# Immortal-ibr/Verifiable-Federated-Training-with-Zero-Knowledge-Proofs-ZK-FL-

Hardware: AMD Instinct MI355X
Metric: Groth16 proofs/sec (training-step circuit, ~2^18 constraints) at 1/8 MI355X (higher is better)
Workload: dtype u32; 1 GPU; groth16 prove, sgd_verified(128, 4, 7, 1000) (BATCH,DIM,DEPTH,PRECISION); constraints=261399, wires=262810, domain=262144, global_batch=20, step=20 proofs per GPU (one per slot), parallelism=replicas1, slots_in_flight=20, hw_queues=28

## Files before the change

include/zkfl.h:

```cpp
#ifndef ZKFL_H
#define ZKFL_H

#include <stddef.h>
#include <stdint.h>

#ifdef __cplusplus
extern "C" {
#endif

#define ZKFL_OK 0
#define ZKFL_E_ARG -1
#define ZKFL_E_FORMAT -2
#define ZKFL_E_PRIME -3
#define ZKFL_E_MISMATCH -4
#define ZKFL_E_DEVICE -5
#define ZKFL_E_OOM -6
#define ZKFL_E_CONSTRAINT -7
#define ZKFL_E_KEY -8

typedef struct zkfl_ctx zkfl_ctx;
typedef struct zkfl_key zkfl_key;
typedef struct zkfl_witness zkfl_witness;
typedef struct zkfl_wprog zkfl_wprog;
typedef struct zkfl_vkey zkfl_vkey;

int zkfl_version(void);
const char* zkfl_build_id(void);
const char* zkfl_last_error(void);
int zkfl_device_count(int* count);

int zkfl_ctx_create(int device, zkfl_ctx** out);
int zkfl_ctx_destroy(zkfl_ctx* ctx);
int zkfl_ctx_set_profiling(zkfl_ctx* ctx, int enabled);
int zkfl_ctx_profile(zkfl_ctx* ctx, const char* name, double* total_ms, uint64_t* launches, double* units,
                     double* median_ms);
int zkfl_ctx_profile_reset(zkfl_ctx* ctx);
int zkfl_ctx_synchronize(zkfl_ctx* ctx);

int zkfl_zkey_load(zkfl_ctx* ctx, const uint8_t* buf, size_t len, zkfl_key** out);
typedef struct zkfl_zkey_file zkfl_zkey_file;
int zkfl_zkey_file_open(const char* path, zkfl_zkey_file** out);
int zkfl_zkey_load_file(zkfl_ctx* ctx, const zkfl_zkey_file* f, zkfl_key** out);
int zkfl_zkey_file_close(zkfl_zkey_file* f);
int zkfl_key_free(zkfl_key* key);
int zkfl_key_info(const zkfl_key* key, uint32_t* n_vars, uint32_t* n_public, uint32_t* domain_size);
int zkfl_key_ab_shared(const zkfl_key* key, uint32_t* d_form, uint32_t* shared_wires, uint32_t* a_bases);
int zkfl_debug_ab_partition(const uint8_t* sec_a, const uint8_t* sec_b1, size_t n, uint32_t shard, uint32_t n_shards,
                            uint32_t* counts, uint32_t* sidx_out, uint8_t* img_out);
typedef struct zkfl_groups_info {
  uint32_t grouped;
  uint32_t learned;
  uint32_t groups;
  uint32_t non_rep;
  uint32_t bases[4];
  uint32_t bases_rep[4];
  uint32_t builds;
  uint32_t last_miss;
  double build_ms;
} zkfl_groups_info;
typedef struct zkfl_group_rows_info {
  uint32_t rows_grouped;
  uint32_t row_classes;
  uint32_t terms;
  uint32_t terms_rep;
  uint32_t wire_list;
  uint32_t wires_over_cap;
  uint32_t last_dirty;
  uint32_t last_plain;
  double rows_build_ms;
} zkfl_group_rows_info;
int zkfl_key_set_groups(zkfl_key* key, const uint32_t* rep, size_t n_vars);
int zkfl_key_learn_groups(zkfl_ctx* ctx, zkfl_key* key, const zkfl_witness* w);
int zkfl_key_groups(const zkfl_key* key, zkfl_groups_info* out);
int zkfl_key_group_rows(const zkfl_key* key, zkfl_group_rows_info* out);
int zkfl_debug_groups(const uint8_t* values, const uint8_t* sig, size_t n, uint32_t* rep_out, const uint32_t* sidx,
                      size_t n_bases, uint32_t u_base, uint32_t* sidx_out, uint32_t* start_out,
                      uint32_t* members_out);
int zkfl_debug_group_rows(const uint32_t* rows, uint32_t domain, const uint32_t* cols, uint32_t cshift,
                          const uint32_t* coefs, const uint32_t* rep, uint32_t n_vars, uint32_t hash_bits,
                          uint32_t wire_cap, uint32_t* cls_out, uint32_t* crp_out, uint32_t* cterms_out,
                          uint32_t* ccoefs_out, uint32_t* wstart_out, uint32_t* wlist_out, uint32_t* info_out);
int zkfl_debug_abc(zkfl_ctx* ctx, zkfl_key* key, const zkfl_witness* w, int grouped, uint8_t* abc_out,
                   uint32_t* counts_out);
int zkfl_key_set_slots(zkfl_key* key, int slots);

int zkfl_groth16_prove(zkfl_ctx* ctx, zkfl_key* key, const uint8_t* wtns, size_t wtns_len,
                       const uint8_t* rs, uint8_t proof_out[256], uint8_t* pub_out, size_t* npub);

int zkfl_witness_upload(zkfl_ctx* ctx, const zkfl_key* key, const uint8_t* wtns, size_t wtns_len,
                        zkfl_witness** out);
int zkfl_witness_free(zkfl_witness* w);
int zkfl_groth16_prove_resident(zkfl_ctx* ctx, zkfl_key* key, const zkfl_witness* w, const uint8_t* rs,
                                uint8_t proof_out[256]);
int zkfl_groth16_prove_batch(zkfl_ctx* ctx, zkfl_key* key, size_t n, const zkfl_witness* const* w,
                             const uint8_t* rs, uint8_t* proofs_out);

int zkfl_groth16_prove_multi(zkfl_ctx* ctx, size_t n, zkfl_key* const* keys, const zkfl_witness* const* w,
                             const uint8_t* rs, uint8_t* proofs_out);

int zkfl_zkey_load_shard(zkfl_ctx* ctx, const uint8_t* buf, size_t len, uint32_t shard, uint32_t n_shards,
                         zkfl_key** out);
int zkfl_key_shard(const zkfl_key* key, uint32_t* shard, uint32_t* n_shards);
int zkfl_groth16_prove_part_batch(zkfl_ctx* ctx, zkfl_key* key, size_t n, const zkfl_witness* const* w,
                                  const uint8_t* rs, uint8_t* parts_out);
int zkfl_groth16_assemble(zkfl_ctx* ctx, size_t n, size_t n_parts, const uint8_t* parts, const uint8_t* rs,
                          uint8_t* proofs_out);

int zkfl_debug_prove_parts(zkfl_ctx* ctx, zkfl_key* key, const uint8_t* wtns, size_t wtns_len, uint8_t* h_out,
                           uint8_t* msm_out);

int zkfl_debug_glv_split(const uint8_t k[32], uint8_t out[40]);

int zkfl_debug_g1_glv_mul(zkfl_ctx* ctx, size_t n, const uint8_t* points, const uint8_t* scalars, uint8_t* out);

int zkfl_debug_msm_front(zkfl_ctx* ctx, uint32_t n1, const size_t* n, const uint8_t* const* bases,
                         const uint8_t* const* scalars, const size_t* n_scalars, const uint32_t* const* sidx,
                         const uint32_t* extra_start, const uint8_t* const* extra, const size_t* n_extra, uint32_t b,
                         const uint8_t* bases_g2, size_t n_b, int fast, int joint, uint8_t* out_g1, uint8_t out_g2[128]);

int zkfl_debug_wtrace(zkfl_ctx* ctx, int op, uint32_t cap, void* out, uint32_t* count);

int zkfl_debug_ntt_coset(zkfl_ctx* ctx, uint8_t* data, uint32_t logn, uint32_t nvec, size_t vstride, int col_max);

int zkfl_msm_g1(zkfl_ctx* ctx, const uint8_t* bases, const uint8_t* scalars, size_t n, uint8_t out[64]);
int zkfl_msm_g2(zkfl_ctx* ctx, const uint8_t* bases, const uint8_t* scalars, size_t n, uint8_t out[128]);
int zkfl_ntt_coset(zkfl_ctx* ctx, uint8_t* data, uint32_t logn);

int zkfl_wprog_load(zkfl_ctx* ctx, const uint8_t* prog, size_t len, zkfl_wprog** out);
int zkfl_wprog_free(zkfl_wprog* prog);
int zkfl_wprog_info(const zkfl_wprog* prog, uint32_t* n_wires, uint32_t* n_inputs, uint32_t* n_public);
size_t zkfl_wtns_size(const zkfl_wprog* prog);
int zkfl_wprog_parse_inputs(const uint8_t* prog, size_t len, const char* input_json, uint8_t* inputs_out, size_t cap,
                            size_t* n_inputs);
int zkfl_witness_compute_json(zkfl_ctx* ctx, const zkfl_wprog* prog, const char* input_json, uint8_t* wtns_out);
int zkfl_witness_compute(zkfl_ctx* ctx, const zkfl_wprog* prog, size_t n, const uint8_t* inputs, uint8_t* wtns_out);
int zkfl_witness_compute_resident(zkfl_ctx* ctx, const zkfl_wprog* prog, const zkfl_key* key, size_t n,
                                  const uint8_t* inputs, zkfl_witness** out);

int zkfl_groth16_full_prove_batch(zkfl_ctx* ctx, zkfl_key* key, const zkfl_wprog* prog, size_t n,
                                  const uint8_t* inputs, const uint8_t* rs, uint8_t* proofs_out, uint8_t* pubs_out);

int zkfl_groth16_full_prove_json(zkfl_ctx* ctx, zkfl_key* key, const zkfl_wprog* prog, const char* input_json,
                                 const uint8_t* rs, uint8_t proof_out[256], uint8_t* pub_out);

int zkfl_groth16_full_prove_json_batch(zkfl_ctx* ctx, zkfl_key* key, const zkfl_wprog* prog, size_t n,
                                       const char* const* input_jsons, const uint8_t* rs, uint8_t* proofs_out,
                                       uint8_t* pubs_out);

int zkfl_groth16_full_prove_multi(zkfl_ctx* ctx, size_t n, zkfl_key* const* keys, const zkfl_wprog* const* progs,
                                  const uint8_t* const* inputs, const uint8_t* rs, uint8_t* proofs_out,
                                  uint8_t* const* pubs_out);

typedef struct zkfl_r1cs zkfl_r1cs;
typedef struct {
  uint32_t n_wires, n_pub_out, n_pub_in, n_prv_in, n_constraints;
  uint64_t n_labels, n_terms;
} zkfl_r1cs_header;
typedef struct {
  uint32_t n_failed, first;
  uint8_t a[32], b[32], c[32];
// ... 132 lines not shown
```

verifiable-federated-training-with-zero-knowledge-proofs-zk-fl-_amd/csrc/groups.h:

```cpp
#pragma once
#include <stddef.h>
#include <stdint.h>
#include <string.h>

#include <algorithm>
#include <unordered_map>
#include <vector>

namespace zkfl {

inline bool groups_valid(const uint32_t* rep, size_t n) {
  for (size_t i = 0; i < n; i++)
    if (rep[i] > i || rep[rep[i]] != rep[i]) return false;
  return true;
}

inline void groups_learn(const uint32_t* w, size_t n, std::vector<uint32_t>& rep) {
  rep.resize(n);
  std::vector<uint32_t> big;
  for (size_t i = 0; i < n; i++) {
    rep[i] = (uint32_t)i;
    const uint32_t* v = w + 8 * i;
    if (v[4] | v[5] | v[6] | v[7]) big.push_back((uint32_t)i);
  }
  std::sort(big.begin(), big.end(), [&](uint32_t a, uint32_t b) {
    const int c = memcmp(w + 8 * (size_t)a, w + 8 * (size_t)b, 32);
    return c ? c < 0 : a < b;
  });
  for (size_t k = 1; k < big.size(); k++)
    if (memcmp(w + 8 * (size_t)big[k], w + 8 * (size_t)big[k - 1], 32) == 0) rep[big[k]] = rep[big[k - 1]];
}

inline void groups_refine(uint32_t* rep, const uint8_t* sig, size_t n) {
  std::unordered_map<uint64_t, uint32_t> first;
  for (size_t i = 0; i < n; i++) {
    const uint32_t r = rep[i];
    if ((sig[i] & ~sig[r]) == 0) continue;
    rep[i] = first.emplace((uint64_t)r << 8 | sig[i], (uint32_t)i).first->second;
  }
}

struct GroupQuery {
  std::vector<uint32_t> sidx;
  std::vector<uint32_t> start;
  std::vector<uint32_t> members;
  uint32_t groups = 0;
  uint32_t non_rep = 0;
};

inline void groups_query(const uint32_t* rep, uint32_t n_vars, const uint32_t* sidx, size_t n, uint32_t u_base,
                         GroupQuery& q) {
  constexpr uint32_t NONE = 0xFFFFFFFFu;
  std::vector<uint32_t> slot_of(n_vars, NONE), to(n, NONE);
  for (size_t j = 0; j < n; j++)
    if (sidx[j] < n_vars) slot_of[sidx[j]] = (uint32_t)j;
  q.sidx.assign(sidx, sidx + n);
  q.start.assign(n + 1, 0);
  q.groups = q.non_rep = 0;
  for (size_t j = 0; j < n; j++) {
    const uint32_t i = sidx[j];
    if (i >= n_vars || rep[i] == i || slot_of[rep[i]] == NONE) continue;
    to[j] = slot_of[rep[i]];
    q.sidx[j] = u_base + i;
    if (q.start[to[j] + 1]++ == 0) q.groups++;
    q.non_rep++;
  }
  for (size_t j = 0; j < n; j++) q.start[j + 1] += q.start[j];
  q.members.resize(q.non_rep);
  std::vector<uint32_t> cur(q.start.begin(), q.start.end() - 1);
  for (size_t j = 0; j < n; j++)
    if (to[j] != NONE) q.members[cur[to[j]]++] = (uint32_t)j;
}


constexpr uint32_t GROUP_ROWS_WIRE_CAP = 256;
constexpr uint32_t GROUP_ROWS_DIRTY_DIV = 8;
inline uint32_t group_rows_dirty_cap(uint32_t domain) { return std::max<uint32_t>(64u, domain / GROUP_ROWS_DIRTY_DIV); }
constexpr uint32_t GROUP_ROWS_MISS_DIV = 64;
inline uint32_t group_rows_miss_cap(uint32_t domain) { return std::max<uint32_t>(64u, domain / GROUP_ROWS_MISS_DIV); }
constexpr uint32_t GROUP_ROWS_OVER = 0x80000000u;

struct GroupRows {
  std::vector<uint32_t> cls;
  std::vector<uint32_t> crp;
  std::vector<uint32_t> cterms;
  std::vector<uint32_t> ccoefs;
  std::vector<uint32_t> wstart;
  std::vector<uint32_t> wlist;
  uint32_t classes = 0;
  uint32_t over_cap = 0;
  bool keep = false;
};

inline void group_rows_build(const uint32_t* rows, uint32_t domain, const uint32_t* cols, uint32_t cshift,
                             const uint32_t* coefs, const uint32_t* rep, uint32_t n_vars, uint32_t hash_bits,
                             uint32_t wire_cap, GroupRows& g) {
  const uint32_t nrows = 2 * domain, K = rows[nrows];
  const uint32_t cmask = cshift ? (1u << cshift) - 1u : 0xFFFFFFFFu;
  std::vector<uint64_t> key(K);
  std::vector<uint32_t> uniq;
  if (cshift) {
    for (uint32_t p = 0; p < K; p++) key[p] = (cols[p] & ~cmask) | rep[cols[p] & cmask];
  } else {
    struct H32 {
      const uint32_t* c;
      size_t operator()(uint32_t p) const {
        uint64_t h = 1469598103934665603ull;
        for (int k = 0; k < 8; k++) h = (h ^ c[8 * (size_t)p + k]) * 1099511628211ull;
        return (size_t)h;
      }
    };
    struct E32 {
      const uint32_t* c;
      bool operator()(uint32_t a, uint32_t b) const { return memcmp(c + 8 * (size_t)a, c + 8 * (size_t)b, 32) == 0; }
    };
    std::unordered_map<uint32_t, uint32_t, H32, E32> ids(16, H32{coefs}, E32{coefs});
    for (uint32_t p = 0; p < K; p++) {
      const auto it = ids.emplace(p, (uint32_t)uniq.size());
      if (it.second) uniq.push_back(p);
      key[p] = (uint64_t)it.first->second << 32 | rep[cols[p]];
    }
  }
  std::vector<uint64_t> hash(nrows);
  const uint64_t hmask = hash_bits >= 64 ? ~0ull : (1ull << hash_bits) - 1ull;
  for (uint32_t r = 0; r < nrows; r++) {
    std::sort(key.begin() + rows[r], key.begin() + rows[r + 1]);
    uint64_t h = 0x9E3779B97F4A7C15ull + (rows[r + 1] - rows[r]);
    for (uint32_t p = rows[r]; p < rows[r + 1]; p++) {
      h = (h ^ key[p]) * 0xFF51AFD7ED558CCDull;
      h ^= h >> 29;
    }
    hash[r] = h & hmask;
  }
  uint32_t tbits = 4;
  while ((1ull << tbits) < 2ull * nrows) tbits++;
  std::vector<uint32_t> table((size_t)1 << tbits, 0xFFFFFFFFu), first;
  const size_t tmask = ((size_t)1 << tbits) - 1;
  g.cls.assign(nrows, 0);
  g.crp.assign(1, 0);
  g.cterms.clear();
  g.ccoefs.clear();
  for (uint32_t r = 0; r < nrows; r++) {
    const uint32_t s = rows[r], len = rows[r + 1] - s;
    size_t slot = (size_t)((hash[r] * 0x9E3779B97F4A7C15ull) >> (64 - tbits)) & tmask;
    uint32_t c;
    for (;; slot = (slot + 1) & tmask) {
      c = table[slot];
      if (c == 0xFFFFFFFFu) break;
      const uint32_t f = first[c];
      if (hash[f] == hash[r] && rows[f + 1] - rows[f] == len &&
          std::equal(key.begin() + s, key.begin() + s + len, key.begin() + rows[f]))
        break;
    }
    if (c == 0xFFFFFFFFu) {
// ... 77 lines not shown
```

verifiable-federated-training-with-zero-knowledge-proofs-zk-fl-_amd/csrc/groups.hip:

```cpp
#include <hip/hip_runtime.h>
#include <stdint.h>

#include <chrono>
#include <cstdio>
#include <vector>

#include "devbufs.h"
#include "groups.h"
#include "objects.h"

using namespace zkfl;

namespace {

ZK_DEV Fq from_m29(const Fq& a) {
  Fq c = fp_zero<FqP>();
  c.v[7] = 0x08000000u;
  return fp_mul(a, c);
}

template <class F>
ZK_DEV Affine<F> load_base(const Affine<F>* __restrict__ p) {
  Affine<F> a = *p;
  Fq* q = reinterpret_cast<Fq*>(&a);
#pragma unroll
  for (int k = 0; k < (int)(sizeof(Affine<F>) / sizeof(Fq)); k++) q[k] = from_m29(q[k]);
  return a;
}

template <class F>
__global__ void __launch_bounds__(64) k_group_sums(const Affine<F>* __restrict__ bases_w, int W, size_t n,
                                                   const uint32_t* __restrict__ start,
                                                   const uint32_t* __restrict__ members, Affine<F>* __restrict__ out) {
  const size_t j = (size_t)blockIdx.x * blockDim.x + threadIdx.x;
  if (j >= n) return;
  const Affine<F> p = load_base<F>(bases_w + j * W);
  const uint32_t b = start[j], e = start[j + 1];
  if (b == e) {
    out[j] = p;
    return;
  }
  XYZZ<F> acc = xyzz_from_affine<F>(p);
  for (uint32_t m = b; m < e; m++) acc = xyzz_madd<F>(acc, load_base<F>(bases_w + (size_t)members[m] * W));
  out[j] = xyzz_to_affine<F>(acc);
}

constexpr int DELTA_T = 256;

__global__ void __launch_bounds__(DELTA_T) k_group_delta(const Fr* __restrict__ w, const uint32_t* __restrict__ rep,
                                                         uint32_t n, Fr* __restrict__ u, uint32_t* __restrict__ cnt,
                                                         uint32_t* __restrict__ miss_out, const GroupMark M) {
  ZK_LIGHT();
  const uint32_t i = blockIdx.x * DELTA_T + threadIdx.x;
  int nz = 0;
  if (i < n) {
    const uint32_t r = rep[i];
    Fr v = fp_zero<FrP>();
    if (r != i) {
      v = fp_sub(w[i], w[r]);
#pragma unroll
      for (int k = 0; k < 8; k++) nz |= v.v[k] != 0;
    }
    u[i] = v;
  }
  if (M.wstart) {
    const unsigned long long m = __ballot(nz);
    if (m) {
      const uint32_t lane = threadIdx.x & (warpSize - 1);
      const int first = __ffsll((long long)m) - 1;
      uint32_t base = 0;
      if ((int)lane == first) base = atomicAdd(&M.state[2], (uint32_t)__popcll(m));
      base = __shfl(base, first);
      const uint32_t at = base + (uint32_t)__popcll(m & ((1ull << lane) - 1ull));
      if (nz && at < M.miss_cap) M.missing[at] = i;
    }
  }
  const int blk = __syncthreads_count(nz);
  if (threadIdx.x == 0) {
    if (blk) atomicAdd(&cnt[0], (uint32_t)blk);
    __threadfence();
    if (atomicAdd(&cnt[1], 1u) == gridDim.x - 1) {
      __threadfence();
      miss_out[0] = atomicExch(&cnt[0], 0u);
      cnt[1] = 0;
    }
  }
}

constexpr int MARK_T = 256, MARK_BLOCKS_MAX = 256;

__global__ void __launch_bounds__(MARK_T) k_group_mark(const GroupMark M) {
  ZK_LIGHT();
  const uint32_t n = M.state[2];
  if (n == 0) return;
  if (n > M.miss_cap) {
    if (blockIdx.x == 0 && threadIdx.x == 0) atomicExch(&M.state[1], 1u);
    return;
  }
  const uint32_t lane = threadIdx.x & (warpSize - 1), per = MARK_T / warpSize;
  for (uint32_t k = blockIdx.x * per + threadIdx.x / warpSize; k < n; k += gridDim.x * per) {
    if (__any((int)__atomic_load_n(&M.state[1], __ATOMIC_RELAXED))) return;
    const uint32_t i = M.missing[k], s = M.wstart[i], e = M.wstart[i + 1] & ~GROUP_ROWS_OVER;
    if (s & GROUP_ROWS_OVER) {
      if (lane == 0) atomicExch(&M.state[1], 1u);
      return;
    }
    for (uint32_t p = s + lane; p < e; p += warpSize) {
      const uint32_t j = M.wlist[p], bit = 1u << (j & 31);
      if (atomicOr(&M.state[GROUP_ROWS_STATE_BITS + (j >> 5)], bit) & bit) continue;
      const uint32_t at = atomicAdd(&M.state[0], 1u);
      if (at < M.cap) M.dirty[at] = j;
      else atomicExch(&M.state[1], 1u);
    }
  }
}

}

namespace zkfl {

template <class F>
void group_sums(hipStream_t st, const Affine<F>* bases_w, int W, size_t n, const uint32_t* start,
                const uint32_t* members, Affine<F>* out) {
  if (n) hipLaunchKernelGGL(k_group_sums<F>, dim3(zk_grid(n, 64)), dim3(64), 0, st, bases_w, W, n, start, members, out);
}
template void group_sums<FqOps>(hipStream_t, const G1Aff*, int, size_t, const uint32_t*, const uint32_t*, G1Aff*);
template void group_sums<Fq2Ops>(hipStream_t, const G2Aff*, int, size_t, const uint32_t*, const uint32_t*, G2Aff*);

void group_delta(hipStream_t st, const Fr* w, const uint32_t* rep, uint32_t n, Fr* u, uint32_t* cnt,
                 uint32_t* miss_out, const GroupMark& mark) {
  hipLaunchKernelGGL(k_group_delta, dim3(zk_grid(n, DELTA_T)), dim3(DELTA_T), 0, st, w, rep, n, u, cnt, miss_out, mark);
}

void group_mark_rows(hipStream_t st, const GroupMark& mark) {
  const unsigned blocks = std::min<unsigned>(zk_grid((size_t)mark.miss_cap * 64, MARK_T), MARK_BLOCKS_MAX);
  hipLaunchKernelGGL(k_group_mark, dim3(blocks), dim3(MARK_T), 0, st, mark);
}

void key_groups_release(zkfl_key* k) {
  msm_bases_free(k->gA);
  msm_bases_free(k->gB1);
  msm_bases_free(k->gB2);
  msm_bases_free(k->gCH);
  void* ptrs[] = {k->grp.d_rep,    k->grp.d_cls,    k->grp.d_crp,  k->grp.d_cterms,
                  k->grp.d_ccoefs, k->grp.d_wstart, k->grp.d_wlist};
  for (void* p : ptrs)
    if (p) (void)hipFree(p);
  const uint32_t builds = k->grp.builds;
  k->grp = KeyGroups();
  k->grp.builds = builds;
}

}

namespace {

template <class F>
hipError_t build_query(const MsmBases<F>& plain, MsmBases<F>& out, const GroupQuery& q, uint32_t extra_start,
                       DevBufs& D, hipStream_t st) {
  ZK_CHECK(msm_bases_alloc(out, plain.n, plain.c));
  if (plain.n == 0) return hipSuccess;
  uint32_t *d_start, *d_members;
  Affine<F>* d_img;
  ZK_CHECK(D.get(&d_start, q.start.size()));
  ZK_CHECK(D.get(&d_members, q.members.size()));
  ZK_CHECK(D.get(&d_img, plain.n));
  ZK_CHECK(hipMemcpyAsync(d_start, q.start.data(), q.start.size() * 4, hipMemcpyHostToDevice, st));
  if (!q.members.empty())
    ZK_CHECK(hipMemcpyAsync(d_members, q.members.data(), q.members.size() * 4, hipMemcpyHostToDevice, st));
  group_sums<F>(st, plain.bases_w, msm_w_of(plain.c), plain.n, d_start, d_members, d_img);
  ZK_CHECK(hipGetLastError());
  return msm_bases_set(out, d_img, q.sidx.data(), extra_start, st, false);
}

bool group_rows_wanted(const zkfl_key* k) {
  return k->ctx->opts.group_rows && k->K != 0 && k->logn > k->ctx->opts.small_logn;
}

hipError_t build_rows(zkfl_key* k, const std::vector<uint32_t>& rep, hipStream_t st) {
  KeyGroups& g = k->grp;
  if (!group_rows_wanted(k)) return hipSuccess;
  const auto t0 = std::chrono::steady_clock::now();
  const uint32_t dom = k->n;
  const size_t K = k->K;
  std::vector<uint32_t> rows(2 * (size_t)dom + 1), cols(K), coefs;
  ZK_CHECK(hipMemcpyAsync(rows.data(), k->rows, rows.size() * 4, hipMemcpyDeviceToHost, st));
  ZK_CHECK(hipMemcpyAsync(cols.data(), k->cols, K * 4, hipMemcpyDeviceToHost, st));
  if (!k->cshift) {
    coefs.resize(K * 8);
    ZK_CHECK(hipMemcpyAsync(coefs.data(), k->coefs, K * 32, hipMemcpyDeviceToHost, st));
  }
  ZK_CHECK(hipStreamSynchronize(st));
  GroupRows R;
  const uint32_t low = (uint32_t)k->ctx->opts.group_rows_cap;
  group_rows_build(rows.data(), dom, cols.data(), k->cshift, coefs.data(), rep.data(), k->nVars, 64,
                   low ? std::min(low, GROUP_ROWS_WIRE_CAP) : GROUP_ROWS_WIRE_CAP, R);
  g.row_classes = R.classes;
  g.terms_rep = (uint32_t)R.cterms.size();
  g.wire_list = (uint32_t)R.wlist.size();
  g.over_cap = R.over_cap;
  if (R.keep && !R.cterms.empty()) {
    auto up = [&](auto*& dst, const std::vector<uint32_t>& v) -> hipError_t {
      ZK_CHECK(hipMalloc(&dst, (v.size() ? v.size() : 1) * 4));
      if (!v.empty()) ZK_CHECK(hipMemcpyAsync(dst, v.data(), v.size() * 4, hipMemcpyHostToDevice, st));
      return hipSuccess;
    };
    ZK_CHECK(up(g.d_cls, R.cls));
    ZK_CHECK(up(g.d_crp, R.crp));
    ZK_CHECK(up(g.d_cterms, R.cterms));
    if (!k->cshift) ZK_CHECK(up(g.d_ccoefs, R.ccoefs));
    ZK_CHECK(up(g.d_wstart, R.wstart));
    ZK_CHECK(up(g.d_wlist, R.wlist));
    ZK_CHECK(hipStreamSynchronize(st));
    g.rows_on = true;
  }
  g.rows_ms = std::chrono::duration<double, std::milli>(std::chrono::steady_clock::now() - t0).count();
  return hipSuccess;
}

int key_build_groups(zkfl_key* k, std::vector<uint32_t>& rep, bool learned, double host_ms) {
  const auto t0 = std::chrono::steady_clock::now();
  HIP_TRY(hipSetDevice(k->ctx->device), "hipSetDevice");
  int rc = key_reset_graphs(k);
  if (rc) return rc;
  key_groups_release(k);
  const uint32_t nV = k->nVars, X = nV, dom = k->n;
  std::vector<uint8_t> sig(nV, 0);
  for (int qi = 0; qi < 4; qi++)
    for (uint32_t i : k->q_sidx[qi])
      if (i < nV) sig[i] |= (uint8_t)(1u << qi);
  groups_refine(rep.data(), sig.data(), nV);
  const uint32_t u_base[4] = {X + 4, X + 4, X + 4, X + dom + 4};
  GroupQuery q[4];
  for (int qi = 0; qi < 4; qi++)
    groups_query(rep.data(), nV, k->q_sidx[qi].data(), k->q_sidx[qi].size(), u_base[qi], q[qi]);
  hipStream_t st = k->ctx->st;
  hipError_t e;
  {
    DevBufs D;
    e = hipMalloc(&k->grp.d_rep, (size_t)(nV ? nV : 1) * 4);
    if (e == hipSuccess) e = hipMemcpyAsync(k->grp.d_rep, rep.data(), (size_t)nV * 4, hipMemcpyHostToDevice, st);
    if (e == hipSuccess) e = build_query(k->bA, k->gA, q[0], X, D, st);
    if (e == hipSuccess) e = build_query(k->bB1, k->gB1, q[1], X, D, st);
    if (e == hipSuccess) e = build_query(k->bB2, k->gB2, q[2], X, D, st);
    if (e == hipSuccess) e = build_query(k->bCH, k->gCH, q[3], X, D, st);
    const hipError_t es = hipStreamSynchronize(st);
    if (e == hipSuccess) e = es;
    if (e == hipSuccess) e = build_rows(k, rep, st);
  }
  if (e != hipSuccess) {
    key_groups_release(k);
    return hip_fail(e, "grouped base sets");
  }
  KeyGroups& g = k->grp;
  g.on = true;
  g.learned = learned;
  for (uint32_t i = 0; i < nV; i++) g.non_rep += rep[i] != i;
  std::vector<uint8_t> has(nV, 0);
  for (uint32_t i = 0; i < nV; i++)
    if (rep[i] != i && !has[rep[i]]) {
      has[rep[i]] = 1;
      g.groups++;
    }
  for (int qi = 0; qi < 4; qi++) {
    g.bases[qi] = (uint32_t)k->q_sidx[qi].size();
    g.bases_rep[qi] = g.bases[qi] - q[qi].non_rep;
  }
  g.builds++;
  g.build_ms = host_ms + std::chrono::duration<double, std::milli>(std::chrono::steady_clock::now() - t0).count();
  fprintf(stderr,
          "zkfl: key of %u wires: %u groups, %u non-representative wires; bases A %u -> %u, B %u -> %u, C+H %u -> %u; "
          "%s and built in %.1f ms\n",
          nV, g.groups, g.non_rep, g.bases[0], g.bases_rep[0], g.bases[1], g.bases_rep[1], g.bases[3], g.bases_rep[3],
          learned ? "learned" : "set", g.build_ms);
  if (group_rows_wanted(k))
    fprintf(stderr,
            "zkfl: key of %u wires: %u row classes, terms %zu -> %u, wire lists %u entries (%u wires over the cap); "
            "%s ABC, built in %.1f ms of the above\n",
            nV, g.row_classes, k->K, g.terms_rep, g.wire_list, g.over_cap, g.rows_on ? "grouped" : "plain", g.rows_ms);
  return ZKFL_OK;
}

int groups_allowed(const zkfl_key* k) {
  if (k->nshards != 1) return fail(ZKFL_E_ARG, "groups: a sharded key keeps the plain form");
  if (!k->ctx->opts.groups) return fail(ZKFL_E_ARG, "groups: turned off on this context (ZKFL_GROUPS=0)");
  return ZKFL_OK;
}

}

int zkfl::key_learn_groups(zkfl_ctx* ctx, zkfl_key* k, const Fr* d_w) {
  const auto t0 = std::chrono::steady_clock::now();
  HIP_TRY(hipSetDevice(ctx->device), "hipSetDevice");
  std::vector<uint32_t> w((size_t)k->nVars * 8), rep;
  HIP_TRY(hipMemcpy(w.data(), d_w, w.size() * 4, hipMemcpyDeviceToHost), "download witness");
  groups_learn(w.data(), k->nVars, rep);
  const double ms = std::chrono::duration<double, std::milli>(std::chrono::steady_clock::now() - t0).count();
  return key_build_groups(k, rep, true, ms);
}

extern "C" {

int zkfl_key_set_groups(zkfl_key* key, const uint32_t* rep, size_t n_vars) {
  if (!key) return fail(ZKFL_E_ARG, "null key");
  if (!rep) {
    HIP_TRY(hipSetDevice(key->ctx->device), "hipSetDevice");
    const int rc = key_reset_graphs(key);
    if (rc) return rc;
    key_groups_release(key);
    return ZKFL_OK;
  }
  int rc = groups_allowed(key);
  if (rc) return rc;
  if (n_vars != key->nVars) return fail(ZKFL_E_ARG, "groups: rep must hold one entry per wire of the key");
  if (!groups_valid(rep, n_vars)) return fail(ZKFL_E_ARG, "groups: rep[i] <= i and rep[rep[i]] == rep[i] must hold");
  std::vector<uint32_t> r(rep, rep + n_vars);
  return key_build_groups(key, r, false, 0.0);
}

int zkfl_key_learn_groups(zkfl_ctx* ctx, zkfl_key* key, const zkfl_witness* w) {
  if (!ctx || !key || !w) return fail(ZKFL_E_ARG, "null argument");
  if (key->ctx != ctx) return fail(ZKFL_E_ARG, "groups: key of another context");
  if (w->key != key) return fail(ZKFL_E_MISMATCH, "witness uploaded for another key");
  const int rc = groups_allowed(key);
  if (rc) return rc;
  return key_learn_groups(ctx, key, w->d);
}

int zkfl_key_groups(const zkfl_key* key, zkfl_groups_info* out) {
  if (!key || !out) return fail(ZKFL_E_ARG, "null argument");
  const KeyGroups& g = key->grp;
  *out = zkfl_groups_info();
  out->grouped = g.on;
  out->learned = g.learned;
  out->groups = g.groups;
  out->non_rep = g.non_rep;
  for (int i = 0; i < 4; i++) {
    out->bases[i] = g.on ? g.bases[i] : (uint32_t)key->q_sidx[i].size();
    out->bases_rep[i] = g.on ? g.bases_rep[i] : out->bases[i];
  }
  out->builds = g.builds;
  out->last_miss = g.last_miss;
  out->build_ms = g.build_ms;
  return ZKFL_OK;
}

int zkfl_key_group_rows(const zkfl_key* key, zkfl_group_rows_info* out) {
  if (!key || !out) return fail(ZKFL_E_ARG, "null argument");
  const KeyGroups& g = key->grp;
  *out = zkfl_group_rows_info();
  out->rows_grouped = g.rows_on;
  out->row_classes = g.row_classes;
  out->terms = (uint32_t)key->K;
  out->terms_rep = g.row_classes ? g.terms_rep : out->terms;
  out->wire_list = g.wire_list;
  out->wires_over_cap = g.over_cap;
  out->last_dirty = g.last_dirty;
  out->last_plain = g.last_plain;
  out->rows_build_ms = g.rows_ms;
  return ZKFL_OK;
}

int zkfl_debug_group_rows(const uint32_t* rows, uint32_t domain, const uint32_t* cols, uint32_t cshift,
                          const uint32_t* coefs, const uint32_t* rep, uint32_t n_vars, uint32_t hash_bits,
                          uint32_t wire_cap, uint32_t* cls_out, uint32_t* crp_out, uint32_t* cterms_out,
                          uint32_t* ccoefs_out, uint32_t* wstart_out, uint32_t* wlist_out, uint32_t* info_out) {
  if (!rows || !rep || !cls_out || !crp_out || !cterms_out || !wstart_out || !wlist_out || !info_out ||
      cshift >= 32 || domain > 0x3FFFFFFFu)
    return fail(ZKFL_E_ARG, "debug_group_rows: bad arguments");
  const uint32_t K = rows[2 * (size_t)domain];
  if (K && (!cols || (!cshift && !coefs))) return fail(ZKFL_E_ARG, "debug_group_rows: terms missing");
  for (uint32_t r = 0; r < 2 * domain; r++)
    if (rows[r] > rows[r + 1]) return fail(ZKFL_E_ARG, "debug_group_rows: row pointers must not descend");
  if (!groups_valid(rep, n_vars)) return fail(ZKFL_E_ARG, "debug_group_rows: not a partition");
  const uint32_t cmask = cshift ? (1u << cshift) - 1u : 0xFFFFFFFFu;
  for (uint32_t p = 0; p < K; p++)
    if ((cols[p] & cmask) >= n_vars) return fail(ZKFL_E_ARG, "debug_group_rows: column past the wires");
  GroupRows R;
  group_rows_build(rows, domain, cols, cshift, coefs, rep, n_vars, hash_bits, wire_cap ? wire_cap : GROUP_ROWS_WIRE_CAP,
                   R);
  auto put = [](uint32_t* dst, const std::vector<uint32_t>& v) {
    if (dst && !v.empty()) memcpy(dst, v.data(), v.size() * 4);
  };
  put(cls_out, R.cls);
  put(crp_out, R.crp);
  put(cterms_out, R.cterms);
  put(ccoefs_out, R.ccoefs);
  put(wstart_out, R.wstart);
  put(wlist_out, R.wlist);
  info_out[0] = R.classes;
  info_out[1] = (uint32_t)R.cterms.size();
  info_out[2] = (uint32_t)R.wlist.size();
  info_out[3] = R.keep;
  return ZKFL_OK;
}

int zkfl_debug_groups(const uint8_t* values, const uint8_t* sig, size_t n, uint32_t* rep_out, const uint32_t* sidx,
                      size_t n_bases, uint32_t u_base, uint32_t* sidx_out, uint32_t* start_out,
                      uint32_t* members_out) {
  if (!rep_out || n > 0x7FFFFFF0u || (n_bases && !sidx)) return fail(ZKFL_E_ARG, "debug_groups: bad arguments");
  std::vector<uint32_t> rep;
  if (values) {
    std::vector<uint32_t> w(n * 8);
    memcpy(w.data(), values, n * 32);
    groups_learn(w.data(), n, rep);
  } else {
    rep.assign(rep_out, rep_out + n);
    if (!groups_valid(rep.data(), n)) return fail(ZKFL_E_ARG, "debug_groups: not a partition");
  }
  if (sig) groups_refine(rep.data(), sig, n);
  memcpy(rep_out, rep.data(), n * 4);
  if (sidx_out || start_out || members_out) {
    GroupQuery q;
    groups_query(rep.data(), (uint32_t)n, sidx, n_bases, u_base, q);
    if (sidx_out) memcpy(sidx_out, q.sidx.data(), n_bases * 4);
    if (start_out) memcpy(start_out, q.start.data(), (n_bases + 1) * 4);
    if (members_out && !q.members.empty()) memcpy(members_out, q.members.data(), q.members.size() * 4);
  }
  return ZKFL_OK;
}

}
```

verifiable-federated-training-with-zero-knowledge-proofs-zk-fl-_amd/csrc/msm.h:

```cpp
#pragma once
#include <algorithm>
#include <cstring>

#include "field29.h"
#include "msm_api.h"
#include "msm_sort.h"
#include "wtrace.h"

namespace zkfl {

template <class F>
struct MsmIO;
template <>
struct MsmIO<FqOps29> {
  using S = FqOps;
  static constexpr int LANES = 1;
  static constexpr int PIECES = 4;
  static ZK_DEV const uint4* piece(const Affine<S>* p, size_t i, int q) {
    return reinterpret_cast<const uint4*>(p + i) + q;
  }
  static ZK_DEV Affine<FqOps29> from_pieces(const uint32_t (&w)[4 * PIECES]) {
    Affine<FqOps29> a;
    uint32_t x[8], y[8];
#pragma unroll
// ... 411 lines not shown
  ZK_WT((L0 ? WT_WSUM0 : WT_WSUM1) | (MsmIO<F>::LANES == 2 ? WT_G2 : 0u));
  ZK_LIGHT();
  constexpr int RB = msm_wsum_rb<L0, Q0, C>();
  __shared__ XYZZ<S> sh[RB], shy[RB];
  msm_wsum_block<F, L0, Q0, C>(ta, blockIdx.y, blockIdx.x, threadIdx.x / MsmIO<F>::LANES, sh, shy, true);
}

template <class S1, class S2>
struct MsmJointArgs {
  MsmTailArgs<S1> a;
  MsmTailArgs<S2> b;
  int n1;
};
constexpr int MSM_JOINT_T = 128;

template <class F1, class F2, int MINW, class S1 = typename MsmIO<F1>::S, class S2 = typename MsmIO<F2>::S>
__global__ void __launch_bounds__(MSM_JOINT_T) __attribute__((amdgpu_waves_per_eu(MINW)))
k_msm_stitch_joint(const MsmJointArgs<S1, S2> ja, int level, int src) {
  ZK_WT(WT_STITCH | WT_JOINT);
  ZK_LIGHT();
  const int y = blockIdx.y;
  if (y < ja.n1) {
    if (ja.a.live[y][level - 1] == 0u) return;
    const uint32_t g = (blockIdx.x * MSM_JOINT_T + threadIdx.x) / MsmIO<F1>::LANES;
    const uint32_t N = msm_items_at<S1>(*ja.a.nnz[y], level, ja.a.target[y]);
    if (g * MSM_SG < N) msm_stitch_lane<F1>(ja.a, y, level, src, g, N);
  } else {
    const int z = y - ja.n1;
    if (ja.b.live[z][level - 1] == 0u) return;
    const uint32_t g = (blockIdx.x * MSM_JOINT_T + threadIdx.x) / MsmIO<F2>::LANES;
    const uint32_t N = msm_items_at<S2>(*ja.b.nnz[z], level, ja.b.target[z]);
    if (g * MSM_SG < N) msm_stitch_lane<F2>(ja.b, z, level, src, g, N);
  }
}

template <class F1, class F2, int MINW, class S1 = typename MsmIO<F1>::S, class S2 = typename MsmIO<F2>::S>
__global__ void __launch_bounds__(2 * MSM_STITCH_LAST) k_msm_stitch_last_joint(const MsmJointArgs<S1, S2> ja, int level,
                                                                                int src) {
  static_assert(MsmIO<F1>::LANES == 1 && MsmIO<F2>::LANES == 2, "joint tails: G1 lanes, G2 lane pairs");
  ZK_WT(WT_STITCH | WT_JOINT);
  ZK_LIGHT();
  const int y = blockIdx.y;
  if (y < ja.n1)
    msm_stitch_last_block<F1>(ja.a, y, level, src);
  else
    msm_stitch_last_block<F2>(ja.b, y - ja.n1, level, src);
}

template <class F1, class F2, int MINW, bool L0, int Q0, int C, class S1 = typename MsmIO<F1>::S,
          class S2 = typename MsmIO<F2>::S>
__global__ void __launch_bounds__((2 * msm_wsum_rb<L0, Q0, C>())) __attribute__((amdgpu_waves_per_eu(MINW)))
k_msm_wsum_joint(const MsmJointArgs<S1, S2> ja) {
  ZK_WT((L0 ? WT_WSUM0 : WT_WSUM1) | WT_JOINT);
  ZK_LIGHT();
  constexpr int RB = msm_wsum_rb<L0, Q0, C>();
  constexpr int NBLK = L0 ? msm_nb_of(C) / (MSM_RB * Q0) : 1;
  constexpr size_t B1 = 2 * 2 * RB * sizeof(XYZZ<S1>), B2 = 2 * RB * sizeof(XYZZ<S2>);
  __shared__ __attribute__((aligned(16))) unsigned char lds[B1 > B2 ? B1 : B2];
  const int y = blockIdx.y;
  if (y < ja.n1) {
    if (2 * (int)blockIdx.x >= NBLK) return;
    const int half = threadIdx.x / RB, bx = 2 * blockIdx.x + half;
    XYZZ<S1>* sh = reinterpret_cast<XYZZ<S1>*>(lds) + half * 2 * RB;
    msm_wsum_block<F1, L0, Q0, C>(ja.a, y, bx, threadIdx.x % RB, sh, sh + RB, bx < NBLK);
  } else {
    XYZZ<S2>* sh = reinterpret_cast<XYZZ<S2>*>(lds);
    msm_wsum_block<F2, L0, Q0, C>(ja.b, y - ja.n1, blockIdx.x, threadIdx.x / MsmIO<F2>::LANES, sh, sh + RB, true);
  }
}

template <class F>
hipError_t msm_bases_alloc(MsmBases<F>& b, size_t n, int c) {
  if (c != MSM_C && c != MSM_C_SMALL) return hipErrorInvalidValue;
  b.n = n;
  b.c = c;
  ZK_CHECK(hipMalloc(&b.bases_w, (n ? n : 1) * msm_w_of(c) * sizeof(Affine<F>)));
  return hipSuccess;
}

template <class F>
void msm_bases_free(MsmBases<F>& b) {
  if (b.bases_w) (void)hipFree(b.bases_w);
  if (b.sidx) (void)hipFree(b.sidx);
  b = MsmBases<F>();
}

template <class F>
hipError_t msm_bases_set(MsmBases<F>& b, const Affine<F>* d_bases, const uint32_t* h_sidx, uint32_t extra_start,
                         hipStream_t st, bool pairs) {
  if (pairs && !std::is_same<F, FqOps>::value) return hipErrorInvalidValue;
  b.extra_start = h_sidx ? extra_start : 0xFFFFFFFFu;
  if (h_sidx && b.n) {
    ZK_CHECK(hipMalloc(&b.sidx, b.n * sizeof(uint32_t)));
    ZK_CHECK(hipMemcpyAsync(b.sidx, h_sidx, b.n * sizeof(uint32_t), hipMemcpyHostToDevice, st));
  }
  if (b.n)
    ZK_CHECK(msm_with_c(b.c, [&](auto cc) {
      constexpr int C = decltype(cc)::value;
      if constexpr (std::is_same<F, FqOps>::value) {
        if (pairs) {
          hipLaunchKernelGGL((k_msm_expand<F, C, true>), dim3(zk_grid(b.n, 64)), dim3(64), 0, st, d_bases, b.n,
                             b.bases_w);
          return hipSuccess;
        }
      }
      hipLaunchKernelGGL((k_msm_expand<F, C>), dim3(zk_grid(b.n, 64)), dim3(64), 0, st, d_bases, b.n, b.bases_w);
      return hipSuccess;
    }));
  const size_t nfq = b.n * msm_w_of(b.c) * (sizeof(Affine<F>) / sizeof(Fq));
  if (nfq)
    hipLaunchKernelGGL(k_msm_to_m29, dim3(zk_grid(nfq, 256)), dim3(256), 0, st, reinterpret_cast<Fq*>(b.bases_w), nfq);
  return hipGetLastError();
}

template <class F>
hipError_t msm_scratch_alloc(MsmScratch<F>& s, size_t cap, int c, hipStream_t st) {
  s.cap = cap;
  s.c = c;
  const size_t m = cap * msm_w_of(c);
  ZK_CHECK(hipMalloc(&s.keys_in, m * sizeof(uint16_t)));
  ZK_CHECK(hipMalloc(&s.keys_out, m * sizeof(uint16_t)));
  ZK_CHECK(hipMalloc(&s.vals_in, m * sizeof(uint32_t)));
  ZK_CHECK(hipMalloc(&s.vals_out, m * sizeof(uint32_t)));
  s.sort_tmp_bytes = MSM_SORT_TMP_WORDS * sizeof(uint32_t);
  ZK_CHECK(hipMalloc(&s.sort_tmp, s.sort_tmp_bytes));
  (void)st;
  return hipSuccess;
}

template <class F>
void msm_scratch_free(MsmScratch<F>& s) {
  void* ptrs[] = {s.keys_in, s.keys_out, s.vals_in, s.vals_out, s.sort_tmp};
  for (void* p : ptrs)
    if (p) (void)hipFree(p);
  s = MsmScratch<F>();
}

template <class F>
uint32_t msm_resident_chunks() {
  if (const char* e = getenv("ZKFL_MSM_TARGET")) return (uint32_t)strtoul(e, nullptr, 10);
  using FC = typename MsmCurve<F>::Compute;
  constexpr int AW = MsmCurve<F>::ACC_WAVES;
  int dev = 0, ncu = 0, nb = 0;
  if (hipGetDevice(&dev) != hipSuccess) return 0;
  if (hipDeviceGetAttribute(&ncu, hipDeviceAttributeMultiprocessorCount, dev) != hipSuccess) return 0;
  if (hipOccupancyMaxActiveBlocksPerMultiprocessor(&nb, k_msm_accumulate<FC, AW>, 64, 0) != hipSuccess) return 0;
  if (ncu <= 0 || nb <= 0) return 0;
  return (uint32_t)ncu * (uint32_t)nb * (64u / MsmIO<FC>::LANES);
}

template <class F>
uint32_t msm_tail_l0(size_t cap) {
  static_assert(MSM_SMALL_L >= 1 && MSM_SMALL_L <= 255 && MsmCurve<F>::L >= 1 && MsmCurve<F>::L <= 255,
                "chunk length: 8 bits of the target argument");
  return cap <= ((size_t)1 << 16) ? (uint32_t)MSM_SMALL_L : (uint32_t)MsmCurve<F>::L;
}

template <class F>
hipError_t msm_tail_alloc(MsmTail<F>& t, size_t cap, int c) {
  if (c != MSM_C && c != MSM_C_SMALL) return hipErrorInvalidValue;
  t.c = c;
  const size_t m = cap * msm_w_of(c);
  t.target = std::min<uint32_t>(msm_resident_chunks<F>(), 0xFFFFFFu);
  t.l0 = msm_tail_l0<F>(cap);
  t.max_chunks = (m + t.l0 - 1) / t.l0;
  if (t.target) t.max_chunks = std::min<size_t>(t.max_chunks, t.target);
  t.item_cap[0] = 2 * t.max_chunks;
  t.item_cap[1] = 2 * ((t.item_cap[0] + MSM_SG - 1) / MSM_SG);
  for (int k = 0; k < 2; k++) {
    ZK_CHECK(hipMalloc(&t.item_key[k], (t.item_cap[k] ? t.item_cap[k] : 2) * sizeof(uint32_t)));
    ZK_CHECK(hipMalloc(&t.item_val[k], (t.item_cap[k] ? t.item_cap[k] : 2) * sizeof(XYZZ<F>)));
  }
  ZK_CHECK(hipMalloc(&t.buckets, msm_nb_of(c) * sizeof(XYZZ<F>)));
  ZK_CHECK(hipMalloc(&t.red_a, MSM_TAIL_RED * sizeof(XYZZ<F>)));
  ZK_CHECK(hipMalloc(&t.red_s, MSM_TAIL_RED * sizeof(XYZZ<F>)));
  ZK_CHECK(hipMalloc(&t.nnz, sizeof(uint32_t)));
  ZK_CHECK(hipMalloc(&t.live, MSM_LIVE_LEVELS * sizeof(uint32_t)));
  return hipSuccess;
}

template <class F>
void msm_tail_free(MsmTail<F>& t) {
  void* ptrs[] = {t.item_key[0], t.item_key[1], t.item_val[0], t.item_val[1], t.buckets, t.red_a, t.red_s, t.nnz,
                  t.live};
  for (void* p : ptrs)
    if (p) (void)hipFree(p);
  t = MsmTail<F>();
}

template <class F>
MsmTailArgs<F> msm_tail_args(MsmTail<F>* const* t, XYZZ<F>* const* outs, int n) {
  MsmTailArgs<F> ta = {};
  ta.c = n > 0 ? t[0]->c : MSM_C;
  for (int i = 0; i < n; i++) {
    for (int k = 0; k < 2; k++) {
      ta.key[i][k] = t[i]->item_key[k];
      ta.val[i][k] = t[i]->item_val[k];
    }
    ta.buckets[i] = t[i]->buckets;
    ta.red_a[i] = t[i]->red_a;
    ta.red_s[i] = t[i]->red_s;
    ta.nnz[i] = t[i]->nnz;
    ta.out[i] = outs ? outs[i] : nullptr;
    ta.live[i] = t[i]->live;
    ta.target[i] = msm_target_arg(*t[i]);
  }
  return ta;
}

template <class F>
bool msm_tails_one_c(MsmTail<F>* const* t, int n) {
  for (int i = 1; i < n; i++)
    if (t[i]->c != t[0]->c) return false;
  return true;
}

template <class F>
hipError_t msm_tails_reset(MsmTail<F>* const* t, int n, hipStream_t st) {
  if (n < 1 || n > MSM_TAIL_MAX || !msm_tails_one_c(t, n)) return hipErrorInvalidValue;
  hipLaunchKernelGGL(k_msm_tail_reset<F>, dim3(128, n), dim3(256), 0, st, msm_tail_args<F>(t, nullptr, n));
  return hipGetLastError();
}

template <class F>
hipError_t msm_sort_multi(const MsmBases<F>* const* b, MsmScratch<F>* const* pl, uint32_t* const* nnz,
                          const uint32_t* const* sc, const uint32_t* const* ex, int n, hipStream_t st) {
  if (n < 1 || n > MSM_TAIL_MAX) return hipErrorInvalidValue;
  MsmSortArgs A = {};
  uint32_t gx = 0;
  int ny = 0;
  bool sorted = true;
  const int c = b[0]->c;
  for (int i = 0; i < n; i++) {
    const size_t m = b[i]->n;
    if (m > pl[i]->cap || b[i]->c != c || pl[i]->c != c) return hipErrorInvalidValue;
    if (m == 0) {
      continue;
    }
    uint32_t per_blk, nblk;
    if (!msm_sort_blocking(m, per_blk, nblk)) return hipErrorInvalidValue;
    MsmSortJob& J = A.j[ny++];
    J = {sc[i], ex[i], b[i]->sidx, b[i]->extra_start, (uint32_t)m, per_blk, nblk,
         static_cast<uint32_t*>(pl[i]->sort_tmp), static_cast<uint32_t*>(pl[i]->sort_tmp) + MSM_SORT_HB * MSM_SORT_MAXBLK,
         nnz[i], pl[i]->keys_in, pl[i]->vals_in, pl[i]->keys_out, pl[i]->vals_out};
    gx = std::max(gx, nblk);
    sorted = sorted && pl[i]->ko_sorted;
    pl[i]->ko_sorted = 1;
  }
  if (ny == 0) return hipSuccess;
  return msm_sort_launch(A, gx, ny, c, sorted, st);
}

template <class F>
hipError_t msm_sort(const MsmBases<F>& b, MsmScratch<F>& pl, uint32_t* nnz, const uint32_t* d_scalars,
                    const uint32_t* d_extra, hipStream_t st) {
  const MsmBases<F>* bp = &b;
  MsmScratch<F>* pp = &pl;
  return msm_sort_multi(&bp, &pp, &nnz, &d_scalars, &d_extra, 1, st);
}

template <class F>
hipError_t msm_accumulate_sorted(const MsmBases<F>& b, const uint16_t* keys, const uint32_t* vals, MsmTail<F>& t,
                                 hipStream_t st, Profiler* prof, const char* tag) {
  if (b.n == 0) return hipSuccess;
  if (b.c != t.c) return hipErrorInvalidValue;
  const size_t m = b.n * msm_w_of(b.c);
  size_t chunks = (m + t.l0 - 1) / t.l0;
  if (t.target) chunks = std::min<size_t>(chunks, t.target);
  if (chunks > t.max_chunks) return hipErrorInvalidValue;
  const int pidx = prof ? prof->begin(tag, st) : -1;
  using FC = typename MsmCurve<F>::Compute;
  constexpr int LN = MsmIO<FC>::LANES;
  constexpr int AW = MsmCurve<F>::ACC_WAVES;
  if (!((ZK_KNOCKOUT & 64) && LN == 1))
    hipLaunchKernelGGL((k_msm_accumulate<FC, AW>), dim3(zk_grid(chunks * LN, 64)), dim3(64), 0, st, keys, vals,
                       b.bases_w, t.nnz, t.item_key[0], t.item_val[0], t.buckets, msm_target_arg(t), t.live);
  if (prof) prof->end(pidx, st, 0.0, t.nnz);
  return hipGetLastError();
}

template <class F>
hipError_t msm_accumulate_sorted_multi(const MsmBases<F>* const* b, const uint16_t* const* keys,
                                       const uint32_t* const* vals, MsmTail<F>* const* t, int n, hipStream_t st) {
  if (n < 1 || n > MSM_TAIL_MAX) return hipErrorInvalidValue;
  using FC = typename MsmCurve<F>::Compute;
  constexpr int LN = MsmIO<FC>::LANES;
  constexpr int AW = MsmCurve<F>::ACC_WAVES;
  MsmAccArgs<F> A = {};
  size_t gx = 0;
  int ny = 0;
  for (int i = 0; i < n; i++) {
    if (b[i]->n == 0) continue;
    if (b[i]->c != t[i]->c) return hipErrorInvalidValue;
    const size_t m = b[i]->n * msm_w_of(b[i]->c);
    size_t chunks = (m + t[i]->l0 - 1) / t[i]->l0;
    if (t[i]->target) chunks = std::min<size_t>(chunks, t[i]->target);
    if (chunks > t[i]->max_chunks) return hipErrorInvalidValue;
    gx = std::max<size_t>(gx, zk_grid(chunks * LN, 64));
    A.keys[ny] = keys[i];
    A.vals[ny] = vals[i];
    A.bases[ny] = b[i]->bases_w;
    A.nnz[ny] = t[i]->nnz;
    A.item_key[ny] = t[i]->item_key[0];
    A.item_val[ny] = t[i]->item_val[0];
    A.buckets[ny] = t[i]->buckets;
    A.target[ny] = msm_target_arg(*t[i]);
    A.live[ny] = t[i]->live;
    ny++;
  }
  if (ny && !((ZK_KNOCKOUT & 64) && LN == 1))
    hipLaunchKernelGGL((k_msm_accumulate_multi<FC, AW>), dim3((uint32_t)gx, ny), dim3(64), 0, st, A);
  return hipGetLastError();
}

template <class F>
hipError_t msm_accumulate(const MsmBases<F>& b, MsmScratch<F>& pl, MsmTail<F>& t, const uint32_t* d_scalars,
                          const uint32_t* d_extra, hipStream_t st, Profiler* prof, const char* tag) {
  ZK_CHECK(msm_sort(b, pl, t.nnz, d_scalars, d_extra, st));
  return msm_accumulate_sorted(b, pl.keys_out, pl.vals_out, t, st, prof, tag);
}

template <class F>
hipError_t msm_stitch(MsmTail<F>* const* t, int n, hipStream_t st) {
  if (n < 1 || n > MSM_TAIL_MAX || !msm_tails_one_c(t, n)) return hipErrorInvalidValue;
  using FC = typename MsmCurve<F>::Compute;
  constexpr int LN = MsmIO<FC>::LANES;
  constexpr int SW = MsmCurve<F>::STITCH_WAVES;
  const MsmTailArgs<F> ta = msm_tail_args<F>(t, nullptr, n);
  size_t N = 0;
  for (int i = 0; i < n; i++) N = std::max(N, t[i]->item_cap[0]);
  N = std::max<size_t>(N, 2);
  int cur = 0;
  for (int level = 1; !(ZK_KNOCKOUT & 8); level++) {
    if (level >= MSM_LIVE_LEVELS) return hipErrorInvalidValue;
    const size_t lanes = (N + MSM_SG - 1) / MSM_SG;
    if (lanes <= (size_t)MSM_STITCH_LAST) {
      hipLaunchKernelGGL((k_msm_stitch_last<FC, SW>), dim3(1, n), dim3(MSM_STITCH_LAST * LN), 0, st, ta, level, cur);
      break;
    }
    hipLaunchKernelGGL((k_msm_stitch<FC, SW>), dim3(zk_grid(lanes * LN, 64), n), dim3(64), 0, st, ta, level, cur);
    if (N <= (size_t)MSM_SG) break;
    N = 2 * lanes;
    cur ^= 1;
  }
  return hipGetLastError();
}

template <class F>
hipError_t msm_wsum(const MsmTailArgs<F>& ta, int n, hipStream_t st, bool fast) {
  if (n < 1 || n > MSM_TAIL_MAX) return hipErrorInvalidValue;
  if (ZK_KNOCKOUT & 16) return hipGetLastError();
  using FC = typename MsmCurve<F>::Compute;
  constexpr int LN = MsmIO<FC>::LANES;
  constexpr int TW = MsmCurve<F>::TAIL_WAVES;
  return msm_with_c(ta.c, [&](auto cc) {
    constexpr int C = decltype(cc)::value, NB = msm_nb_of(C);
    constexpr int Q0 = MsmCurve<F>::WSUM_Q, QF = msm_wsum_q_fast<C>();
    if (fast) {
      hipLaunchKernelGGL((k_msm_wsum<FC, TW, true, QF, C>), dim3(NB / (MSM_RB * QF), n), dim3(MSM_RB * LN), 0, st, ta);
      hipLaunchKernelGGL((k_msm_wsum<FC, TW, false, QF, C>), dim3(1, n), dim3(msm_wsum_rb<false, QF, C>() * LN), 0, st,
                         ta);
    } else {
      hipLaunchKernelGGL((k_msm_wsum<FC, TW, true, Q0, C>), dim3(NB / (MSM_RB * Q0), n), dim3(MSM_RB * LN), 0, st, ta);
      hipLaunchKernelGGL((k_msm_wsum<FC, TW, false, Q0, C>), dim3(1, n), dim3(msm_wsum_rb<false, Q0, C>() * LN), 0, st,
                         ta);
    }
    return hipGetLastError();
  });
}

template <class F>
hipError_t msm_tails(MsmTail<F>* const* t, XYZZ<F>* const* outs, int n, hipStream_t st, bool fast) {
  ZK_CHECK(msm_stitch(t, n, st));
  return msm_wsum(msm_tail_args<F>(t, outs, n), n, st, fast);
}

template <class S1, class S2>
hipError_t msm_tails_joint(MsmTail<S1>* const* t1, XYZZ<S1>* const* o1, int n1, MsmTail<S2>* const* t2,
                           XYZZ<S2>* const* o2, int n2, hipStream_t st, bool fast) {
  if (n1 < 1 || n1 > MSM_TAIL_MAX || n2 < 1 || n2 > MSM_TAIL_MAX || !msm_tails_one_c(t1, n1) ||
      !msm_tails_one_c(t2, n2) || t1[0]->c != t2[0]->c)
    return hipErrorInvalidValue;
  using F1 = typename MsmCurve<S1>::Compute;
  using F2 = typename MsmCurve<S2>::Compute;
  static_assert(MsmCurve<S1>::WSUM_Q == MsmCurve<S2>::WSUM_Q, "joint reduction: one fold for both curves");
  constexpr int W = std::min(MsmCurve<S1>::TAIL_WAVES, MsmCurve<S2>::TAIL_WAVES);
  constexpr int L1 = MsmIO<F1>::LANES, L2 = MsmIO<F2>::LANES;
  static_assert(L1 == 1 && L2 == 2, "joint tails: G1 lanes, G2 lane pairs");
  MsmJointArgs<S1, S2> ja;
  ja.a = msm_tail_args<S1>(t1, o1, n1);
  ja.b = msm_tail_args<S2>(t2, o2, n2);
  ja.n1 = n1;
  const int ny = n1 + n2;
  size_t N1 = 2, N2 = 2;
  for (int i = 0; i < n1; i++) N1 = std::max(N1, t1[i]->item_cap[0]);
  for (int i = 0; i < n2; i++) N2 = std::max(N2, t2[i]->item_cap[0]);
  int cur = 0;
  for (int level = 1; !(ZK_KNOCKOUT & 8); level++) {
    if (level >= MSM_LIVE_LEVELS) return hipErrorInvalidValue;
    const size_t lanes1 = (N1 + MSM_SG - 1) / MSM_SG, lanes2 = (N2 + MSM_SG - 1) / MSM_SG;
    if (lanes1 <= (size_t)MSM_STITCH_LAST && lanes2 <= (size_t)MSM_STITCH_LAST) {
      hipLaunchKernelGGL((k_msm_stitch_last_joint<F1, F2, W>), dim3(1, ny), dim3(2 * MSM_STITCH_LAST), 0, st, ja,
                         level, cur);
      break;
    }
    const size_t bx = std::max(zk_grid(lanes1 * L1, MSM_JOINT_T), zk_grid(lanes2 * L2, MSM_JOINT_T));
    hipLaunchKernelGGL((k_msm_stitch_joint<F1, F2, W>), dim3((uint32_t)bx, ny), dim3(MSM_JOINT_T), 0, st, ja, level, cur);
    if (N1 > (size_t)MSM_SG) N1 = 2 * lanes1;
    if (N2 > (size_t)MSM_SG) N2 = 2 * lanes2;
    cur ^= 1;
  }
  if (ZK_KNOCKOUT & 16) return hipGetLastError();
  return msm_with_c(t1[0]->c, [&](auto cc) {
    constexpr int C = decltype(cc)::value, NB = msm_nb_of(C);
    constexpr int Q0 = MsmCurve<S1>::WSUM_Q, QF = msm_wsum_q_fast<C>();
    if (fast) {
      hipLaunchKernelGGL((k_msm_wsum_joint<F1, F2, W, true, QF, C>), dim3(NB / (MSM_RB * QF), ny),
                         dim3(2 * msm_wsum_rb<true, QF, C>()), 0, st, ja);
      hipLaunchKernelGGL((k_msm_wsum_joint<F1, F2, W, false, QF, C>), dim3(1, ny), dim3(2 * msm_wsum_rb<false, QF, C>()),
                         0, st, ja);
    } else {
      hipLaunchKernelGGL((k_msm_wsum_joint<F1, F2, W, true, Q0, C>), dim3(NB / (MSM_RB * Q0), ny),
                         dim3(2 * msm_wsum_rb<true, Q0, C>()), 0, st, ja);
      hipLaunchKernelGGL((k_msm_wsum_joint<F1, F2, W, false, Q0, C>), dim3(1, ny), dim3(2 * msm_wsum_rb<false, Q0, C>()),
                         0, st, ja);
    }
    return hipGetLastError();
  });
}

template <class F>
hipError_t msm_run(const MsmBases<F>& b, MsmScratch<F>& pl, MsmTail<F>& t, const uint32_t* d_scalars,
                   const uint32_t* d_extra, XYZZ<F>* d_out, hipStream_t st, Profiler* prof, const char* tag) {
  MsmTail<F>* tp = &t;
  ZK_CHECK(msm_tails_reset(&tp, 1, st));
  ZK_CHECK(msm_accumulate(b, pl, t, d_scalars, d_extra, st, prof, tag));
  return msm_tails(&tp, &d_out, 1, st);
}

}
```

verifiable-federated-training-with-zero-knowledge-proofs-zk-fl-_amd/csrc/msm_api.h:

```cpp
#pragma once
#include <hip/hip_runtime.h>

#include <cstdlib>
#include <type_traits>

#include "common.h"
#include "curve.h"
#include "prof.h"

namespace zkfl {

constexpr int MSM_C = 16;
constexpr int MSM_C_SMALL = 14;
constexpr int MSM_SMALL_C_BASES = 1 << 16;
constexpr int MSM_SORT_HIGH_BITS = 7;
constexpr int MSM_SORT_BIN_THREADS = 1024;
constexpr int MSM_SG = 8;
constexpr int MSM_SMALL_L = 8;

struct FqOps29;
struct Fq2Pair29;
template <class S>
struct MsmCurve;
template <>
struct MsmCurve<FqOps> {
  using Compute = FqOps29;
  static constexpr int ACC_WAVES = 3, STITCH_WAVES = 2, TAIL_WAVES = 2;
  static constexpr int L = 16, WSUM_Q = 16;
};
template <>
struct MsmCurve<Fq2Ops> {
  using Compute = Fq2Pair29;
  static constexpr int ACC_WAVES = 2, STITCH_WAVES = 2, TAIL_WAVES = 2;
  static constexpr int L = 16, WSUM_Q = 16;
};

__host__ __device__ constexpr int msm_w_of(int c) { return (255 + c - 1) / c; }
__host__ __device__ constexpr int msm_nb_of(int c) { return 1 << (c - 1); }
constexpr int MSM_W = msm_w_of(MSM_C);
constexpr int MSM_NB = msm_nb_of(MSM_C);
constexpr int MSM_W_MAX = msm_w_of(MSM_C < MSM_C_SMALL ? MSM_C : MSM_C_SMALL);
static_assert(MSM_C >= 14 && MSM_C <= 16 && MSM_C_SMALL >= 14 && MSM_C_SMALL <= 16,
              "window width: the widths the GPU parity suite runs (>= 64 low counters per high bin of the bucket sort)");
#ifndef ZK_KNOCKOUT
#define ZK_KNOCKOUT 0
#endif
#if ZK_KNOCKOUT != 0 && !defined(ZK_KNOCKOUT_AB_ONLY)
#error "ZK_KNOCKOUT builds compute wrong proofs: timing A/B only (define ZK_KNOCKOUT_AB_ONLY to acknowledge)"
#endif
constexpr int MSM_RB = 64;
constexpr uint32_t MSM_ITEM_DUMMY = 0x80000000u;
template <class S>
__host__ __device__ inline uint32_t msm_chunk_len(uint32_t nnz, uint32_t target) {
  const uint32_t L0 = (target >> 24) ? (target >> 24) : (uint32_t)MsmCurve<S>::L;
  target &= 0xFFFFFFu;
  if (target == 0) return L0;
  const uint32_t l = (uint32_t)(((uint64_t)nnz + target - 1) / target);
  return l > L0 ? l : L0;
}
constexpr int MSM_LIVE_LEVELS = 32;


template <class F>
struct MsmBases {
  size_t n = 0;
  int c = MSM_C;
  Affine<F>* bases_w = nullptr;
  uint32_t* sidx = nullptr;
  uint32_t extra_start = 0xFFFFFFFFu;
};

template <class F>
struct MsmScratch {
  size_t cap = 0;
  int c = MSM_C;
  uint16_t* keys_in = nullptr;
  uint16_t* keys_out = nullptr;
  uint32_t* vals_in = nullptr;
  uint32_t* vals_out = nullptr;
  void* sort_tmp = nullptr;
  size_t sort_tmp_bytes = 0;
  int ko_sorted = 0;
};

template <class F>
struct MsmTail {
  size_t max_chunks = 0;
  int c = MSM_C;
  uint32_t* item_key[2] = {nullptr, nullptr};
  XYZZ<F>* item_val[2] = {nullptr, nullptr};
  size_t item_cap[2] = {0, 0};
  XYZZ<F>* buckets = nullptr;
  XYZZ<F>* red_a = nullptr;
  XYZZ<F>* red_s = nullptr;
  uint32_t* nnz = nullptr;
  uint32_t* live = nullptr;
  uint32_t target = 0;
  uint32_t l0 = 0;
};

template <class F>
inline uint32_t msm_target_arg(const MsmTail<F>& t) {
  return (t.l0 << 24) | (t.target & 0xFFFFFFu);
}

inline int msm_pick_c(size_t n) {
  if (const char* e = getenv("ZKFL_MSM_C")) {
    const int c = atoi(e);
    if (c == MSM_C || c == MSM_C_SMALL) return c;
  }
  return n <= (size_t)MSM_SMALL_C_BASES ? MSM_C_SMALL : MSM_C;
}
template <class Fn>
hipError_t msm_with_c(int c, Fn&& fn) {
  if (c == MSM_C) return fn(std::integral_constant<int, MSM_C>());
  if constexpr (MSM_C_SMALL != MSM_C)
    if (c == MSM_C_SMALL) return fn(std::integral_constant<int, MSM_C_SMALL>());
  return hipErrorInvalidValue;
}

constexpr int MSM_TAIL_MAX = 4;
constexpr int MSM_TAIL_RED = 4 * MSM_RB;

template <class F>
hipError_t msm_bases_alloc(MsmBases<F>& b, size_t n, int c);
template <class F>
hipError_t msm_bases_set(MsmBases<F>& b, const Affine<F>* src, const uint32_t* h_sidx, uint32_t extra_start,
                         hipStream_t st, bool pairs = false);
template <class F>
void msm_bases_free(MsmBases<F>& b);
template <class F>
hipError_t msm_scratch_alloc(MsmScratch<F>& s, size_t cap, int c, hipStream_t st);
template <class F>
void msm_scratch_free(MsmScratch<F>& s);
template <class F>
hipError_t msm_tail_alloc(MsmTail<F>& t, size_t cap, int c);
template <class F>
void msm_tail_free(MsmTail<F>& t);
template <class F>
hipError_t msm_accumulate(const MsmBases<F>& b, MsmScratch<F>& s, MsmTail<F>& t, const uint32_t* scalars,
                          const uint32_t* extra, hipStream_t st, Profiler* prof, const char* tag);
template <class F>
hipError_t msm_tails_reset(MsmTail<F>* const* t, int n, hipStream_t st);
template <class F>
hipError_t msm_sort(const MsmBases<F>& b, MsmScratch<F>& s, uint32_t* nnz, const uint32_t* sc, const uint32_t* ex,
                    hipStream_t st);
template <class F>
hipError_t msm_accumulate_sorted(const MsmBases<F>& b, const uint16_t* keys, const uint32_t* vals, MsmTail<F>& t,
                                 hipStream_t st, Profiler* prof, const char* tag);
template <class F>
hipError_t msm_tails(MsmTail<F>* const* t, XYZZ<F>* const* outs, int n, hipStream_t st, bool fast = false);
template <class F>
hipError_t msm_run(const MsmBases<F>& b, MsmScratch<F>& s, MsmTail<F>& t, const uint32_t* scalars,
                   const uint32_t* extra, XYZZ<F>* out, hipStream_t st, Profiler* prof, const char* tag);
template <class F>
hipError_t msm_sort_multi(const MsmBases<F>* const* b, MsmScratch<F>* const* s, uint32_t* const* nnz,
                          const uint32_t* const* sc, const uint32_t* const* ex, int n, hipStream_t st);
template <class F>
hipError_t msm_accumulate_sorted_multi(const MsmBases<F>* const* b, const uint16_t* const* keys,
                                       const uint32_t* const* vals, MsmTail<F>* const* t, int n, hipStream_t st);

#define ZKFL_MSM_API(X, F)                                                                                     \
  X hipError_t msm_bases_alloc<F>(MsmBases<F>&, size_t, int);                                                  \
  X hipError_t msm_bases_set<F>(MsmBases<F>&, const Affine<F>*, const uint32_t*, uint32_t, hipStream_t, bool); \
  X void msm_bases_free<F>(MsmBases<F>&);                                                                      \
  X hipError_t msm_scratch_alloc<F>(MsmScratch<F>&, size_t, int, hipStream_t);                                 \
  X void msm_scratch_free<F>(MsmScratch<F>&);                                                                  \
  X hipError_t msm_tail_alloc<F>(MsmTail<F>&, size_t, int);                                                    \
  X void msm_tail_free<F>(MsmTail<F>&);                                                                        \
  X hipError_t msm_accumulate<F>(const MsmBases<F>&, MsmScratch<F>&, MsmTail<F>&, const uint32_t*,             \
                                 const uint32_t*, hipStream_t, Profiler*, const char*);                        \
  X hipError_t msm_tails_reset<F>(MsmTail<F>* const*, int, hipStream_t);                                       \
  X hipError_t msm_sort<F>(const MsmBases<F>&, MsmScratch<F>&, uint32_t*, const uint32_t*, const uint32_t*,    \
                           hipStream_t);                                                                       \
  X hipError_t msm_accumulate_sorted<F>(const MsmBases<F>&, const uint16_t*, const uint32_t*, MsmTail<F>&,     \
                                        hipStream_t, Profiler*, const char*);                                  \
  X hipError_t msm_tails<F>(MsmTail<F>* const*, XYZZ<F>* const*, int, hipStream_t, bool);                      \
  X hipError_t msm_run<F>(const MsmBases<F>&, MsmScratch<F>&, MsmTail<F>&, const uint32_t*, const uint32_t*,   \
                          XYZZ<F>*, hipStream_t, Profiler*, const char*);                                      \
  X hipError_t msm_sort_multi<F>(const MsmBases<F>* const*, MsmScratch<F>* const*, uint32_t* const*,           \
                                 const uint32_t* const*, const uint32_t* const*, int, hipStream_t);            \
  X hipError_t msm_accumulate_sorted_multi<F>(const MsmBases<F>* const*, const uint16_t* const*,               \
                                              const uint32_t* const*, MsmTail<F>* const*, int, hipStream_t);
ZKFL_MSM_API(extern template, FqOps)
ZKFL_MSM_API(extern template, Fq2Ops)

hipError_t msm_tails_joint(MsmTail<FqOps>* const* t1, XYZZ<FqOps>* const* o1, int n1, MsmTail<Fq2Ops>* const* t2,
                           XYZZ<Fq2Ops>* const* o2, int n2, hipStream_t st, bool fast);

}
```

verifiable-federated-training-with-zero-knowledge-proofs-zk-fl-_amd/csrc/msm_joint.hip:

```cpp
#include "msm.h"

namespace zkfl {
hipError_t zk_wtrace_bind_joint(const WtBuf& b) { return zk_wtrace_bind_tu(b); }
hipError_t msm_tails_joint(MsmTail<FqOps>* const* t1, XYZZ<FqOps>* const* o1, int n1, MsmTail<Fq2Ops>* const* t2,
                           XYZZ<Fq2Ops>* const* o2, int n2, hipStream_t st, bool fast) {
  return msm_tails_joint<FqOps, Fq2Ops>(t1, o1, n1, t2, o2, n2, st, fast);
}
}
```

verifiable-federated-training-with-zero-knowledge-proofs-zk-fl-_amd/csrc/msm_sort.h:

```cpp
#pragma once
#include "msm_api.h"

namespace zkfl {

constexpr int MSM_SORT_T = 256;
constexpr int MSM_SORT_HB = 1 << MSM_SORT_HIGH_BITS;
constexpr int MSM_SORT_MAXBLK = 32768 / MSM_SORT_HB;
constexpr int MSM_SORT_BT = 1024;
constexpr int MSM_SORT_BINT = MSM_SORT_BIN_THREADS;
static_assert(MSM_SORT_HB <= MSM_SORT_T, "bucket sort split");
static_assert(MSM_SORT_HB * MSM_SORT_MAXBLK == 32 * MSM_SORT_BT, "scan: 32 counters per thread");
constexpr size_t MSM_SORT_TMP_WORDS = MSM_SORT_HB * MSM_SORT_MAXBLK + MSM_SORT_HB + 1;

struct MsmSortJob {
  const uint32_t* scalars;
  const uint32_t* extra;
  const uint32_t* sidx;
  uint32_t extra_start;
  uint32_t n, per_blk, nblk;
  uint32_t* cnt;
  uint32_t* bin_start;
  uint32_t* nnz;
  uint16_t* keys_in;
  uint32_t* vals_in;
  uint16_t* keys_out;
  uint32_t* vals_out;
};
struct MsmSortArgs {
  MsmSortJob j[MSM_TAIL_MAX];
};

inline bool msm_sort_blocking(size_t m, uint32_t& per_blk, uint32_t& nblk) {
  const size_t per = (m + MSM_SORT_MAXBLK - 1) / MSM_SORT_MAXBLK;
  const size_t pb = per < MSM_SORT_T ? (size_t)MSM_SORT_T : (per + MSM_SORT_T - 1) / MSM_SORT_T * MSM_SORT_T;
  per_blk = (uint32_t)pb;
  nblk = (uint32_t)((m + pb - 1) / pb);
  return nblk <= (uint32_t)MSM_SORT_MAXBLK;
}

hipError_t msm_sort_launch(const MsmSortArgs& A, uint32_t gx, int ny, int c, bool sorted, hipStream_t st);

}
```

verifiable-federated-training-with-zero-knowledge-proofs-zk-fl-_amd/csrc/msm_sort.hip:

```cpp
#include "msm_sort.h"
#include "wtrace.h"

namespace zkfl {

hipError_t zk_wtrace_bind_sort(const WtBuf& b) { return zk_wtrace_bind_tu(b); }

template <int C>
constexpr int msm_sort_lb() {
  return C - 1 - MSM_SORT_HIGH_BITS;
}
template <int C>
constexpr int msm_sort_nl() {
  return 1 << msm_sort_lb<C>();
}

template <int C>
ZK_DEV uint32_t msm_window(const uint32_t (&s)[8], int j) {
  const int b = C * j, w = b >> 5, sh = b & 31;
  uint32_t x = s[w] >> sh;
  if (sh + C > 32 && w + 1 < 8) x |= s[w + 1] << (32 - sh);
  return x & ((1u << C) - 1u);
}

template <int C, class Fn>
ZK_DEV void msm_for_digits(const uint32_t* __restrict__ scalars, const uint32_t* __restrict__ extra,
                           const uint32_t* __restrict__ sidx, uint32_t extra_start, size_t i, Fn&& fn) {
  constexpr int W = msm_w_of(C), NB = msm_nb_of(C);
  const uint32_t si = sidx ? sidx[i] : (uint32_t)i;
  const uint32_t* src = si < extra_start ? scalars + (size_t)si * 8 : extra + (size_t)(si - extra_start) * 8;
  const uint4* sp = reinterpret_cast<const uint4*>(src);
  const uint4 a = sp[0], b = sp[1];
  const uint32_t s[8] = {a.x, a.y, a.z, a.w, b.x, b.y, b.z, b.w};
  uint32_t carry = 0;
#pragma unroll
  for (int j = 0; j < W; j++) {
    const uint32_t raw = msm_window<C>(s, j);
    int32_t d = (int32_t)(raw + carry);
    carry = d > NB ? 1u : 0u;
    if (carry) d -= (1 << C);
    if (d != 0) {
      const uint32_t mag = (uint32_t)(d < 0 ? -d : d);
      fn(mag - 1, (uint32_t)(i * W + j) | (d < 0 ? 0x80000000u : 0u));
    }
  }
}

template <int C>
__global__ void __launch_bounds__(MSM_SORT_T) k_msm_bin_count(const MsmSortArgs A) {
  ZK_WT(WT_SORT_COUNT);
  ZK_LIGHT();
  constexpr int LB = msm_sort_lb<C>();
  const MsmSortJob& J = A.j[blockIdx.y];
  if (blockIdx.x >= J.nblk) return;
  __shared__ uint32_t h[MSM_SORT_HB];
  if (threadIdx.x < MSM_SORT_HB) h[threadIdx.x] = 0;
  __syncthreads();
  const size_t i0 = (size_t)blockIdx.x * J.per_blk, i1 = i0 + J.per_blk < J.n ? i0 + J.per_blk : J.n;
  for (size_t i = i0 + threadIdx.x; i < i1; i += MSM_SORT_T)
    msm_for_digits<C>(J.scalars, J.extra, J.sidx, J.extra_start, i,
                      [&](uint32_t key, uint32_t) { atomicAdd(&h[key >> LB], 1u); });
  __syncthreads();
  if (threadIdx.x < MSM_SORT_HB) J.cnt[(size_t)threadIdx.x * J.nblk + blockIdx.x] = h[threadIdx.x];
}

#if defined(__HIP_DEVICE_COMPILE__) && !defined(__gfx950__)
#error "the bucket sort's scan needs gfx950's 160 KB of LDS"
#endif
static __global__ void __launch_bounds__(MSM_SORT_BT) k_msm_bin_scan(const MsmSortArgs A) {
  ZK_WT(WT_SORT_SCAN);
  ZK_LIGHT();
  const MsmSortJob& J = A.j[blockIdx.y];
  uint32_t* __restrict__ cnt = J.cnt;
  uint32_t* __restrict__ bin_start = J.bin_start;
  const uint32_t nblk = J.nblk;
  __shared__ uint32_t c[MSM_SORT_HB * MSM_SORT_MAXBLK + MSM_SORT_BT];
  __shared__ uint32_t part[MSM_SORT_BT];
  const uint32_t total = MSM_SORT_HB * nblk, t = threadIdx.x;
  for (uint32_t k = t; k < total; k += MSM_SORT_BT) c[k + (k >> 5)] = cnt[k];
  __syncthreads();
  uint32_t s = 0;
  for (uint32_t q = 0; q < 32; q++) {
    const uint32_t k = t * 32 + q;
    if (k < total) s += c[k + (k >> 5)];
  }
  part[t] = s;
  __syncthreads();
  for (uint32_t off = 1; off < MSM_SORT_BT; off <<= 1) {
    const uint32_t v = t >= off ? part[t - off] : 0u;
    __syncthreads();
    part[t] += v;
    __syncthreads();
  }
  uint32_t run = part[t] - s;
  for (uint32_t q = 0; q < 32; q++) {
    const uint32_t k = t * 32 + q;
    if (k < total) {
      const uint32_t v = c[k + (k >> 5)];
      c[k + (k >> 5)] = run;
      run += v;
    }
  }
  __syncthreads();
  for (uint32_t k = t; k < total; k += MSM_SORT_BT) {
    const uint32_t v = c[k + (k >> 5)];
    cnt[k] = v;
    if (k % nblk == 0) bin_start[k / nblk] = v;
  }
  if (t == MSM_SORT_BT - 1) {
    bin_start[MSM_SORT_HB] = part[t];
    *J.nnz = part[t];
  }
}

template <int C>
__global__ void __launch_bounds__(MSM_SORT_T) k_msm_bin_scatter(const MsmSortArgs A) {
  ZK_WT(WT_SORT_SCATTER);
  ZK_LIGHT();
  constexpr int LB = msm_sort_lb<C>();
  const MsmSortJob& J = A.j[blockIdx.y];
  if (blockIdx.x >= J.nblk) return;
  __shared__ uint32_t cur[MSM_SORT_HB];
  if (threadIdx.x < MSM_SORT_HB) cur[threadIdx.x] = J.cnt[(size_t)threadIdx.x * J.nblk + blockIdx.x];
  __syncthreads();
  uint16_t* __restrict__ keys = J.keys_in;
  uint32_t* __restrict__ vals = J.vals_in;
  const size_t i0 = (size_t)blockIdx.x * J.per_blk, i1 = i0 + J.per_blk < J.n ? i0 + J.per_blk : J.n;
  for (size_t i = i0 + threadIdx.x; i < i1; i += MSM_SORT_T)
    msm_for_digits<C>(J.scalars, J.extra, J.sidx, J.extra_start, i, [&](uint32_t key, uint32_t val) {
      const uint32_t p = atomicAdd(&cur[key >> LB], 1u);
      keys[p] = (uint16_t)key;
      vals[p] = val;
    });
}

template <int BINT, int NL>
__global__ void __launch_bounds__(BINT) k_msm_bin_sort(const MsmSortArgs A) {
  static_assert(BINT >= NL && BINT <= 1024 && NL >= 64, "bins: one thread per low counter");
  ZK_WT(WT_SORT_BINS);
  ZK_LIGHT();
  const MsmSortJob& J = A.j[blockIdx.y];
  const uint32_t* __restrict__ bin_start = J.bin_start;
  const uint16_t* __restrict__ tk = J.keys_in;
  const uint32_t* __restrict__ tv = J.vals_in;
  uint16_t* __restrict__ ko = J.keys_out;
  uint32_t* __restrict__ vo = J.vals_out;
  __shared__ uint32_t c[NL];
  const uint32_t b0 = bin_start[blockIdx.x], b1 = bin_start[blockIdx.x + 1], t = threadIdx.x;
  if (b0 == b1) return;
  if (t < NL) c[t] = 0;
  __syncthreads();
  for (uint32_t p = b0 + t; p < b1; p += BINT) atomicAdd(&c[tk[p] & (NL - 1)], 1u);
  __syncthreads();
  uint32_t v = 0, x = 0;
  if (t < NL) {
    v = c[t];
    x = v;
#pragma unroll
    for (int o = 1; o < 64; o <<= 1) {
      const uint32_t y = __shfl_up(x, o);
      if ((t & 63) >= (uint32_t)o) x += y;
    }
  }
  __shared__ uint32_t wt[NL / 64];
  if (t < NL && (t & 63) == 63) wt[t >> 6] = x;
  __syncthreads();
  if (t < NL) {
    uint32_t base = b0;
    for (uint32_t w = 0; w < (t >> 6); w++) base += wt[w];
    c[t] = base + x - v;
  }
  __syncthreads();
  for (uint32_t p = b0 + t; p < b1; p += BINT) {
    const uint16_t key = tk[p];
    const uint32_t val = tv[p];
    const uint32_t q = atomicAdd(&c[key & (NL - 1)], 1u);
    ko[q] = key;
    vo[q] = val;
  }
}

hipError_t msm_sort_launch(const MsmSortArgs& A, uint32_t gx, int ny, int c, bool sorted, hipStream_t st) {
  return msm_with_c(c, [&](auto cc) {
    constexpr int C = decltype(cc)::value;
    constexpr int NL = msm_sort_nl<C>();
    static_assert(NL >= 64 && NL <= 1024 && MSM_SORT_BINT >= NL, "bins: one thread per low counter");
    hipLaunchKernelGGL((k_msm_bin_count<C>), dim3(gx, ny), dim3(MSM_SORT_T), 0, st, A);
    hipLaunchKernelGGL(k_msm_bin_scan, dim3(1, ny), dim3(MSM_SORT_BT), 0, st, A);
    if (!(ZK_KNOCKOUT & 2) || !sorted) {
      hipLaunchKernelGGL((k_msm_bin_scatter<C>), dim3(gx, ny), dim3(MSM_SORT_T), 0, st, A);
      hipLaunchKernelGGL((k_msm_bin_sort<MSM_SORT_BINT, NL>), dim3(MSM_SORT_HB, ny), dim3(MSM_SORT_BINT), 0, st, A);
    }
    return hipGetLastError();
  });
}

}
```

verifiable-federated-training-with-zero-knowledge-proofs-zk-fl-_amd/csrc/objects.h:

```cpp
#pragma once
#include <hip/hip_runtime.h>
#include <stdint.h>

#include <atomic>
#include <string>
#include <vector>

#include "curve.h"
#include "field.h"
#include "msm_api.h"
#include "ntt.h"
#include "prof.h"
#include "wtrace.h"
#include "zkfl.h"

namespace zkfl {
struct VkDev;
struct PosTables;
struct WProg;

int fail(int code, const std::string& msg);
int hip_fail(hipError_t e, const char* where);
}

#define HIP_TRY(x, where)                              \
  do {                                                 \
    hipError_t _e = (x);                               \
    if (_e != hipSuccess) return ::zkfl::hip_fail(_e, where); \
  } while (0)

using namespace zkfl;

struct WitPipe;

struct SchedOpts {
  bool graph = true;
  bool stagger = true;
  bool lowlat = true;
  bool fast_wsum = true;
  int small_logn = 16;
  bool ab_shared = true;
  bool groups = true;
  int group_min_batch = 8;
  bool group_rows = true;
  int group_rows_cap = 0;
};

struct zkfl_ctx {
  int device = 0;
  hipStream_t st = nullptr;
  SchedOpts opts;
  Profiler prof;
  zkfl::VkDev* vk = nullptr;
  zkfl::PosTables* pos = nullptr;
  void* asm_buf = nullptr;
  size_t asm_cap = 0;
  WtBuf wt;
  std::atomic<int> refs{1};
};

struct ProofSlot {
  hipStream_t st_main = nullptr;
  hipEvent_t ev_done = nullptr;
  MsmScratch<FqOps> g1s;
#if ZK_KNOCKOUT & 2
  MsmScratch<FqOps> g1s_ko[3];
#endif
  MsmTail<FqOps> g1t[4];
  MsmScratch<Fq2Ops> g2s;
  MsmTail<Fq2Ops> g2t;
  Fr* extra = nullptr;
  Fr* abc = nullptr;
  Fr* abc_head = nullptr;
  Fr* abc_tail = nullptr;
  Fr* h = nullptr;
  uint32_t* grp_cnt = nullptr;
  uint32_t* gr_state = nullptr;
  uint32_t* gr_dirty = nullptr;
  uint32_t* gr_missing = nullptr;
  Fr* cls_val = nullptr;
  size_t cls_cap = 0;
  zkfl_key* key = nullptr;
  bool grouped_run = false;
  bool rows_run = false;
  G1P* res = nullptr;
  G2P* resB2 = nullptr;
  Fr* d_rs = nullptr;
  uint32_t* d_parts = nullptr;
  uint8_t* pinned = nullptr;
  hipStream_t st_lat[2] = {nullptr, nullptr};
  hipEvent_t ev_lat[3] = {nullptr, nullptr, nullptr};
  MsmScratch<FqOps> g1s_b;
  MsmScratch<FqOps> g1s_a;
  hipGraph_t graph = nullptr;
  hipGraphExec_t graph_exec = nullptr;
  Fr* w_stage = nullptr;
  uint32_t direct_proofs = 0;
  bool nnz_alias = false;
  bool busy = false;
  int index = 0;
  size_t job = 0;
  uint8_t* out_proof = nullptr;
  uint8_t* out_part = nullptr;
};

struct KeyGroups {
  bool on = false;
  bool learned = false;
  uint32_t groups = 0;
  uint32_t non_rep = 0;
  uint32_t bases[4] = {0, 0, 0, 0};
  uint32_t bases_rep[4] = {0, 0, 0, 0};
  double build_ms = 0;
  uint32_t builds = 0;
  uint32_t last_miss = 0;
  uint32_t* d_rep = nullptr;
  bool rows_on = false;
  uint32_t row_classes = 0;
  uint32_t terms_rep = 0;
  uint32_t wire_list = 0;
  uint32_t over_cap = 0;
  double rows_ms = 0;
  uint32_t last_dirty = 0, last_plain = 0;
  uint32_t *d_cls = nullptr, *d_crp = nullptr, *d_cterms = nullptr, *d_wstart = nullptr, *d_wlist = nullptr;
  Fr* d_ccoefs = nullptr;
};

struct zkfl_key {
  zkfl_ctx* ctx = nullptr;
  uint32_t nVars = 0, nPub = 0, n = 0;
  int logn = 0;
  size_t nC = 0;
  size_t K = 0;
  uint32_t* rows = nullptr;
  uint32_t* cols = nullptr;
  Fr* coefs = nullptr;
  uint32_t cshift = 0;
  MsmBases<FqOps> bA, bB1;
  MsmBases<Fq2Ops> bB2;
  MsmBases<FqOps> bCH;
  MsmBases<FqOps> gA, gB1, gCH;
  MsmBases<Fq2Ops> gB2;
  KeyGroups grp;
  std::vector<uint32_t> q_sidx[4];
  Fr* dbg_zero = nullptr;
  bool a_diff = false;
  uint32_t ab_shared = 0;
  bool share_b = false;
  bool front = false;
  int msm_c = MSM_C;
  NttPlan ntt;
  std::vector<ProofSlot*> slots;
  int max_slots = 3;
  uint32_t shard = 0, nshards = 1;
  WitPipe* wpipe = nullptr;
};

struct zkfl_witness {
  const zkfl_key* key = nullptr;
  Fr* d = nullptr;
  std::vector<uint8_t> pub;
};

struct zkfl_wprog {
  zkfl_ctx* ctx = nullptr;
  zkfl::WProg* p = nullptr;
};

struct zkfl_vkey {
  zkfl_ctx* ctx = nullptr;
  zkfl::VkDev* vk = nullptr;
  void* wtab = nullptr;
  bool wave_ok = false;
};

namespace zkfl {
void ctx_retain(zkfl_ctx* ctx);
void ctx_release(zkfl_ctx* ctx);
int pos_ready(zkfl_ctx* ctx);
int get_slot(zkfl_key* k, size_t idx, ProofSlot** out);
void key_release_slots(zkfl_key* k);
int key_reset_graphs(zkfl_key* k);
void key_groups_release(zkfl_key* k);
int key_learn_groups(zkfl_ctx* ctx, zkfl_key* k, const Fr* d_w);
constexpr size_t MISS_OFF = 456;
}
```

verifiable-federated-training-with-zero-knowledge-proofs-zk-fl-_amd/csrc/prove.hip:

```cpp
#include <hip/hip_runtime.h>
#include <stdint.h>
#include <string.h>
#include <sys/random.h>

#include <algorithm>
#include <atomic>
#include <chrono>
#include <condition_variable>
#include <mutex>
#include <string>
#include <thread>
#include <vector>

#include "assemble.h"
#include "devbufs.h"
#include "glv.h"
#include "groups.h"
#include "host_parse.h"
#include "objects.h"
#include "poly.h"
#include "witness.h"

using namespace zkfl;

// ... 8 lines not shown
    if (st) {
      (void)hipStreamSynchronize(st);
      (void)hipStreamDestroy(st);
      st = nullptr;
    }
  for (hipEvent_t& e : s->ev_lat)
    if (e) {
      (void)hipEventDestroy(e);
      e = nullptr;
    }
}

void slot_release(ProofSlot* s) {
  if (!s) return;
  if (s->st_main) (void)hipStreamSynchronize(s->st_main);
  slot_drop_lowlat(s);
  if (s->nnz_alias) s->g2t.nnz = nullptr;
  msm_scratch_free(s->g1s);
#if ZK_KNOCKOUT & 2
  for (MsmScratch<FqOps>& x : s->g1s_ko) msm_scratch_free(x);
#endif
  for (auto& t : s->g1t) msm_tail_free(t);
  msm_scratch_free(s->g2s);
  msm_tail_free(s->g2t);
  void* ptrs[] = {s->abc, s->abc_head, s->abc_tail, s->h, s->res, s->resB2, s->d_rs, s->d_parts,
                  s->w_stage, s->grp_cnt, s->gr_state, s->gr_dirty, s->gr_missing, s->cls_val};
  for (void* p : ptrs)
    if (p) (void)hipFree(p);
  if (s->pinned) (void)hipHostFree(s->pinned);
  msm_scratch_free(s->g1s_b);
  msm_scratch_free(s->g1s_a);
  if (s->graph_exec) (void)hipGraphExecDestroy(s->graph_exec);
  if (s->graph) (void)hipGraphDestroy(s->graph);
  if (s->ev_done) (void)hipEventDestroy(s->ev_done);
  if (s->st_main) (void)hipStreamDestroy(s->st_main);
  delete s;
}

hipError_t slot_side_resources(ProofSlot* s, const zkfl_key* k, bool need_streams) {
  if (need_streams) {
    for (hipStream_t& st : s->st_lat)
      if (!st) ZK_CHECK(hipStreamCreateWithFlags(&st, hipStreamNonBlocking));
    for (hipEvent_t& e : s->ev_lat)
      if (!e) ZK_CHECK(hipEventCreateWithFlags(&e, hipEventDisableTiming));
  }
  if (!s->g1s_a.keys_out) ZK_CHECK(msm_scratch_alloc(s->g1s_a, k->bA.n, k->msm_c, k->ctx->st));
  if (!s->g1s_b.keys_out) ZK_CHECK(msm_scratch_alloc(s->g1s_b, k->bB1.n, k->msm_c, k->ctx->st));
  return hipSuccess;
}

hipError_t slot_create(zkfl_key* k, ProofSlot** out) {
  ProofSlot* s = new ProofSlot();
  *out = s;
  const size_t nV = k->nVars, n = k->n;
  const size_t cap1 = std::max<size_t>({k->bA.n, k->bB1.n, k->bCH.n});
  hipStream_t st = k->ctx->st;
  ZK_CHECK(hipStreamCreateWithFlags(&s->st_main, hipStreamNonBlocking));
  ZK_CHECK(hipEventCreateWithFlags(&s->ev_done, hipEventDisableTiming));
  const int c = k->msm_c;
  ZK_CHECK(msm_scratch_alloc(s->g1s, cap1, c, st));
#if ZK_KNOCKOUT & 2
  for (MsmScratch<FqOps>& x : s->g1s_ko) {
    ZK_CHECK(msm_scratch_alloc(x, cap1, c, st));
    ZK_CHECK(hipMemsetAsync(x.keys_out, 0, cap1 * msm_w_of(c) * sizeof(uint16_t), st));
    ZK_CHECK(hipMemsetAsync(x.vals_out, 0, cap1 * msm_w_of(c) * sizeof(uint32_t), st));
  }
#endif
  const size_t caps[4] = {k->bA.n, k->bB1.n, k->bCH.n, k->bCH.n};
  for (int i = 0; i < 4; i++) ZK_CHECK(msm_tail_alloc(s->g1t[i], caps[i], c));
  ZK_CHECK(msm_scratch_alloc(s->g2s, k->bB2.n, c, st));
  ZK_CHECK(msm_tail_alloc(s->g2t, k->bB2.n, c));
  if (k->share_b && !ZK_KNOCKOUT) {
    ZK_CHECK(hipFree(s->g2t.nnz));
    s->g2t.nnz = s->g1t[1].nnz;
    s->nnz_alias = true;
  }
  if (k->ctx->opts.graph) ZK_CHECK(hipMalloc(&s->w_stage, nV * 32));
  if (k->front) ZK_CHECK(slot_side_resources(s, k, false));
  const bool may_group = k->ctx->opts.groups && k->nshards == 1;
  ZK_CHECK(hipMalloc(&s->h, (n + 4 + (may_group ? nV : 0)) * 32));
  s->extra = s->h + n;
  ZK_CHECK(hipMalloc(&s->grp_cnt, 2 * sizeof(uint32_t)));
  ZK_CHECK(hipMemsetAsync(s->grp_cnt, 0, 2 * sizeof(uint32_t), st));
  if (may_group && k->ctx->opts.group_rows && k->K && k->logn > k->ctx->opts.small_logn) {
    ZK_CHECK(hipMalloc(&s->gr_state, group_rows_state_words(n) * sizeof(uint32_t)));
    ZK_CHECK(hipMalloc(&s->gr_missing, (size_t)group_rows_miss_cap((uint32_t)n) * sizeof(uint32_t)));
    ZK_CHECK(hipMalloc(&s->gr_dirty, (size_t)group_rows_dirty_cap((uint32_t)n) * sizeof(uint32_t)));
  }
  s->key = k;
  ZK_CHECK(hipMalloc(&s->abc, n * 3 * 32));
  const size_t abc_chunks = (k->K + ABC_L - 1) / ABC_L + 1;
  ZK_CHECK(hipMalloc(&s->abc_head, abc_chunks * 32));
  ZK_CHECK(hipMalloc(&s->abc_tail, abc_chunks * 32));
  ZK_CHECK(hipMalloc(&s->res, 5 * sizeof(G1P)));
  ZK_CHECK(hipMalloc(&s->resB2, sizeof(G2P)));
  ZK_CHECK(hipMalloc(&s->d_rs, 2 * 32 + 4 * sizeof(GlvScalar)));
  ZK_CHECK(hipMalloc(&s->d_parts, PART_WORDS * 4));
  ZK_CHECK(hipHostMalloc(&s->pinned, 2048, hipHostMallocCoherent));
  return hipStreamSynchronize(st);
}

}

int zkfl::get_slot(zkfl_key* k, size_t idx, ProofSlot** out) {
  size_t want = idx % (size_t)k->max_slots;
  while (k->slots.size() <= want) {
    ProofSlot* s = nullptr;
    hipError_t e = slot_create(k, &s);
    if (e != hipSuccess) {
      slot_release(s);
      return hip_fail(e, "proof slot allocation");
    }
    s->index = (int)k->slots.size();
    k->slots.push_back(s);
  }
  *out = k->slots[want];
  return ZKFL_OK;
}

constexpr int WIT_SETS = 4;
struct WitPipe {
  struct Set {
    Fr* W = nullptr;
    Fr* d = nullptr;
    uint32_t* in = nullptr;
    uint32_t* fail = nullptr;
    Fr** outs = nullptr;
    uint8_t* pin_in = nullptr;
    hipEvent_t ev = nullptr;
  };
  size_t G = 0, nw = 0, n_in = 0;
  hipStream_t st = nullptr;
  Set set[WIT_SETS];
};

namespace {

void wpipe_release(WitPipe* p) {
  if (!p) return;
  if (p->st) (void)hipStreamSynchronize(p->st);
  for (auto& b : p->set) {
    for (void* q : {(void*)b.W, (void*)b.d, (void*)b.in, (void*)b.fail, (void*)b.outs})
      if (q) (void)hipFree(q);
    if (b.pin_in) (void)hipHostFree(b.pin_in);
    if (b.ev) (void)hipEventDestroy(b.ev);
  }
  if (p->st) (void)hipStreamDestroy(p->st);
  delete p;
}

}

int zkfl::key_reset_graphs(zkfl_key* k) {
  for (ProofSlot* s : k->slots)
    if (s->busy) return fail(ZKFL_E_ARG, "slots busy");
  for (ProofSlot* s : k->slots) {
    if (s->st_main) (void)hipStreamSynchronize(s->st_main);
    if (s->graph_exec) (void)hipGraphExecDestroy(s->graph_exec);
    if (s->graph) (void)hipGraphDestroy(s->graph);
    s->graph_exec = nullptr;
    s->graph = nullptr;
  }
  return ZKFL_OK;
}

void zkfl::key_release_slots(zkfl_key* k) {
  wpipe_release(k->wpipe);
  k->wpipe = nullptr;
  for (ProofSlot* s : k->slots) slot_release(s);
  k->slots.clear();
}

namespace {

hipError_t wpipe_get(zkfl_key* k, size_t G, size_t nw, size_t n_in, WitPipe** out) {
  WitPipe* p = k->wpipe;
  if (p && p->G == G && p->nw == nw && p->n_in == n_in) {
    *out = p;
    return hipSuccess;
  }
  wpipe_release(p);
  k->wpipe = p = new WitPipe();
  p->G = G;
  p->nw = nw;
  p->n_in = n_in;
  ZK_CHECK(hipStreamCreateWithFlags(&p->st, hipStreamNonBlocking));
  for (auto& b : p->set) {
    ZK_CHECK(hipMalloc(&b.W, G * nw * 32));
    ZK_CHECK(hipMalloc(&b.d, G * nw * 32));
    ZK_CHECK(hipMalloc(&b.in, G * n_in * 32 + 16));
    ZK_CHECK(hipMalloc(&b.fail, G * 4));
    ZK_CHECK(hipMalloc(&b.outs, G * sizeof(Fr*)));
    ZK_CHECK(hipHostMalloc(&b.pin_in, G * n_in * 32 + 16));
    ZK_CHECK(hipEventCreateWithFlags(&b.ev, hipEventDisableTiming));
    std::vector<Fr*> ptrs(G);
    for (size_t j = 0; j < G; j++) ptrs[j] = b.d + j * nw;
    ZK_CHECK(hipMemcpy(b.outs, ptrs.data(), G * sizeof(Fr*), hipMemcpyHostToDevice));
  }
  *out = p;
  return hipSuccess;
}

int get_rs(const uint8_t* rs, uint32_t out[16]) {
  if (rs) {
    memcpy(out, rs, 64);
    if (!fr_lt_r(out) || !fr_lt_r(out + 8)) return fail(ZKFL_E_ARG, "r/s must be < r");
    return ZKFL_OK;
  }
  for (int k = 0; k < 2; k++) {
    for (int tries = 0;; tries++) {
      uint8_t b[32];
      if (getrandom(b, 32, 0) != 32) return fail(ZKFL_E_DEVICE, "getrandom failed");
      b[31] &= 0x3f;
      memcpy(out + 8 * k, b, 32);
      if (fr_lt_r(out + 8 * k)) break;
      if (tries > 64) return fail(ZKFL_E_DEVICE, "rng");
    }
  }
  return ZKFL_OK;
}

int check_fr(const uint8_t* v, size_t count, const std::string& what) {
  for (size_t i = 0; i < count; i++) {
    uint32_t w[8];
    memcpy(w, v + 32 * i, 32);
    if (!fr_lt_r(w)) return fail(ZKFL_E_ARG, what + " " + std::to_string(i) + " is not < r");
  }
  return ZKFL_OK;
}

enum class ProofMode {
  Proof,
  Parts,
  SplitPart,
};

enum class Schedule { Lowlat, Front, Chain };

struct ProofPlan {
  ProofMode mode;
  Schedule schedule;
  bool share_b_sort;
  bool light_first;
  bool joint_tails;
  bool fast_wsum;
  bool graph;
  bool grouped;
  bool group_rows;
};

struct PlanBases {
  const MsmBases<FqOps>&A, &B1, &CH;
  const MsmBases<Fq2Ops>& B2;
};
inline PlanBases plan_bases(const zkfl_key* k, const ProofPlan& p) {
  if (p.grouped) return {k->gA, k->gB1, k->gCH, k->gB2};
  return {k->bA, k->bB1, k->bCH, k->bB2};
}

ProofPlan plan_proof(const SchedOpts& o, const zkfl_key* k, const ProofSlot* s, ProofMode mode, bool batch_of_one,
                     const Profiler* prof) {
  ProofPlan p = {};
  p.mode = mode;
  p.grouped = mode == ProofMode::Proof && k->grp.on && !ZK_KNOCKOUT;
  p.group_rows = p.grouped && k->grp.rows_on && s->gr_state;
  const bool plain = mode == ProofMode::Proof && k->share_b && !prof->serialize && !ZK_KNOCKOUT;
  const bool want_lowlat = batch_of_one && o.lowlat;
  p.graph = o.graph && s->w_stage && !want_lowlat && plain && !prof->on && s->direct_proofs > 0;
  p.share_b_sort = k->share_b && !(ZK_KNOCKOUT & 32);
  if (want_lowlat && plain) {
    p.schedule = Schedule::Lowlat;
    p.fast_wsum = o.fast_wsum;
    return p;
  }
  p.joint_tails = p.share_b_sort && k->front;
  const bool front = p.joint_tails && mode != ProofMode::Parts && !(ZK_KNOCKOUT & 2);
  p.schedule = front ? Schedule::Front : Schedule::Chain;
  p.light_first = !front && o.stagger && (s->index & 1) && !prof->serialize;
  p.fast_wsum = o.fast_wsum && k->logn <= o.small_logn;
  return p;
}

inline const GlvScalar* glv_halves(const ProofSlot* s) {
  return reinterpret_cast<const GlvScalar*>(reinterpret_cast<const uint8_t*>(s->d_rs) + 64);
}

void start(zkfl_key* k, ProofSlot* s, const ProofPlan& p) {
  const bool parts = p.mode == ProofMode::Parts;
  const int ntails = parts ? 4 : 3;
  ProofStart ps = {};
  auto add = [&](void* buckets, size_t bytes, uint32_t* nnz, uint32_t* live) {
    ps.buckets[ps.n] = static_cast<uint4*>(buckets);
    ps.nvec[ps.n] = (uint32_t)(bytes / sizeof(uint4));
    ps.nnz[ps.n] = nnz;
    ps.live[ps.n] = live;
    ps.n++;
  };
  const size_t nb = msm_nb_of(k->msm_c);
  for (int i = 0; i < ntails; i++) add(s->g1t[i].buckets, nb * sizeof(G1P), s->g1t[i].nnz, s->g1t[i].live);
  if (p.share_b_sort) add(s->g2t.buckets, nb * sizeof(G2P), s->g2t.nnz, s->g2t.live);
  uint32_t* res3 = parts ? nullptr : reinterpret_cast<uint32_t*>(s->res + 3);
  if (p.graph) {
    ps.w_src_host = reinterpret_cast<const uint64_t*>(s->pinned + W_PTR_OFF);
    ps.w_dst = reinterpret_cast<uint4*>(s->w_stage);
    ps.w_nvec = (uint32_t)((size_t)k->nVars * 32 / sizeof(uint4));
  }
  if (p.group_rows) {
    ps.gr_state = s->gr_state;
    ps.gr_words = (uint32_t)group_rows_state_words(k->n);
  }
  proof_start(s->st_main, reinterpret_cast<const uint32_t*>(s->pinned + 256), reinterpret_cast<uint32_t*>(s->d_rs),
              s->extra, parts, res3, ps);
}

inline GroupMark group_mark(const zkfl_key* k, const ProofSlot* s, const ProofPlan& p) {
  if (!p.group_rows) return GroupMark{};
  return {k->grp.d_wstart, k->grp.d_wlist, s->gr_state, s->gr_missing, group_rows_miss_cap(k->n), s->gr_dirty,
          group_rows_dirty_cap(k->n)};
}

void abc_stage(zkfl_key* k, ProofSlot* s, const Fr* d_w, hipStream_t st, const ProofPlan& p) {
  const size_t n = k->n;
  const uint32_t K = (uint32_t)k->K;
  const AbcTerms T = {k->cols, k->coefs, k->cshift};
  if (p.group_rows) {
    const KeyGroups& g = k->grp;
    const AbcTerms R = {g.d_cterms, k->cshift ? k->coefs : g.d_ccoefs, k->cshift};
    const AbcGrouped G = {g.d_crp, g.row_classes, R, g.terms_rep, g.d_cls, s->cls_val, s->gr_state, s->gr_dirty,
                          group_rows_dirty_cap(k->n), reinterpret_cast<uint32_t*>(s->pinned + MISS_OFF) + 1};
    abc_grouped(st, G, k->rows, n, T, d_w, K, s->abc_head, s->abc_tail, s->abc);
    return;
  }
  if (K) abc_chunks(st, k->rows, (uint32_t)(2 * n), T, d_w, K, s->abc_head, s->abc_tail, s->abc);
  abc_rows(st, k->rows, n, K, s->abc_head, s->abc_tail, s->abc);
}

hipError_t abc_ntt(zkfl_key* k, ProofSlot* s, const Fr* d_w, hipStream_t st, const ProofPlan& p, Profiler* prof) {
  const size_t n = k->n;
  int pi = prof->begin("abc", st);
  abc_stage(k, s, d_w, st, p);
  prof->end(pi, st, (double)k->K);
  pi = prof->begin("ntt", st);
  if (!(ZK_KNOCKOUT & 4)) ZK_CHECK(ntt_coset_shift(k->ntt, s->abc, 3, n, st));
  prof->end(pi, st, 3.0 * (double)n);
  join_h(st, s->abc, n, s->h);
  return hipSuccess;
}

hipError_t b2_from_b1_sort(const MsmBases<Fq2Ops>& bB2, MsmTail<Fq2Ops>& g2t, const uint32_t* b1_nnz, bool nnz_alias,
                           const MsmScratch<FqOps>& sorted, hipStream_t st, Profiler* prof) {
  if (!nnz_alias) ZK_CHECK(hipMemcpyAsync(g2t.nnz, b1_nnz, sizeof(uint32_t), hipMemcpyDeviceToDevice, st));
  return msm_accumulate_sorted(bB2, sorted.keys_out, sorted.vals_out, g2t, st, prof, "msm_accumulate_g2");
}

int finish(const zkfl_key* k, ProofSlot* s, const ProofPlan& p, Profiler* prof) {
  hipStream_t st = s->st_main;
  if (k->a_diff) fold_a(st, s->res);
  if (p.mode == ProofMode::SplitPart) {
    part_out(st, s->res, s->resB2, s->d_parts);
    HIP_TRY(hipMemcpyAsync(s->pinned + 512, s->d_parts, PART_WORDS * 4, hipMemcpyDeviceToHost, st), "download part");
  }
  if (p.mode == ProofMode::Proof && !(ZK_KNOCKOUT & 1)) {
    const int pa = prof->begin("assemble", st);
    assemble(st, 1, s->res, s->resB2, glv_halves(s), proof_out(s));
    prof->end(pa, st, 1.0);
  }
  return ZKFL_OK;
}

int run_lowlat(zkfl_key* k, ProofSlot* s, const Fr* d_w, const ProofPlan& p, Profiler* prof) {
  HIP_TRY(slot_side_resources(s, k, true), "latency schedule resources");
  hipStream_t st = s->st_main, sb = s->st_lat[0], sa = s->st_lat[1];
  hipEvent_t ev = s->ev_lat[0], ev_b2 = s->ev_lat[1], ev_t = s->ev_lat[2];
  const uint32_t *W = (const uint32_t*)d_w, *E = (const uint32_t*)s->extra;
  const PlanBases b = plan_bases(k, p);
  MsmTail<FqOps>* tails[3] = {&s->g1t[0], &s->g1t[1], &s->g1t[2]};
  G1P* outs[3] = {s->res + 0, s->res + 1, s->res + 2};
  MsmTail<Fq2Ops>* t2 = &s->g2t;
  G2P* o2 = s->resB2;
  HIP_TRY(hipEventRecord(ev, st), "event");
  HIP_TRY(hipStreamWaitEvent(sb, ev, 0), "wait");
  HIP_TRY(msm_sort(b.B1, s->g1s_b, s->g1t[1].nnz, W, E, sb), "msm B sort");
  HIP_TRY(hipEventRecord(ev, sb), "event");
  HIP_TRY(hipStreamWaitEvent(sa, ev, 0), "wait");
  HIP_TRY(b2_from_b1_sort(b.B2, s->g2t, s->g1t[1].nnz, s->nnz_alias, s->g1s_b, sb, prof), "msm B2");
  HIP_TRY(msm_tails(&t2, &o2, 1, sb, p.fast_wsum), "msm B2 tail");
  HIP_TRY(hipEventRecord(ev_b2, sb), "event");
  HIP_TRY(msm_accumulate_sorted(b.B1, s->g1s_b.keys_out, s->g1s_b.vals_out, s->g1t[1], sa, prof,
                                   "msm_accumulate_g1"), "msm B1");
  HIP_TRY(msm_accumulate(b.A, s->g1s_a, s->g1t[0], W, E, sa, prof, "msm_accumulate_g1"), "msm A");
  HIP_TRY(msm_tails(tails, outs, 2, sa, p.fast_wsum), "msm tails A, B1");
  if (k->a_diff) fold_a(sa, s->res);
  assemble_t(sa, s->res, glv_halves(s), proof_out(s));
  HIP_TRY(hipEventRecord(ev_t, sa), "event");
  HIP_TRY(abc_ntt(k, s, d_w, st, p, prof), "ntt");
  HIP_TRY(msm_accumulate(b.CH, s->g1s, s->g1t[2], W, (const uint32_t*)s->h, st, prof, "msm_accumulate_g1"),
          "msm C+H");
  HIP_TRY(msm_tails(&tails[2], &outs[2], 1, st, p.fast_wsum), "msm tail C+H");
  HIP_TRY(hipStreamWaitEvent(st, ev_b2, 0), "wait");
  HIP_TRY(hipStreamWaitEvent(st, ev_t, 0), "wait");
  const int pa = prof->begin("assemble", st);
  assemble_c(st, s->res, s->resB2, proof_out(s));
  prof->end(pa, st, 1.0);
  return ZKFL_OK;
}

struct FrontMsm {
  int n1 = 0;
  const MsmBases<FqOps>* bases[MSM_TAIL_MAX] = {};
  MsmScratch<FqOps>* scratch[MSM_TAIL_MAX] = {};
  MsmTail<FqOps>* tails[MSM_TAIL_MAX] = {};
  const uint32_t* scalars[MSM_TAIL_MAX] = {};
  const uint32_t* extra[MSM_TAIL_MAX] = {};
  G1P* outs[MSM_TAIL_MAX] = {};
  int ib = 1;
  const MsmBases<Fq2Ops>* b2 = nullptr;
  MsmTail<Fq2Ops>* t2 = nullptr;
  bool nnz_alias = false;
  G2P* out2 = nullptr;
};
int front_msm(const FrontMsm& m, hipStream_t st, bool fast, bool joint, Profiler* prof) {
  const int n = m.n1;
  uint32_t* nn[MSM_TAIL_MAX] = {};
  const uint16_t* kk[MSM_TAIL_MAX] = {};
  const uint32_t* vv[MSM_TAIL_MAX] = {};
  for (int i = 0; i < n; i++) nn[i] = m.tails[i]->nnz;
  HIP_TRY(msm_sort_multi(m.bases, m.scratch, nn, m.scalars, m.extra, n, st), "msm A, B1, C+H sorts");
  for (int i = 0; i < n; i++) {
    kk[i] = m.scratch[i]->keys_out;
    vv[i] = m.scratch[i]->vals_out;
  }
  HIP_TRY(msm_accumulate_sorted_multi(m.bases, kk, vv, m.tails, n, st), "msm A, B1, C+H");
  HIP_TRY(b2_from_b1_sort(*m.b2, *m.t2, m.tails[m.ib]->nnz, m.nnz_alias, *m.scratch[m.ib], st, prof), "msm B2");
  MsmTail<Fq2Ops>* t2 = m.t2;
  G2P* o2 = m.out2;
  if (joint) {
    HIP_TRY(msm_tails_joint(m.tails, m.outs, n, &t2, &o2, 1, st, fast), "msm tails (G1 + G2)");
  } else {
    HIP_TRY(msm_tails(m.tails, m.outs, n, st, fast), "msm tails");
    HIP_TRY(msm_tails(&t2, &o2, 1, st, fast), "msm B2 tail");
  }
  return ZKFL_OK;
}

int run_front(zkfl_key* k, ProofSlot* s, const Fr* d_w, const ProofPlan& p, Profiler* prof) {
  hipStream_t st = s->st_main;
  const uint32_t *W = (const uint32_t*)d_w, *E = (const uint32_t*)s->extra;
  HIP_TRY(abc_ntt(k, s, d_w, st, p, prof), "ntt");
  const PlanBases b = plan_bases(k, p);
  FrontMsm m;
  m.n1 = 3;
  const MsmBases<FqOps>* bs[3] = {&b.A, &b.B1, &b.CH};
  MsmScratch<FqOps>* ss[3] = {&s->g1s_a, &s->g1s_b, &s->g1s};
  const uint32_t* ex[3] = {E, E, (const uint32_t*)s->h};
  for (int i = 0; i < 3; i++) {
    m.bases[i] = bs[i];
    m.scratch[i] = ss[i];
    m.tails[i] = &s->g1t[i];
    m.scalars[i] = W;
    m.extra[i] = ex[i];
    m.outs[i] = s->res + i;
  }
  m.ib = 1;
  m.b2 = &b.B2;
  m.t2 = &s->g2t;
  m.nnz_alias = s->nnz_alias;
  m.out2 = s->resB2;
  const int rc = front_msm(m, st, p.fast_wsum, true, prof);
  if (rc) return rc;
  return finish(k, s, p, prof);
}

int run_chain(zkfl_key* k, ProofSlot* s, const Fr* d_w, const ProofPlan& p, Profiler* prof) {
  hipStream_t st = s->st_main;
  const bool parts = p.mode == ProofMode::Parts;
  if (parts && !k->dbg_zero) return fail(ZKFL_E_ARG, "parity hook: zeros not allocated");
  const uint32_t *W = (const uint32_t*)d_w, *E = (const uint32_t*)s->extra, *H = (const uint32_t*)s->h,
                 *Z = (const uint32_t*)k->dbg_zero;
#if ZK_KNOCKOUT & 2
  MsmScratch<FqOps>&sA = s->g1s_ko[0], &sB = s->g1s_ko[1], &sCH = s->g1s_ko[2];
#else
  MsmScratch<FqOps>&sA = s->g1s, &sB = s->g1s, &sCH = s->g1s;
#endif
  const PlanBases b = plan_bases(k, p);
  MsmTail<FqOps>* tails[4] = {&s->g1t[0], &s->g1t[1], &s->g1t[2], &s->g1t[3]};
  G1P* outs[4] = {s->res + 0, s->res + 1, s->res + 2, s->res + 3};
  MsmTail<Fq2Ops>* t2 = &s->g2t;
  G2P* o2 = s->resB2;
  if (!p.share_b_sort && !(ZK_KNOCKOUT & 32))
    HIP_TRY(msm_run(b.B2, s->g2s, s->g2t, W, E, s->resB2, st, prof, "msm_accumulate_g2"), "msm B2");
  if (p.light_first) HIP_TRY(abc_ntt(k, s, d_w, st, p, prof), "ntt");
  HIP_TRY(msm_accumulate(b.A, sA, s->g1t[0], W, E, st, prof, "msm_accumulate_g1"), "msm A");
  if (p.share_b_sort) {
    HIP_TRY(msm_sort(b.B1, sB, s->g1t[1].nnz, W, E, st), "msm B1 sort");
    HIP_TRY(msm_accumulate_sorted(b.B1, sB.keys_out, sB.vals_out, s->g1t[1], st, prof, "msm_accumulate_g1"),
            "msm B1");
    HIP_TRY(b2_from_b1_sort(b.B2, s->g2t, s->g1t[1].nnz, s->nnz_alias, sB, st, prof), "msm B2");
    if (!p.joint_tails) HIP_TRY(msm_tails(&t2, &o2, 1, st, p.fast_wsum), "msm B2 tail");
  } else {
    HIP_TRY(msm_accumulate(b.B1, sB, s->g1t[1], W, E, st, prof, "msm_accumulate_g1"), "msm B1");
  }
  if (parts) HIP_TRY(msm_accumulate(b.CH, s->g1s, s->g1t[2], W, Z, st, prof, "msm_accumulate_g1"), "msm C");
  if (!p.light_first) HIP_TRY(abc_ntt(k, s, d_w, st, p, prof), "ntt");
  if (parts)
    HIP_TRY(msm_accumulate(b.CH, s->g1s, s->g1t[3], Z, H, st, prof, "msm_accumulate_g1"), "msm H");
  else
    HIP_TRY(msm_accumulate(b.CH, sCH, s->g1t[2], W, H, st, prof, "msm_accumulate_g1"), "msm C+H");
  const int ntails = parts ? 4 : 3;
  if (p.joint_tails)
    HIP_TRY(msm_tails_joint(tails, outs, ntails, &t2, &o2, 1, st, p.fast_wsum), "msm tails (G1 + G2)");
  else
    HIP_TRY(msm_tails(tails, outs, ntails, st, p.fast_wsum), "msm tails");
  return finish(k, s, p, prof);
}

int run_proof(zkfl_ctx* ctx, zkfl_key* k, ProofSlot* s, const Fr* d_w, const ProofPlan& p) {
  Profiler* prof = &ctx->prof;
  const int pp = prof->begin("prove", s->st_main);
  start(k, s, p);
  if (p.grouped)
    group_delta(s->st_main, d_w, k->grp.d_rep, k->nVars, s->extra + 4, s->grp_cnt,
                reinterpret_cast<uint32_t*>(s->pinned + MISS_OFF), group_mark(k, s, p));
  if (p.group_rows) group_mark_rows(s->st_main, group_mark(k, s, p));
  const int rc = p.schedule == Schedule::Lowlat  ? run_lowlat(k, s, d_w, p, prof)
                 : p.schedule == Schedule::Front ? run_front(k, s, d_w, p, prof)
                                                 : run_chain(k, s, d_w, p, prof);
  if (rc) return rc;
  prof->end(pp, s->st_main, 1.0);
  return ZKFL_OK;
}

int enqueue_proof_graph(zkfl_ctx* ctx, zkfl_key* k, ProofSlot* s, const ProofPlan& p) {
  hipStream_t st = s->st_main;
  if (!s->graph_exec) {
    HIP_TRY(hipStreamBeginCapture(st, hipStreamCaptureModeThreadLocal), "begin capture");
    const int rc = run_proof(ctx, k, s, s->w_stage, p);
    hipError_t e = hipStreamEndCapture(st, &s->graph);
    if (rc == ZKFL_OK && e == hipSuccess) e = hipGraphInstantiate(&s->graph_exec, s->graph, nullptr, nullptr, 0);
    if (rc || e != hipSuccess) {
      if (s->graph) (void)hipGraphDestroy(s->graph);
      s->graph = nullptr;
      s->graph_exec = nullptr;
      return rc ? rc : hip_fail(e, "graph capture");
    }
  }
  HIP_TRY(hipGraphLaunch(s->graph_exec, st), "graph launch");
  return ZKFL_OK;
}

int enqueue_proof(zkfl_ctx* ctx, zkfl_key* k, ProofSlot* s, const Fr* d_w, const uint32_t rs_host[16], ProofMode mode,
                  bool batch_of_one) {
  memcpy(s->pinned + 256, rs_host, 64);
  GlvScalar* ks = reinterpret_cast<GlvScalar*>(s->pinned + 320);
  glv_split(rs_host + 8, ks[0], ks[1]);
  glv_split(rs_host, ks[2], ks[3]);
  const ProofPlan p = plan_proof(ctx->opts, k, s, mode, batch_of_one, &ctx->prof);
  s->grouped_run = p.grouped;
  s->rows_run = p.group_rows;
  if (p.group_rows && s->cls_cap < k->grp.row_classes) {
    if (s->cls_val) (void)hipFree(s->cls_val);
    s->cls_val = nullptr;
    s->cls_cap = 0;
    HIP_TRY(hipMalloc(&s->cls_val, (size_t)k->grp.row_classes * 32), "class values");
    s->cls_cap = k->grp.row_classes;
  }
  int rc;
  if (p.graph) {
    const uint64_t src = reinterpret_cast<uint64_t>(d_w);
    memcpy(s->pinned + W_PTR_OFF, &src, sizeof(src));
    rc = enqueue_proof_graph(ctx, k, s, p);
  } else {
    s->direct_proofs++;
    rc = run_proof(ctx, k, s, d_w, p);
  }
  if (rc) return rc;
  HIP_TRY(hipEventRecord(s->ev_done, s->st_main), "event");
  HIP_TRY(hipGetLastError(), "launch");
  return ZKFL_OK;
}

constexpr int WAIT_US = 50;
static hipError_t host_wait(hipEvent_t ev, bool poll) {
  if (!poll) return hipEventSynchronize(ev);
  for (;;) {
    const hipError_t e = hipEventQuery(ev);
    if (e != hipErrorNotReady) return e;
    std::this_thread::sleep_for(std::chrono::microseconds(WAIT_US));
  }
}

int wait_slot(ProofSlot* s, bool poll = false) {
  HIP_TRY(host_wait(s->ev_done, poll), "sync");
  if (s->out_proof) memcpy(s->out_proof, s->pinned, 256);
  if (s->out_part) memcpy(s->out_part, s->pinned + 512, PART_WORDS * 4);
  if (s->grouped_run) {
    uint32_t c[3];
    memcpy(c, s->pinned + MISS_OFF, sizeof(c));
    KeyGroups& g = s->key->grp;
    g.last_miss = c[0];
    g.last_dirty = s->rows_run ? c[1] : 0;
    g.last_plain = s->rows_run ? c[2] : 0;
  }
  s->rows_run = false;
  s->grouped_run = false;
  s->busy = false;
  return ZKFL_OK;
}

struct Job {
  zkfl_key* key = nullptr;
  const Fr* w = nullptr;
  hipEvent_t w_ready = nullptr;
  const uint8_t* rs = nullptr;
  uint8_t* proof_out = nullptr;
  uint8_t* part_out = nullptr;
};

int learn_for_batch(zkfl_ctx* ctx, const Job& J, size_t n) {
  zkfl_key* k = J.key;
  if (!ctx->opts.groups || ZK_KNOCKOUT || n < (size_t)ctx->opts.group_min_batch || k->nshards != 1 || J.part_out)
    return ZKFL_OK;
  const KeyGroups& g = k->grp;
  if (g.on && !(g.learned && 2 * (uint64_t)g.last_miss > g.non_rep)) return ZKFL_OK;
  if (J.w_ready) HIP_TRY(hipEventSynchronize(J.w_ready), "wait for the witness group");
  return key_learn_groups(ctx, k, J.w);
}

template <class GetJob>
int run_jobs(zkfl_ctx* ctx, size_t n, GetJob job) {
  HIP_TRY(hipSetDevice(ctx->device), "hipSetDevice");
  struct PerKey {
    zkfl_key* key;
    size_t issued = 0;
  };
  std::vector<PerKey> cursor;
  auto issue = [&](PerKey& pk, size_t i, const Job& J, const uint32_t* rsl) -> int {
    ProofSlot* s = nullptr;
    int rc = get_slot(J.key, pk.issued++, &s);
    if (rc) return rc;
    if (s->busy) {
      rc = wait_slot(s, n > 1);
      if (rc) return rc;
    }
    s->job = i;
    s->out_proof = J.part_out ? nullptr : J.proof_out;
    s->out_part = J.part_out;
    if (J.w_ready) {
      hipError_t e = hipStreamWaitEvent(s->st_main, J.w_ready, 0);
      if (e != hipSuccess) return hip_fail(e, "wait for the witness group");
    }
    rc = enqueue_proof(ctx, J.key, s, J.w, rsl, J.part_out ? ProofMode::SplitPart : ProofMode::Proof, n == 1);
    if (rc) return rc;
    s->busy = true;
    return ZKFL_OK;
  };
  int rc = ZKFL_OK;
  for (size_t i = 0; i < n && rc == ZKFL_OK; i++) {
    Job J;
    rc = job(i, J);
    if (rc) break;
    if (J.key->nshards != 1 && !J.part_out) {
      rc = fail(ZKFL_E_ARG, "this key is shard " + std::to_string(J.key->shard) + " of " +
                                std::to_string(J.key->nshards) +
                                " of a split proof: prove parts (zkfl_groth16_prove_part_batch) and assemble them");
      break;
    }
    uint32_t rsl[16];
    rc = get_rs(J.rs, rsl);
    if (rc) break;
    size_t c = 0;
    while (c < cursor.size() && cursor[c].key != J.key) c++;
    if (c == cursor.size()) {
      cursor.emplace_back();
      cursor.back().key = J.key;
      rc = learn_for_batch(ctx, J, n);
      if (rc) break;
    }
    rc = issue(cursor[c], i, J, rsl);
  }
  for (auto& pk : cursor) {
    for (ProofSlot* s : pk.key->slots)
      if (s->busy) {
        int r2 = wait_slot(s, n > 1);
        if (rc == ZKFL_OK) rc = r2;
      }
  }
  return rc;
}

}

extern "C" {

int zkfl_groth16_prove_resident(zkfl_ctx* ctx, zkfl_key* key, const zkfl_witness* w, const uint8_t* rs,
                                uint8_t proof_out[256]) {
  return zkfl_groth16_prove_batch(ctx, key, 1, &w, rs, proof_out);
}

int zkfl_key_set_slots(zkfl_key* key, int slots) {
  if (!key || slots < 1 || slots > 32) return fail(ZKFL_E_ARG, "slots must be in 1..32");
  (void)hipSetDevice(key->ctx->device);
  for (ProofSlot* s : key->slots) {
    if (s->busy) return fail(ZKFL_E_ARG, "slots busy");
// ... 587 lines not shown
```

verifiable-federated-training-with-zero-knowledge-proofs-zk-fl-_amd/csrc/zkfl.hip:

```cpp
#include <hip/hip_runtime.h>
#include <stdint.h>
#include <string.h>
#include <sys/random.h>

#include <algorithm>
#include <cstdlib>
#include <string>
#include <type_traits>
#include <vector>

#include "assemble.h"
#include "devbufs.h"
#include "glv.h"
#include "host_parse.h"
#include "merkle.h"
#include "objects.h"
#include "poly.h"
#include "setup.h"
#include "verify.h"
#include "witness.h"

using namespace zkfl;

static thread_local std::string g_err;
// ... 115 lines not shown

extern "C" {

int zkfl_version(void) { return 1; }

int zkfl_debug_glv_split(const uint8_t k[32], uint8_t out[40]) {
  if (!k || !out) return fail(ZKFL_E_ARG, "null argument");
  uint32_t kk[8];
  memcpy(kk, k, 32);
  if (!fr_lt_r(kk)) return fail(ZKFL_E_ARG, "k must be < r");
  GlvScalar a, b;
  glv_split(kk, a, b);
  memcpy(out, a.mag, 16);
  memcpy(out + 16, &a.neg, 4);
  memcpy(out + 20, b.mag, 16);
  memcpy(out + 36, &b.neg, 4);
  return ZKFL_OK;
}

int zkfl_debug_g1_glv_mul(zkfl_ctx* ctx, size_t n, const uint8_t* points, const uint8_t* scalars, uint8_t* out) {
  if (!ctx || (n && (!points || !scalars || !out))) return fail(ZKFL_E_ARG, "null argument");
  if (n == 0) return ZKFL_OK;
  if (n > (1u << 20)) return fail(ZKFL_E_ARG, "glv mul: n too large");
  std::vector<GlvScalar> ks(2 * n);
  for (size_t i = 0; i < n; i++) {
    uint32_t kk[8];
    memcpy(kk, scalars + 32 * i, 32);
    if (!fr_lt_r(kk)) return fail(ZKFL_E_ARG, "glv mul: scalar " + std::to_string(i) + " is not < r");
    glv_split(kk, ks[2 * i], ks[2 * i + 1]);
  }
  HIP_TRY(hipSetDevice(ctx->device), "hipSetDevice");
  hipStream_t st = ctx->st;
  DevBufs D;
  uint32_t *d_p, *d_o;
  GlvScalar* d_k;
  HIP_TRY(D.get(&d_p, n * 16), "glv mul");
  HIP_TRY(D.get(&d_k, ks.size()), "glv mul");
  HIP_TRY(D.get(&d_o, n * 16), "glv mul");
  HIP_TRY(hipMemcpyAsync(d_p, points, n * 64, hipMemcpyHostToDevice, st), "glv mul");
  HIP_TRY(hipMemcpyAsync(d_k, ks.data(), ks.size() * sizeof(GlvScalar), hipMemcpyHostToDevice, st), "glv mul");
  debug_glv_mul(st, (uint32_t)n, d_p, d_k, d_o);
  HIP_TRY(hipGetLastError(), "glv mul");
  HIP_TRY(hipMemcpyAsync(out, d_o, n * 64, hipMemcpyDeviceToHost, st), "glv mul");
  HIP_TRY(hipStreamSynchronize(st), "glv mul");
  return ZKFL_OK;
}

const char* zkfl_last_error(void) { return g_err.c_str(); }

int zkfl_device_count(int* count) {
  if (!count) return fail(ZKFL_E_ARG, "null");
  int c = 0;
  hipError_t e = hipGetDeviceCount(&c);
  if (e != hipSuccess) {
    *count = 0;
    return hip_fail(e, "hipGetDeviceCount");
  }
  *count = c;
  return ZKFL_OK;
}

int zkfl_ctx_create(int device, zkfl_ctx** out) {
  if (!out) return fail(ZKFL_E_ARG, "null out");
  int c = 0;
  if (hipGetDeviceCount(&c) != hipSuccess || c == 0) return fail(ZKFL_E_DEVICE, "no HIP device available");
  if (device < 0 || device >= c) return fail(ZKFL_E_ARG, "device index out of range");
  HIP_TRY(hipSetDevice(device), "hipSetDevice");
  zkfl_ctx* ctx = new zkfl_ctx();
  ctx->device = device;
  auto env = [](const char* name, int dflt) {
    const char* v = getenv(name);
    return v ? atoi(v) : dflt;
  };
  ctx->opts.graph = env("ZKFL_GRAPH", 1) != 0;
  ctx->opts.stagger = env("ZKFL_STAGGER", 1) != 0;
  ctx->opts.lowlat = env("ZKFL_LOWLAT", 1) != 0;
  ctx->opts.fast_wsum = env("ZKFL_FAST_WSUM", 1) != 0;
  ctx->opts.small_logn = env("ZKFL_SMALL_LOGN", 16);
  ctx->opts.ab_shared = env("ZKFL_AB_SHARED", 1) != 0;
  ctx->opts.groups = env("ZKFL_GROUPS", 1) != 0;
  ctx->opts.group_min_batch = std::max(1, env("ZKFL_GROUP_MIN_BATCH", 8));
  ctx->opts.group_rows = env("ZKFL_GROUP_ROWS", 1) != 0;
  ctx->opts.group_rows_cap = std::max(0, env("ZKFL_GROUP_ROWS_CAP", 0));
  hipError_t e = hipStreamCreateWithFlags(&ctx->st, hipStreamNonBlocking);
  if (e != hipSuccess) {
    delete ctx;
    return hip_fail(e, "hipStreamCreate");
  }
  *out = ctx;
  return ZKFL_OK;
}

int zkfl_ctx_destroy(zkfl_ctx* ctx) {
  if (!ctx) return ZKFL_OK;
  (void)hipSetDevice(ctx->device);
  (void)hipStreamSynchronize(ctx->st);
  ctx_release(ctx);
  return ZKFL_OK;
}

int zkfl_ctx_set_profiling(zkfl_ctx* ctx, int enabled) {
  if (!ctx) return fail(ZKFL_E_ARG, "null ctx");
  ctx->prof.on = enabled != 0;
  ctx->prof.serialize = enabled == 2;
  return ZKFL_OK;
}

int zkfl_ctx_profile(zkfl_ctx* ctx, const char* name, double* total_ms, uint64_t* launches, double* units,
                     double* median_ms) {
  if (!ctx || !name || !total_ms || !launches) return fail(ZKFL_E_ARG, "null");
  (void)hipSetDevice(ctx->device);
  HIP_TRY(hipDeviceSynchronize(), "sync");
  ctx->prof.query(name, total_ms, launches, units, median_ms);
  return ZKFL_OK;
}

int zkfl_ctx_profile_reset(zkfl_ctx* ctx) {
  if (!ctx) return fail(ZKFL_E_ARG, "null ctx");
  (void)hipStreamSynchronize(ctx->st);
  ctx->prof.reset();
  return ZKFL_OK;
}

int zkfl_ctx_synchronize(zkfl_ctx* ctx) {
  if (!ctx) return fail(ZKFL_E_ARG, "null ctx");
  HIP_TRY(hipSetDevice(ctx->device), "hipSetDevice");
  HIP_TRY(hipDeviceSynchronize(), "sync");
  return ZKFL_OK;
}

int zkfl_witness_upload(zkfl_ctx* ctx, const zkfl_key* key, const uint8_t* wtns, size_t wtns_len,
                        zkfl_witness** out) {
  if (!ctx || !key || !wtns || !out) return fail(ZKFL_E_ARG, "null argument");
  WtnsView v;
  int rc = parse_wtns(wtns, wtns_len, v);
  if (rc) return rc;
  if (v.n != key->nVars) return fail(ZKFL_E_MISMATCH, "wtns: nWitness != zkey nVars");
  HIP_TRY(hipSetDevice(ctx->device), "hipSetDevice");
  zkfl_witness* w = new zkfl_witness();
  w->key = key;
  hipError_t e = hipMalloc(&w->d, (size_t)v.n * 32);
  if (e == hipSuccess) e = hipMemcpyAsync(w->d, v.data, (size_t)v.n * 32, hipMemcpyHostToDevice, ctx->st);
  if (e == hipSuccess) e = hipStreamSynchronize(ctx->st);
  if (e != hipSuccess) {
    zkfl_witness_free(w);
    return hip_fail(e, "witness upload");
  }
  w->pub.assign(v.data + 32, v.data + 32 + (size_t)key->nPub * 32);
  *out = w;
  return ZKFL_OK;
}

int zkfl_witness_free(zkfl_witness* w) {
  if (!w) return ZKFL_OK;
  if (w->d) (void)hipFree(w->d);
  delete w;
  return ZKFL_OK;
}

int zkfl_debug_wtrace(zkfl_ctx* ctx, int op, uint32_t cap, void* out, uint32_t* count) {
#if !ZK_WTRACE
  (void)ctx;
  (void)op;
  (void)cap;
  (void)out;
  (void)count;
// ... 645 lines not shown
```

verifiable-federated-training-with-zero-knowledge-proofs-zk-fl-_amd/zkfl/native.py:

```python

from __future__ import annotations

import ctypes as C
import os

_PKG_DIR = os.path.dirname(os.path.dirname(os.path.abspath(__file__)))
LIB_PATH = os.path.abspath(os.environ["ZKFL_LIB"]) if os.environ.get("ZKFL_LIB") else os.path.join(_PKG_DIR, "libzkfl.so")

ZKFL_OK = 0
PART_BYTES = 768
PART_LAYOUT = {"A": (0, 128), "B1": (128, 256), "B2": (256, 512), "C": (512, 640), "H": (640, 768)}
ERRORS = {
    -1: "ZKFL_E_ARG", -2: "ZKFL_E_FORMAT", -3: "ZKFL_E_PRIME", -4: "ZKFL_E_MISMATCH",
    -5: "ZKFL_E_DEVICE", -6: "ZKFL_E_OOM", -7: "ZKFL_E_CONSTRAINT", -8: "ZKFL_E_KEY",
}

_P = C.c_void_p
_U8P = C.POINTER(C.c_uint8)


class R1csHeader(C.Structure):
    _fields_ = [("n_wires", C.c_uint32), ("n_pub_out", C.c_uint32), ("n_pub_in", C.c_uint32),
                ("n_prv_in", C.c_uint32), ("n_constraints", C.c_uint32), ("n_labels", C.c_uint64),
                ("n_terms", C.c_uint64)]

    def as_dict(self) -> dict:
        return {k: int(getattr(self, k)) for k, _ in self._fields_}


class R1csReport(C.Structure):
    _fields_ = [("n_failed", C.c_uint32), ("first", C.c_uint32), ("a", C.c_uint8 * 32), ("b", C.c_uint8 * 32),
                ("c", C.c_uint8 * 32)]


class PtauView(C.Structure):
    _fields_ = [("power", C.c_uint32),
                ("L", C.c_char_p), ("L2", C.c_char_p), ("La", C.c_char_p), ("Lb", C.c_char_p), ("H0", C.c_char_p),
                ("L_len", C.c_size_t), ("L2_len", C.c_size_t), ("La_len", C.c_size_t), ("Lb_len", C.c_size_t),
                ("H0_len", C.c_size_t),
                ("alpha1", C.c_char_p), ("beta1", C.c_char_p), ("beta2", C.c_char_p)]


KEY_CHECKS = ("header", "points", "coefficients", "A", "B1", "B2", "IC", "C", "H")
KEY_STATES = ("pass", "fail", "not run")


class ZkeyReport(C.Structure):
    _fields_ = [("status", C.c_uint32 * len(KEY_CHECKS)),
                ("point_section", C.c_uint32), ("point_index", C.c_uint32), ("point_count", C.c_uint32),
                ("coef_matrix", C.c_uint32), ("coef_row", C.c_uint32), ("coef_count", C.c_uint32)]


PTAU_CHECKS = ("STRUCTURE", "POINTS", "TAU_G1", "TAU_G2", "ALPHA_G1", "BETA_G1", "BETA_G2",
               "L_TAU_G1", "L_TAU_G2", "L_ALPHA_G1", "L_BETA_G1")
PTAU_LAGRANGE_CHECKS = PTAU_CHECKS[7:]


class PtauHeader(C.Structure):
    _fields_ = [("power", C.c_uint32), ("ceremony_power", C.c_uint32), ("prepared", C.c_uint32),
                ("contributions", C.c_uint32)]

    def as_dict(self) -> dict:
        return {k: int(getattr(self, k)) for k, _ in self._fields_}


class PtauReportC(C.Structure):
    _fields_ = [("status", C.c_uint32 * len(PTAU_CHECKS)), ("prepared", C.c_uint32), ("power", C.c_uint32),
                ("point_section", C.c_uint32), ("point_index", C.c_uint32), ("point_count", C.c_uint32),
                ("chunks", C.c_uint32)]


GROUP_QUERIES = ("A", "B1", "B2", "CH")


class GroupsInfo(C.Structure):
    _fields_ = [("grouped", C.c_uint32), ("learned", C.c_uint32), ("groups", C.c_uint32), ("non_rep", C.c_uint32),
                ("bases", C.c_uint32 * 4), ("bases_rep", C.c_uint32 * 4), ("builds", C.c_uint32),
                ("last_miss", C.c_uint32), ("build_ms", C.c_double)]


class GroupRowsInfo(C.Structure):
    _fields_ = [("rows_grouped", C.c_uint32), ("row_classes", C.c_uint32), ("terms", C.c_uint32),
                ("terms_rep", C.c_uint32), ("wire_list", C.c_uint32), ("wires_over_cap", C.c_uint32),
                ("last_dirty", C.c_uint32), ("last_plain", C.c_uint32), ("rows_build_ms", C.c_double)]


SIGNATURES = {
    "zkfl_version": (C.c_int, []),
    "zkfl_build_id": (C.c_char_p, []),
    "zkfl_last_error": (C.c_char_p, []),
    "zkfl_device_count": (C.c_int, [C.POINTER(C.c_int)]),
    "zkfl_ctx_create": (C.c_int, [C.c_int, C.POINTER(_P)]),
    "zkfl_ctx_destroy": (C.c_int, [_P]),
    "zkfl_ctx_set_profiling": (C.c_int, [_P, C.c_int]),
    "zkfl_ctx_profile": (C.c_int, [_P, C.c_char_p, C.POINTER(C.c_double), C.POINTER(C.c_uint64),
                                   C.POINTER(C.c_double), C.POINTER(C.c_double)]),
    "zkfl_ctx_profile_reset": (C.c_int, [_P]),
    "zkfl_ctx_synchronize": (C.c_int, [_P]),
    "zkfl_zkey_load": (C.c_int, [_P, C.c_char_p, C.c_size_t, C.POINTER(_P)]),
    "zkfl_zkey_load_shard": (C.c_int, [_P, C.c_char_p, C.c_size_t, C.c_uint32, C.c_uint32, C.POINTER(_P)]),
    "zkfl_zkey_file_open": (C.c_int, [C.c_char_p, C.POINTER(_P)]),
    "zkfl_zkey_load_file": (C.c_int, [_P, _P, C.POINTER(_P)]),
    "zkfl_zkey_file_close": (C.c_int, [_P]),
    "zkfl_key_shard": (C.c_int, [_P, C.POINTER(C.c_uint32), C.POINTER(C.c_uint32)]),
    "zkfl_groth16_prove_part_batch": (C.c_int, [_P, _P, C.c_size_t, C.POINTER(_P), C.c_char_p, _U8P]),
    "zkfl_groth16_assemble": (C.c_int, [_P, C.c_size_t, C.c_size_t, C.c_char_p, C.c_char_p, _U8P]),
    "zkfl_key_free": (C.c_int, [_P]),
    "zkfl_key_info": (C.c_int, [_P, C.POINTER(C.c_uint32), C.POINTER(C.c_uint32), C.POINTER(C.c_uint32)]),
    "zkfl_key_ab_shared": (C.c_int, [_P, C.POINTER(C.c_uint32), C.POINTER(C.c_uint32), C.POINTER(C.c_uint32)]),
    "zkfl_debug_ab_partition": (C.c_int, [C.c_char_p, C.c_char_p, C.c_size_t, C.c_uint32, C.c_uint32,
                                          C.POINTER(C.c_uint32), C.POINTER(C.c_uint32), _U8P]),
    "zkfl_key_set_groups": (C.c_int, [_P, C.POINTER(C.c_uint32), C.c_size_t]),
    "zkfl_key_learn_groups": (C.c_int, [_P, _P, _P]),
    "zkfl_key_groups": (C.c_int, [_P, C.POINTER(GroupsInfo)]),
    "zkfl_key_group_rows": (C.c_int, [_P, C.POINTER(GroupRowsInfo)]),
    "zkfl_debug_groups": (C.c_int, [C.c_char_p, C.c_char_p, C.c_size_t, C.POINTER(C.c_uint32), C.POINTER(C.c_uint32),
                                    C.c_size_t, C.c_uint32, C.POINTER(C.c_uint32), C.POINTER(C.c_uint32),
                                    C.POINTER(C.c_uint32)]),
    "zkfl_debug_group_rows": (C.c_int, [C.POINTER(C.c_uint32), C.c_uint32, C.POINTER(C.c_uint32), C.c_uint32,
                                        C.POINTER(C.c_uint32), C.POINTER(C.c_uint32), C.c_uint32, C.c_uint32,
                                        C.c_uint32] + [C.POINTER(C.c_uint32)] * 7),
    "zkfl_debug_abc": (C.c_int, [_P, _P, _P, C.c_int, _U8P, C.POINTER(C.c_uint32)]),
    "zkfl_key_set_slots": (C.c_int, [_P, C.c_int]),
    "zkfl_groth16_prove": (C.c_int, [_P, _P, C.c_char_p, C.c_size_t, C.c_char_p, _U8P, _U8P,
                                     C.POINTER(C.c_size_t)]),
    "zkfl_witness_upload": (C.c_int, [_P, _P, C.c_char_p, C.c_size_t, C.POINTER(_P)]),
    "zkfl_witness_free": (C.c_int, [_P]),
    "zkfl_groth16_prove_resident": (C.c_int, [_P, _P, _P, C.c_char_p, _U8P]),
    "zkfl_groth16_prove_batch": (C.c_int, [_P, _P, C.c_size_t, C.POINTER(_P), C.c_char_p, _U8P]),
    "zkfl_debug_prove_parts": (C.c_int, [_P, _P, C.c_char_p, C.c_size_t, _U8P, _U8P]),
    "zkfl_debug_glv_split": (C.c_int, [C.c_char_p, _U8P]),
    "zkfl_debug_g1_glv_mul": (C.c_int, [_P, C.c_size_t, C.c_char_p, C.c_char_p, _U8P]),
    "zkfl_debug_msm_front": (C.c_int, [_P, C.c_uint32, C.POINTER(C.c_size_t), C.POINTER(C.c_char_p),
                                       C.POINTER(C.c_char_p), C.POINTER(C.c_size_t),
                                       C.POINTER(C.POINTER(C.c_uint32)), C.POINTER(C.c_uint32), C.POINTER(C.c_char_p),
                                       C.POINTER(C.c_size_t), C.c_uint32, C.c_char_p, C.c_size_t, C.c_int, C.c_int,
                                       _U8P, _U8P]),
    "zkfl_debug_wtrace": (C.c_int, [_P, C.c_int, C.c_uint32, _P, C.POINTER(C.c_uint32)]),
    "zkfl_msm_g1": (C.c_int, [_P, C.c_char_p, C.c_char_p, C.c_size_t, _U8P]),
    "zkfl_msm_g2": (C.c_int, [_P, C.c_char_p, C.c_char_p, C.c_size_t, _U8P]),
    "zkfl_ntt_coset": (C.c_int, [_P, _U8P, C.c_uint32]),
    "zkfl_debug_ntt_coset": (C.c_int, [_P, _U8P, C.c_uint32, C.c_uint32, C.c_size_t, C.c_int]),
    "zkfl_setup_g1_gen_mul": (C.c_int, [_P, C.c_char_p, C.c_size_t, _U8P]),
    "zkfl_setup_g2_gen_mul": (C.c_int, [_P, C.c_char_p, C.c_size_t, _U8P]),
    "zkfl_setup_g1_scale": (C.c_int, [_P, C.c_char_p, C.c_char_p, C.c_size_t, _U8P]),
    "zkfl_setup_g2_scale": (C.c_int, [_P, C.c_char_p, C.c_char_p, C.c_size_t, _U8P]),
    "zkfl_setup_g1_lagrange": (C.c_int, [_P, C.c_char_p, C.c_uint32, _U8P]),
    "zkfl_setup_g2_lagrange": (C.c_int, [_P, C.c_char_p, C.c_uint32, _U8P]),
    "zkfl_setup_g1_lincomb": (C.c_int, [_P, C.c_char_p, C.c_size_t, C.c_size_t, C.POINTER(C.c_uint64),
                                        C.POINTER(C.c_uint32), C.c_char_p, _U8P]),
    "zkfl_setup_g2_lincomb": (C.c_int, [_P, C.c_char_p, C.c_size_t, C.c_size_t, C.POINTER(C.c_uint64),
                                        C.POINTER(C.c_uint32), C.c_char_p, _U8P]),
    "zkfl_groth16_verify": (C.c_int, [_P, C.c_char_p, C.c_size_t, C.c_char_p, C.c_size_t, C.c_char_p]),
    "zkfl_groth16_verify_batch": (C.c_int, [_P, C.c_char_p, C.c_size_t, C.c_size_t, C.c_char_p, C.c_size_t,
                                            C.c_char_p, C.POINTER(C.c_int32)]),
    "zkfl_pairing": (C.c_int, [_P, C.c_size_t, C.c_char_p, C.c_char_p, _U8P]),
    "zkfl_debug_miller_loop": (C.c_int, [_P, C.c_size_t, C.c_char_p, C.c_char_p, _U8P]),
    "zkfl_vkey_load": (C.c_int, [_P, C.c_char_p, C.c_size_t, C.POINTER(_P)]),
    "zkfl_vkey_info": (C.c_int, [_P, C.POINTER(C.c_uint32)]),
    "zkfl_vkey_free": (C.c_int, [_P]),
    "zkfl_groth16_verify_multi": (C.c_int, [_P, C.c_size_t, C.POINTER(_P), C.POINTER(C.c_char_p),
                                            C.POINTER(C.c_size_t), C.c_char_p, C.POINTER(C.c_int32), C.c_int]),
    "zkfl_groth16_verify_round": (C.c_int, [_P, C.c_size_t, C.POINTER(_P), C.POINTER(C.c_char_p),
                                            C.POINTER(C.c_size_t), C.c_char_p, C.c_char_p, C.POINTER(C.c_int32),
                                            C.POINTER(C.c_uint32)]),
    "zkfl_debug_verify_round": (C.c_int, [_P, C.c_size_t, C.POINTER(_P), C.POINTER(C.c_char_p),
                                          C.POINTER(C.c_size_t), C.c_char_p, C.c_char_p, C.c_size_t, _U8P,
                                          C.POINTER(C.c_int32)]),
    "zkfl_debug_wave_pairing": (C.c_int,[_P, C.c_size_t, C.c_char_p, C.c_char_p, C.c_int, _U8P]),
    "zkfl_wprog_load": (C.c_int, [_P, C.c_char_p, C.c_size_t, C.POINTER(_P)]),
    "zkfl_wprog_free": (C.c_int, [_P]),
    "zkfl_wprog_info": (C.c_int, [_P, C.POINTER(C.c_uint32), C.POINTER(C.c_uint32), C.POINTER(C.c_uint32)]),
    "zkfl_wtns_size": (C.c_size_t, [_P]),
    "zkfl_witness_compute": (C.c_int, [_P, _P, C.c_size_t, C.c_char_p, _U8P]),
    "zkfl_witness_compute_resident": (C.c_int, [_P, _P, _P, C.c_size_t, C.c_char_p, C.POINTER(_P)]),
    "zkfl_wprog_parse_inputs": (C.c_int, [C.c_char_p, C.c_size_t, C.c_char_p, _U8P, C.c_size_t,
                                          C.POINTER(C.c_size_t)]),
    "zkfl_witness_compute_json": (C.c_int, [_P, _P, C.c_char_p, _U8P]),
    "zkfl_groth16_full_prove_batch": (C.c_int, [_P, _P, _P, C.c_size_t, C.c_char_p, C.c_char_p, _U8P, _U8P]),
    "zkfl_poseidon_params": (C.c_int, [C.c_uint32, _U8P, _U8P, C.POINTER(C.c_uint32)]),
    "zkfl_poseidon_batch": (C.c_int, [_P, C.c_uint32, C.c_size_t, C.c_char_p, _U8P]),
    "zkfl_vector_hash_batch": (C.c_int, [_P, C.c_uint32, C.c_size_t, C.c_char_p, _U8P]),
    "zkfl_merkle_build": (C.c_int, [_P, C.c_char_p, C.c_size_t, C.c_uint32, _U8P]),
    "zkfl_dataset_commit": (C.c_int, [_P, C.c_char_p, C.c_size_t, C.c_uint32, C.c_uint32, _U8P]),
    "zkfl_groth16_full_prove_json": (C.c_int, [_P, _P, _P, C.c_char_p, C.c_char_p, _U8P, _U8P]),
    "zkfl_groth16_prove_multi": (C.c_int, [_P, C.c_size_t, C.POINTER(_P), C.POINTER(_P), C.c_char_p, _U8P]),
    "zkfl_groth16_full_prove_json_batch": (C.c_int, [_P, _P, _P, C.c_size_t, C.POINTER(C.c_char_p), C.c_char_p, _U8P,
                                                     _U8P]),
    "zkfl_groth16_full_prove_multi": (C.c_int, [_P, C.c_size_t, C.POINTER(_P), C.POINTER(_P), C.POINTER(C.c_char_p),
                                                C.c_char_p, _U8P, C.POINTER(_U8P)]),
    "zkfl_r1cs_parse": (C.c_int, [C.c_char_p, C.c_size_t, C.POINTER(R1csHeader)]),
    "zkfl_r1cs_load": (C.c_int, [_P, C.c_char_p, C.c_size_t, C.POINTER(_P)]),
    "zkfl_r1cs_info": (C.c_int, [_P, C.POINTER(R1csHeader)]),
    "zkfl_r1cs_free": (C.c_int, [_P]),
    "zkfl_r1cs_check": (C.c_int, [_P, _P, C.c_size_t, C.POINTER(C.c_char_p), C.POINTER(C.c_size_t),
                                  C.POINTER(R1csReport)]),
    "zkfl_r1cs_check_resident": (C.c_int, [_P, _P, C.c_size_t, C.POINTER(_P), C.POINTER(R1csReport)]),
    "zkfl_zkey_check": (C.c_int, [_P, _P, C.c_char_p, C.c_size_t, C.POINTER(PtauView), C.c_char_p, C.c_char_p,
                                  C.POINTER(ZkeyReport)]),
    "zkfl_ptau_parse": (C.c_int, [_P, C.c_size_t, C.POINTER(PtauHeader)]),
    "zkfl_ptau_check": (C.c_int, [_P, _P, C.c_size_t, C.c_char_p, C.c_uint32, C.POINTER(PtauReportC)]),
# ... 491 lines not shown
        check(lib().zkfl_groth16_assemble(self.h, n, n_parts, parts, rs, out))
        return _proofs(out, n)

    def pairing(self, g1: bytes, g2: bytes, final_exp: bool = True) -> bytes:
        n = len(g1) // 64
        assert len(g1) == 64 * n and len(g2) == 128 * n
        out = _buf(384 * n if n else 1)
        fn = lib().zkfl_pairing if final_exp else lib().zkfl_debug_miller_loop
        check(fn(self.h, n, g1, g2, out))
        return bytes(out)[:384 * n]


VERIFY_SCHEDULES = {"auto": 0, "lanes": 1, "waves": 2}
ROUND_REPORT_FIELDS = ("keys", "screened", "combined", "passed", "fallback")


class VerifyingKey(_Handle):
    _free = "zkfl_vkey_free"

    def __init__(self, ctx: Context, vk_bytes: bytes):
        h = _P()
        check(lib().zkfl_vkey_load(ctx.h, vk_bytes, len(vk_bytes), C.byref(h)))
        self.h = h
        self.ctx = ctx
        ctx._own(self)
        npub = C.c_uint32()
        check(lib().zkfl_vkey_info(h, C.byref(npub)))
        self.n_public = npub.value


class ProvingKey(_Handle):
    _free = "zkfl_key_free"

    def __init__(self, ctx: Context, zkey, shard: int = 0, n_shards: int = 1):
        h = _P()
        if isinstance(zkey, (str, os.PathLike)):
            if (shard, n_shards) != (0, 1):
                with open(zkey, "rb") as f:
                    zkey = f.read()
            else:
                fh = _P()
                check(lib().zkfl_zkey_file_open(os.fsencode(zkey), C.byref(fh)))
                try:
                    check(lib().zkfl_zkey_load_file(ctx.h, fh, C.byref(h)))
                finally:
                    lib().zkfl_zkey_file_close(fh)
        if h:
            pass
        elif n_shards == 1 and shard == 0:
            check(lib().zkfl_zkey_load(ctx.h, zkey, len(zkey), C.byref(h)))
        else:
            check(lib().zkfl_zkey_load_shard(ctx.h, zkey, len(zkey), shard, n_shards, C.byref(h)))
        self.h = h
        self.shard, self.n_shards = shard, n_shards
        self.ctx = ctx
        ctx._own(self)
        nv, npub, dom = C.c_uint32(), C.c_uint32(), C.c_uint32()
        check(lib().zkfl_key_info(h, C.byref(nv), C.byref(npub), C.byref(dom)))
        self.n_vars, self.n_public, self.domain_size = nv.value, npub.value, dom.value

    def ab_shared(self) -> dict:
        d, sh, nb = C.c_uint32(), C.c_uint32(), C.c_uint32()
        check(lib().zkfl_key_ab_shared(self.h, C.byref(d), C.byref(sh), C.byref(nb)))
        return {"form": "D" if d.value else "A", "shared_wires": sh.value, "a_bases": nb.value}

    def set_groups(self, rep):
        if rep is None:
            check(lib().zkfl_key_set_groups(self.h, None, 0))
            return
        arr = (C.c_uint32 * max(1, len(rep)))(*rep)
        check(lib().zkfl_key_set_groups(self.h, arr, len(rep)))

    def learn_groups(self, w: "ResidentWitness"):
        check(lib().zkfl_key_learn_groups(self.ctx.h, self.h, w.h))

    def groups(self) -> dict:
        g = GroupsInfo()
        check(lib().zkfl_key_groups(self.h, C.byref(g)))
        r = GroupRowsInfo()
        check(lib().zkfl_key_group_rows(self.h, C.byref(r)))
        return {"grouped": bool(g.grouped), "learned": bool(g.learned), "groups": g.groups, "non_rep": g.non_rep,
                "bases": dict(zip(GROUP_QUERIES, g.bases)), "bases_rep": dict(zip(GROUP_QUERIES, g.bases_rep)),
                "builds": g.builds, "last_miss": g.last_miss, "build_ms": g.build_ms,
                "rows_grouped": bool(r.rows_grouped), "row_classes": r.row_classes, "terms": r.terms,
                "terms_rep": r.terms_rep, "wire_list": r.wire_list, "wires_over_cap": r.wires_over_cap,
                "last_dirty": r.last_dirty, "last_plain": bool(r.last_plain), "rows_build_ms": r.rows_build_ms}

    def debug_abc(self, w: "ResidentWitness", grouped: bool = True):
        out = _buf(96 * self.domain_size)
        cnt = (C.c_uint32 * 3)()
        check(lib().zkfl_debug_abc(self.ctx.h, self.h, w.h, 1 if grouped else 0, out, cnt))
        return bytes(out), cnt[0], cnt[1], bool(cnt[2])

    def set_slots(self, slots: int):
        check(lib().zkfl_key_set_slots(self.h, slots))
        self.slots = slots

    def prove(self, wtns: bytes, rs: bytes | None = None):
        proof = _buf(256)
        pub = _buf(32 * max(1, self.n_public))
        npub = C.c_size_t()
        check(lib().zkfl_groth16_prove(self.ctx.h, self.h, wtns, len(wtns), rs, proof, pub, C.byref(npub)))
        pb = bytes(pub)
        return bytes(proof), [int.from_bytes(pb[32 * i:32 * i + 32], "little") for i in range(npub.value)]

    def upload(self, wtns: bytes) -> "ResidentWitness":
        return ResidentWitness(self, wtns)

    def prove_resident(self, w: "ResidentWitness", rs: bytes | None = None) -> bytes:
        proof = _buf(256)
        check(lib().zkfl_groth16_prove_resident(self.ctx.h, self.h, w.h, rs, proof))
        return bytes(proof)

    def prove_batch(self, ws, rs: bytes | None = None) -> list:
        n = len(ws)
        arr = (_P * n)(*[w.h for w in ws])
        out = _buf(256 * n)
        check(lib().zkfl_groth16_prove_batch(self.ctx.h, self.h, n, arr, rs, out))
        return _proofs(out, n)

    def prove_part_batch(self, ws, rs: bytes) -> list:
        n = len(ws)
        if rs is None or len(rs) != 64 * n:
            raise ZkflError(-1, "prove_part_batch: rs must be n x 64 bytes")
        arr = (_P * max(1, n))(*[w.h for w in ws])
        out = _buf(PART_BYTES * max(1, n))
        check(lib().zkfl_groth16_prove_part_batch(self.ctx.h, self.h, n, arr, rs, out))
        ob = bytes(out)
        return [ob[PART_BYTES * i:PART_BYTES * (i + 1)] for i in range(n)]

    def full_prove_batch(self, prog: "WitnessProgram", inputs, rs: bytes | None = None):
        n = len(inputs)
        buf = prog._inputs(inputs)
        out = _buf(256 * max(1, n))
        pubs = _buf(32 * max(1, self.n_public) * max(1, n))
        check(lib().zkfl_groth16_full_prove_batch(self.ctx.h, self.h, prog.h, n, buf, rs, out, pubs))
        return _proofs_publics(out, pubs, n, self.n_public)

    def full_prove_json_batch(self, prog: "WitnessProgram", texts, rs: bytes | None = None):
        n = len(texts)
        arr = (C.c_char_p * max(1, n))(*[t.encode() if isinstance(t, str) else t for t in texts])
        out = _buf(256 * max(1, n))
        pubs = _buf(32 * max(1, self.n_public) * max(1, n))
        check(lib().zkfl_groth16_full_prove_json_batch(self.ctx.h, self.h, prog.h, n, arr, rs, out, pubs))
        return _proofs_publics(out, pubs, n, self.n_public)

    def full_prove_json(self, prog: "WitnessProgram", input_json: str, rs: bytes | None = None):
        out = _buf(256)
        pub = _buf(32 * max(1, self.n_public))
        check(lib().zkfl_groth16_full_prove_json(self.ctx.h, self.h, prog.h, input_json.encode(), rs, out, pub))
        return bytes(out), _ints(bytes(pub))[:self.n_public]

    def debug_parts(self, wtns: bytes):
        h = _buf(32 * self.domain_size)
        m = _buf(384)
        check(lib().zkfl_debug_prove_parts(self.ctx.h, self.h, wtns, len(wtns), h, m))
        hb, mb = bytes(h), bytes(m)
        hs = [int.from_bytes(hb[32 * i:32 * i + 32], "little") for i in range(self.domain_size)]
        parts = dict(A=mb[0:64], B1=mb[64:128], B2=mb[128:256], C=mb[256:320], H=mb[320:384])
        return hs, parts


class ResidentWitness(_Handle):
    _free = "zkfl_witness_free"

    def __init__(self, key: ProvingKey, wtns: bytes | None = None, handle=None):
# ... 205 lines not shown
```

Before: 860.2 proofs/s.

## Let MSM sorts walk only live bases plus missed group members

Builds per-query live lists (bases that are not grouped non-representatives) and a wire-to-base map at key build time. The MSM sort kernel then iterates only the live bases plus the per-proof list of group members whose values missed their representative, instead of scanning every base. This is meant to cut sort work on grouped keys, at the cost of extra device buffers and a more complex sort path. It also adds profiler spans around sorts and tails, and no longer disables group learning under knockout builds.

After: 861.6 proofs/s, median of 6. About the same (+0.2%).

```diff
diff --git a/include/zkfl.h b/include/zkfl.h
--- a/include/zkfl.h
+++ b/include/zkfl.h
@@ -57,6 +57,9 @@
   uint32_t builds;
   uint32_t last_miss;
   double build_ms;
+  uint32_t live[4];
+  uint32_t live_lists;
+  uint32_t reserved_;
 } zkfl_groups_info;
 typedef struct zkfl_group_rows_info {
   uint32_t rows_grouped;
@@ -76,6 +79,8 @@
 int zkfl_debug_groups(const uint8_t* values, const uint8_t* sig, size_t n, uint32_t* rep_out, const uint32_t* sidx,
                       size_t n_bases, uint32_t u_base, uint32_t* sidx_out, uint32_t* start_out,
                       uint32_t* members_out);
+int zkfl_debug_live_lists(const uint32_t* gsidx, size_t n_bases, uint32_t u_base, uint32_t n_vars, uint32_t* live_out,
+                          uint32_t* n_live_out, uint32_t* base_of_out);
 int zkfl_debug_group_rows(const uint32_t* rows, uint32_t domain, const uint32_t* cols, uint32_t cshift,
                           const uint32_t* coefs, const uint32_t* rep, uint32_t n_vars, uint32_t hash_bits,
                           uint32_t wire_cap, uint32_t* cls_out, uint32_t* crp_out, uint32_t* cterms_out,
diff --git a/verifiable-federated-training-with-zero-knowledge-proofs-zk-fl-_amd/csrc/groups.h b/verifiable-federated-training-with-zero-knowledge-proofs-zk-fl-_amd/csrc/groups.h
--- a/verifiable-federated-training-with-zero-knowledge-proofs-zk-fl-_amd/csrc/groups.h
+++ b/verifiable-federated-training-with-zero-knowledge-proofs-zk-fl-_amd/csrc/groups.h
@@ -70,6 +70,18 @@
   std::vector<uint32_t> cur(q.start.begin(), q.start.end() - 1);
   for (size_t j = 0; j < n; j++)
     if (to[j] != NONE) q.members[cur[to[j]]++] = (uint32_t)j;
+}
+
+constexpr uint32_t LIVE_NONE = 0xFFFFFFFFu;
+inline void groups_live(const uint32_t* gsidx, size_t n, uint32_t u_base, uint32_t n_vars, std::vector<uint32_t>& live,
+                        std::vector<uint32_t>& base_of) {
+  live.clear();
+  base_of.assign(n_vars, LIVE_NONE);
+  for (size_t j = 0; j < n; j++) {
+    const uint32_t si = gsidx[j];
+    if (si >= u_base && si - u_base < n_vars) base_of[si - u_base] = (uint32_t)j;
+    else live.push_back((uint32_t)j);
+  }
 }
 
 
diff --git a/verifiable-federated-training-with-zero-knowledge-proofs-zk-fl-_amd/csrc/groups.hip b/verifiable-federated-training-with-zero-knowledge-proofs-zk-fl-_amd/csrc/groups.hip
--- a/verifiable-federated-training-with-zero-knowledge-proofs-zk-fl-_amd/csrc/groups.hip
+++ b/verifiable-federated-training-with-zero-knowledge-proofs-zk-fl-_amd/csrc/groups.hip
@@ -63,7 +63,7 @@
     }
     u[i] = v;
   }
-  if (M.wstart) {
+  if (M.missing) {
     const unsigned long long m = __ballot(nz);
     if (m) {
       const uint32_t lane = threadIdx.x & (warpSize - 1);
@@ -171,6 +171,24 @@
   group_sums<F>(st, plain.bases_w, msm_w_of(plain.c), plain.n, d_start, d_members, d_img);
   ZK_CHECK(hipGetLastError());
   return msm_bases_set(out, d_img, q.sidx.data(), extra_start, st, false);
+}
+
+bool live_lists_wanted(const zkfl_key* k) { return k->ctx->opts.live_sort && k->logn > k->ctx->opts.small_logn; }
+
+template <class F>
+hipError_t build_live(MsmBases<F>& out, const GroupQuery& q, uint32_t u_base, uint32_t n_vars, uint32_t* n_live_out,
+                      hipStream_t st) {
+  std::vector<uint32_t> live, base_of;
+  groups_live(q.sidx.data(), q.sidx.size(), u_base, n_vars, live, base_of);
+  *n_live_out = (uint32_t)live.size();
+  if (out.n == 0) return hipSuccess;
+  ZK_CHECK(hipMalloc(&out.live, (live.size() ? live.size() : 1) * 4));
+  ZK_CHECK(hipMalloc(&out.base_of, (base_of.size() ? base_of.size() : 1) * 4));
+  if (!live.empty()) ZK_CHECK(hipMemcpyAsync(out.live, live.data(), live.size() * 4, hipMemcpyHostToDevice, st));
+  if (!base_of.empty())
+    ZK_CHECK(hipMemcpyAsync(out.base_of, base_of.data(), base_of.size() * 4, hipMemcpyHostToDevice, st));
+  out.n_live = (uint32_t)live.size();
+  return hipStreamSynchronize(st);
 }
 
 bool group_rows_wanted(const zkfl_key* k) {
@@ -246,6 +264,13 @@
     if (e == hipSuccess) e = build_query(k->bCH, k->gCH, q[3], X, D, st);
     const hipError_t es = hipStreamSynchronize(st);
     if (e == hipSuccess) e = es;
+    if (live_lists_wanted(k)) {
+      if (e == hipSuccess) e = build_live(k->gA, q[0], u_base[0], nV, &k->grp.live[0], st);
+      if (e == hipSuccess) e = build_live(k->gB1, q[1], u_base[1], nV, &k->grp.live[1], st);
+      if (e == hipSuccess) e = build_live(k->gB2, q[2], u_base[2], nV, &k->grp.live[2], st);
+      if (e == hipSuccess) e = build_live(k->gCH, q[3], u_base[3], nV, &k->grp.live[3], st);
+      k->grp.live_on = e == hipSuccess;
+    }
     if (e == hipSuccess) e = build_rows(k, rep, st);
   }
   if (e != hipSuccess) {
@@ -270,9 +295,10 @@
   g.build_ms = host_ms + std::chrono::duration<double, std::milli>(std::chrono::steady_clock::now() - t0).count();
   fprintf(stderr,
           "zkfl: key of %u wires: %u groups, %u non-representative wires; bases A %u -> %u, B %u -> %u, C+H %u -> %u; "
-          "%s and built in %.1f ms\n",
+          "live lists A %u, B %u, C+H %u (%s); %s and built in %.1f ms\n",
           nV, g.groups, g.non_rep, g.bases[0], g.bases_rep[0], g.bases[1], g.bases_rep[1], g.bases[3], g.bases_rep[3],
-          learned ? "learned" : "set", g.build_ms);
+          g.live[0], g.live[1], g.live[3], g.live_on ? "the sorts walk them" : "not built", learned ? "learned" : "set",
+          g.build_ms);
   if (group_rows_wanted(k))
     fprintf(stderr,
             "zkfl: key of %u wires: %u row classes, terms %zu -> %u, wire lists %u entries (%u wires over the cap); "
@@ -338,7 +364,9 @@
   for (int i = 0; i < 4; i++) {
     out->bases[i] = g.on ? g.bases[i] : (uint32_t)key->q_sidx[i].size();
     out->bases_rep[i] = g.on ? g.bases_rep[i] : out->bases[i];
-  }
+    out->live[i] = g.live_on ? g.live[i] : 0;
+  }
+  out->live_lists = g.live_on;
   out->builds = g.builds;
   out->last_miss = g.last_miss;
   out->build_ms = g.build_ms;
@@ -395,6 +423,18 @@
   return ZKFL_OK;
 }
 
+int zkfl_debug_live_lists(const uint32_t* gsidx, size_t n_bases, uint32_t u_base, uint32_t n_vars, uint32_t* live_out,
+                          uint32_t* n_live_out, uint32_t* base_of_out) {
+  if ((n_bases && !gsidx) || !live_out || !n_live_out || !base_of_out || n_bases > 0x7FFFFFF0u)
+    return fail(ZKFL_E_ARG, "debug_live_lists: bad arguments");
+  std::vector<uint32_t> live, base_of;
+  groups_live(gsidx, n_bases, u_base, n_vars, live, base_of);
+  if (!live.empty()) memcpy(live_out, live.data(), live.size() * 4);
+  if (!base_of.empty()) memcpy(base_of_out, base_of.data(), base_of.size() * 4);
+  *n_live_out = (uint32_t)live.size();
+  return ZKFL_OK;
+}
+
 int zkfl_debug_groups(const uint8_t* values, const uint8_t* sig, size_t n, uint32_t* rep_out, const uint32_t* sidx,
                       size_t n_bases, uint32_t u_base, uint32_t* sidx_out, uint32_t* start_out,
                       uint32_t* members_out) {
diff --git a/verifiable-federated-training-with-zero-knowledge-proofs-zk-fl-_amd/csrc/msm.h b/verifiable-federated-training-with-zero-knowledge-proofs-zk-fl-_amd/csrc/msm.h
--- a/verifiable-federated-training-with-zero-knowledge-proofs-zk-fl-_amd/csrc/msm.h
+++ b/verifiable-federated-training-with-zero-knowledge-proofs-zk-fl-_amd/csrc/msm.h
@@ -517,6 +517,8 @@
 void msm_bases_free(MsmBases<F>& b) {
   if (b.bases_w) (void)hipFree(b.bases_w);
   if (b.sidx) (void)hipFree(b.sidx);
+  if (b.live) (void)hipFree(b.live);
+  if (b.base_of) (void)hipFree(b.base_of);
   b = MsmBases<F>();
 }
 
@@ -659,7 +661,7 @@
 
 template <class F>
 hipError_t msm_sort_multi(const MsmBases<F>* const* b, MsmScratch<F>* const* pl, uint32_t* const* nnz,
-                          const uint32_t* const* sc, const uint32_t* const* ex, int n, hipStream_t st) {
+                          const uint32_t* const* sc, const uint32_t* const* ex, int n, hipStream_t st, Profiler* prof) {
   if (n < 1 || n > MSM_TAIL_MAX) return hipErrorInvalidValue;
   MsmSortArgs A = {};
   uint32_t gx = 0;
@@ -678,20 +680,32 @@
     J = {sc[i], ex[i], b[i]->sidx, b[i]->extra_start, (uint32_t)m, per_blk, nblk,
          static_cast<uint32_t*>(pl[i]->sort_tmp), static_cast<uint32_t*>(pl[i]->sort_tmp) + MSM_SORT_HB * MSM_SORT_MAXBLK,
          nnz[i], pl[i]->keys_in, pl[i]->vals_in, pl[i]->keys_out, pl[i]->vals_out};
+    const MsmSortLive& lv = pl[i]->lv;
+    if (b[i]->live && b[i]->base_of && lv.missing && lv.n_missing && b[i]->n_live <= m) {
+      J.live = b[i]->live;
+      J.base_of = b[i]->base_of;
+      J.missing = lv.missing;
+      J.n_missing = lv.n_missing;
+      J.n_live = b[i]->n_live;
+      J.miss_cap = lv.miss_cap;
+    }
     gx = std::max(gx, nblk);
     sorted = sorted && pl[i]->ko_sorted;
     pl[i]->ko_sorted = 1;
   }
   if (ny == 0) return hipSuccess;
-  return msm_sort_launch(A, gx, ny, c, sorted, st);
+  const int pidx = prof ? prof->begin("msm_sort", st) : -1;
+  const hipError_t e = msm_sort_launch(A, gx, ny, c, sorted, st);
+  if (prof) prof->end(pidx, st, (double)ny);
+  return e;
 }
 
 template <class F>
 hipError_t msm_sort(const MsmBases<F>& b, MsmScratch<F>& pl, uint32_t* nnz, const uint32_t* d_scalars,
-                    const uint32_t* d_extra, hipStream_t st) {
+                    const uint32_t* d_extra, hipStream_t st, Profiler* prof) {
   const MsmBases<F>* bp = &b;
   MsmScratch<F>* pp = &pl;
-  return msm_sort_multi(&bp, &pp, &nnz, &d_scalars, &d_extra, 1, st);
+  return msm_sort_multi(&bp, &pp, &nnz, &d_scalars, &d_extra, 1, st, prof);
 }
 
 template <class F>
@@ -751,7 +765,7 @@
 template <class F>
 hipError_t msm_accumulate(const MsmBases<F>& b, MsmScratch<F>& pl, MsmTail<F>& t, const uint32_t* d_scalars,
                           const uint32_t* d_extra, hipStream_t st, Profiler* prof, const char* tag) {
-  ZK_CHECK(msm_sort(b, pl, t.nnz, d_scalars, d_extra, st));
+  ZK_CHECK(msm_sort(b, pl, t.nnz, d_scalars, d_extra, st, prof));
   return msm_accumulate_sorted(b, pl.keys_out, pl.vals_out, t, st, prof, tag);
 }
 
@@ -805,14 +819,17 @@
 }
 
 template <class F>
-hipError_t msm_tails(MsmTail<F>* const* t, XYZZ<F>* const* outs, int n, hipStream_t st, bool fast) {
-  ZK_CHECK(msm_stitch(t, n, st));
-  return msm_wsum(msm_tail_args<F>(t, outs, n), n, st, fast);
+hipError_t msm_tails(MsmTail<F>* const* t, XYZZ<F>* const* outs, int n, hipStream_t st, bool fast, Profiler* prof) {
+  const int pidx = prof ? prof->begin("msm_tails", st) : -1;
+  hipError_t e = msm_stitch(t, n, st);
+  if (e == hipSuccess) e = msm_wsum(msm_tail_args<F>(t, outs, n), n, st, fast);
+  if (prof) prof->end(pidx, st, (double)n);
+  return e;
 }
 
 template <class S1, class S2>
 hipError_t msm_tails_joint(MsmTail<S1>* const* t1, XYZZ<S1>* const* o1, int n1, MsmTail<S2>* const* t2,
-                           XYZZ<S2>* const* o2, int n2, hipStream_t st, bool fast) {
+                           XYZZ<S2>* const* o2, int n2, hipStream_t st, bool fast, Profiler* prof) {
   if (n1 < 1 || n1 > MSM_TAIL_MAX || n2 < 1 || n2 > MSM_TAIL_MAX || !msm_tails_one_c(t1, n1) ||
       !msm_tails_one_c(t2, n2) || t1[0]->c != t2[0]->c)
     return hipErrorInvalidValue;
@@ -831,6 +848,7 @@
   for (int i = 0; i < n1; i++) N1 = std::max(N1, t1[i]->item_cap[0]);
   for (int i = 0; i < n2; i++) N2 = std::max(N2, t2[i]->item_cap[0]);
   int cur = 0;
+  const int pidx = prof ? prof->begin("msm_tails", st) : -1;
   for (int level = 1; !(ZK_KNOCKOUT & 8); level++) {
     if (level >= MSM_LIVE_LEVELS) return hipErrorInvalidValue;
     const size_t lanes1 = (N1 + MSM_SG - 1) / MSM_SG, lanes2 = (N2 + MSM_SG - 1) / MSM_SG;
@@ -845,8 +863,11 @@
     if (N2 > (size_t)MSM_SG) N2 = 2 * lanes2;
     cur ^= 1;
   }
-  if (ZK_KNOCKOUT & 16) return hipGetLastError();
-  return msm_with_c(t1[0]->c, [&](auto cc) {
+  if (ZK_KNOCKOUT & 16) {
+    if (prof) prof->end(pidx, st, (double)ny);
+    return hipGetLastError();
+  }
+  const hipError_t e = msm_with_c(t1[0]->c, [&](auto cc) {
     constexpr int C = decltype(cc)::value, NB = msm_nb_of(C);
     constexpr int Q0 = MsmCurve<S1>::WSUM_Q, QF = msm_wsum_q_fast<C>();
     if (fast) {
@@ -862,6 +883,8 @@
     }
     return hipGetLastError();
   });
+  if (prof) prof->end(pidx, st, (double)ny);
+  return e;
 }
 
 template <class F>
@@ -870,7 +893,7 @@
   MsmTail<F>* tp = &t;
   ZK_CHECK(msm_tails_reset(&tp, 1, st));
   ZK_CHECK(msm_accumulate(b, pl, t, d_scalars, d_extra, st, prof, tag));
-  return msm_tails(&tp, &d_out, 1, st);
-}
-
-}
+  return msm_tails(&tp, &d_out, 1, st, false, prof);
+}
+
+}
diff --git a/verifiable-federated-training-with-zero-knowledge-proofs-zk-fl-_amd/csrc/msm_api.h b/verifiable-federated-training-with-zero-knowledge-proofs-zk-fl-_amd/csrc/msm_api.h
--- a/verifiable-federated-training-with-zero-knowledge-proofs-zk-fl-_amd/csrc/msm_api.h
+++ b/verifiable-federated-training-with-zero-knowledge-proofs-zk-fl-_amd/csrc/msm_api.h
@@ -68,6 +68,15 @@
   Affine<F>* bases_w = nullptr;
   uint32_t* sidx = nullptr;
   uint32_t extra_start = 0xFFFFFFFFu;
+  uint32_t* live = nullptr;
+  uint32_t n_live = 0;
+  uint32_t* base_of = nullptr;
+};
+
+struct MsmSortLive {
+  const uint32_t* missing = nullptr;
+  const uint32_t* n_missing = nullptr;
+  uint32_t miss_cap = 0;
 };
 
 template <class F>
@@ -81,6 +90,7 @@
   void* sort_tmp = nullptr;
   size_t sort_tmp_bytes = 0;
   int ko_sorted = 0;
+  MsmSortLive lv;
 };
 
 template <class F>
@@ -144,18 +154,20 @@
 hipError_t msm_tails_reset(MsmTail<F>* const* t, int n, hipStream_t st);
 template <class F>
 hipError_t msm_sort(const MsmBases<F>& b, MsmScratch<F>& s, uint32_t* nnz, const uint32_t* sc, const uint32_t* ex,
-                    hipStream_t st);
+                    hipStream_t st, Profiler* prof = nullptr);
 template <class F>
 hipError_t msm_accumulate_sorted(const MsmBases<F>& b, const uint16_t* keys, const uint32_t* vals, MsmTail<F>& t,
                                  hipStream_t st, Profiler* prof, const char* tag);
 template <class F>
-hipError_t msm_tails(MsmTail<F>* const* t, XYZZ<F>* const* outs, int n, hipStream_t st, bool fast = false);
+hipError_t msm_tails(MsmTail<F>* const* t, XYZZ<F>* const* outs, int n, hipStream_t st, bool fast = false,
+                     Profiler* prof = nullptr);
 template <class F>
 hipError_t msm_run(const MsmBases<F>& b, MsmScratch<F>& s, MsmTail<F>& t, const uint32_t* scalars,
                    const uint32_t* extra, XYZZ<F>* out, hipStream_t st, Profiler* prof, const char* tag);
 template <class F>
 hipError_t msm_sort_multi(const MsmBases<F>* const* b, MsmScratch<F>* const* s, uint32_t* const* nnz,
-                          const uint32_t* const* sc, const uint32_t* const* ex, int n, hipStream_t st);
+                          const uint32_t* const* sc, const uint32_t* const* ex, int n, hipStream_t st,
+                          Profiler* prof = nullptr);
 template <class F>
 hipError_t msm_accumulate_sorted_multi(const MsmBases<F>* const* b, const uint16_t* const* keys,
                                        const uint32_t* const* vals, MsmTail<F>* const* t, int n, hipStream_t st);
@@ -172,20 +184,20 @@
                                  const uint32_t*, hipStream_t, Profiler*, const char*);                        \
   X hipError_t msm_tails_reset<F>(MsmTail<F>* const*, int, hipStream_t);                                       \
   X hipError_t msm_sort<F>(const MsmBases<F>&, MsmScratch<F>&, uint32_t*, const uint32_t*, const uint32_t*,    \
-                           hipStream_t);                                                                       \
+                           hipStream_t, Profiler*);                                                            \
   X hipError_t msm_accumulate_sorted<F>(const MsmBases<F>&, const uint16_t*, const uint32_t*, MsmTail<F>&,     \
                                         hipStream_t, Profiler*, const char*);                                  \
-  X hipError_t msm_tails<F>(MsmTail<F>* const*, XYZZ<F>* const*, int, hipStream_t, bool);                      \
+  X hipError_t msm_tails<F>(MsmTail<F>* const*, XYZZ<F>* const*, int, hipStream_t, bool, Profiler*);           \
   X hipError_t msm_run<F>(const MsmBases<F>&, MsmScratch<F>&, MsmTail<F>&, const uint32_t*, const uint32_t*,   \
                           XYZZ<F>*, hipStream_t, Profiler*, const char*);                                      \
   X hipError_t msm_sort_multi<F>(const MsmBases<F>* const*, MsmScratch<F>* const*, uint32_t* const*,           \
-                                 const uint32_t* const*, const uint32_t* const*, int, hipStream_t);            \
+                                 const uint32_t* const*, const uint32_t* const*, int, hipStream_t, Profiler*); \
   X hipError_t msm_accumulate_sorted_multi<F>(const MsmBases<F>* const*, const uint16_t* const*,               \
                                               const uint32_t* const*, MsmTail<F>* const*, int, hipStream_t);
 ZKFL_MSM_API(extern template, FqOps)
 ZKFL_MSM_API(extern template, Fq2Ops)
 
 hipError_t msm_tails_joint(MsmTail<FqOps>* const* t1, XYZZ<FqOps>* const* o1, int n1, MsmTail<Fq2Ops>* const* t2,
-                           XYZZ<Fq2Ops>* const* o2, int n2, hipStream_t st, bool fast);
-
-}
+                           XYZZ<Fq2Ops>* const* o2, int n2, hipStream_t st, bool fast, Profiler* prof = nullptr);
+
+}
diff --git a/verifiable-federated-training-with-zero-knowledge-proofs-zk-fl-_amd/csrc/msm_joint.hip b/verifiable-federated-training-with-zero-knowledge-proofs-zk-fl-_amd/csrc/msm_joint.hip
--- a/verifiable-federated-training-with-zero-knowledge-proofs-zk-fl-_amd/csrc/msm_joint.hip
+++ b/verifiable-federated-training-with-zero-knowledge-proofs-zk-fl-_amd/csrc/msm_joint.hip
@@ -3,7 +3,7 @@
 namespace zkfl {
 hipError_t zk_wtrace_bind_joint(const WtBuf& b) { return zk_wtrace_bind_tu(b); }
 hipError_t msm_tails_joint(MsmTail<FqOps>* const* t1, XYZZ<FqOps>* const* o1, int n1, MsmTail<Fq2Ops>* const* t2,
-                           XYZZ<Fq2Ops>* const* o2, int n2, hipStream_t st, bool fast) {
-  return msm_tails_joint<FqOps, Fq2Ops>(t1, o1, n1, t2, o2, n2, st, fast);
+                           XYZZ<Fq2Ops>* const* o2, int n2, hipStream_t st, bool fast, Profiler* prof) {
+  return msm_tails_joint<FqOps, Fq2Ops>(t1, o1, n1, t2, o2, n2, st, fast, prof);
 }
 }
diff --git a/verifiable-federated-training-with-zero-knowledge-proofs-zk-fl-_amd/csrc/msm_sort.h b/verifiable-federated-training-with-zero-knowledge-proofs-zk-fl-_amd/csrc/msm_sort.h
--- a/verifiable-federated-training-with-zero-knowledge-proofs-zk-fl-_amd/csrc/msm_sort.h
+++ b/verifiable-federated-training-with-zero-knowledge-proofs-zk-fl-_amd/csrc/msm_sort.h
@@ -25,6 +25,11 @@
   uint32_t* vals_in;
   uint16_t* keys_out;
   uint32_t* vals_out;
+  const uint32_t* live;
+  const uint32_t* base_of;
+  const uint32_t* missing;
+  const uint32_t* n_missing;
+  uint32_t n_live, miss_cap;
 };
 struct MsmSortArgs {
   MsmSortJob j[MSM_TAIL_MAX];
diff --git a/verifiable-federated-training-with-zero-knowledge-proofs-zk-fl-_amd/csrc/msm_sort.hip b/verifiable-federated-training-with-zero-knowledge-proofs-zk-fl-_amd/csrc/msm_sort.hip
--- a/verifiable-federated-training-with-zero-knowledge-proofs-zk-fl-_amd/csrc/msm_sort.hip
+++ b/verifiable-federated-training-with-zero-knowledge-proofs-zk-fl-_amd/csrc/msm_sort.hip
@@ -45,6 +45,34 @@
   }
 }
 
+struct MsmSortWalk {
+  uint32_t lo, hi, n_live;
+  bool lists;
+};
+ZK_DEV MsmSortWalk msm_sort_walk(const MsmSortJob& J, uint32_t blk) {
+  MsmSortWalk w;
+  uint32_t total = J.n, per = J.per_blk;
+  w.lists = false;
+  w.n_live = 0;
+  if (J.live) {
+    const uint32_t nm = *J.n_missing;
+    if (nm <= J.miss_cap) {
+      w.lists = true;
+      w.n_live = J.n_live;
+      total = J.n_live + nm;
+      per = (total + J.nblk - 1) / J.nblk;
+    }
+  }
+  const uint64_t lo = (uint64_t)blk * per, hi = lo + per;
+  w.lo = lo < total ? (uint32_t)lo : total;
+  w.hi = hi < total ? (uint32_t)hi : total;
+  return w;
+}
+ZK_DEV uint32_t msm_sort_base(const MsmSortJob& J, const MsmSortWalk& w, uint32_t p) {
+  if (!w.lists) return p;
+  return p < w.n_live ? J.live[p] : J.base_of[J.missing[p - w.n_live]];
+}
+
 template <int C>
 __global__ void __launch_bounds__(MSM_SORT_T) k_msm_bin_count(const MsmSortArgs A) {
   ZK_WT(WT_SORT_COUNT);
@@ -55,10 +83,13 @@
   __shared__ uint32_t h[MSM_SORT_HB];
   if (threadIdx.x < MSM_SORT_HB) h[threadIdx.x] = 0;
   __syncthreads();
-  const size_t i0 = (size_t)blockIdx.x * J.per_blk, i1 = i0 + J.per_blk < J.n ? i0 + J.per_blk : J.n;
-  for (size_t i = i0 + threadIdx.x; i < i1; i += MSM_SORT_T)
+  const MsmSortWalk w = msm_sort_walk(J, blockIdx.x);
+  for (uint32_t p = w.lo + threadIdx.x; p < w.hi; p += MSM_SORT_T) {
+    const uint32_t i = msm_sort_base(J, w, p);
+    if (i == 0xFFFFFFFFu) continue;
     msm_for_digits<C>(J.scalars, J.extra, J.sidx, J.extra_start, i,
                       [&](uint32_t key, uint32_t) { atomicAdd(&h[key >> LB], 1u); });
+  }
   __syncthreads();
   if (threadIdx.x < MSM_SORT_HB) J.cnt[(size_t)threadIdx.x * J.nblk + blockIdx.x] = h[threadIdx.x];
 }
@@ -124,13 +155,16 @@
   __syncthreads();
   uint16_t* __restrict__ keys = J.keys_in;
   uint32_t* __restrict__ vals = J.vals_in;
-  const size_t i0 = (size_t)blockIdx.x * J.per_blk, i1 = i0 + J.per_blk < J.n ? i0 + J.per_blk : J.n;
-  for (size_t i = i0 + threadIdx.x; i < i1; i += MSM_SORT_T)
+  const MsmSortWalk w = msm_sort_walk(J, blockIdx.x);
+  for (uint32_t q = w.lo + threadIdx.x; q < w.hi; q += MSM_SORT_T) {
+    const uint32_t i = msm_sort_base(J, w, q);
+    if (i == 0xFFFFFFFFu) continue;
     msm_for_digits<C>(J.scalars, J.extra, J.sidx, J.extra_start, i, [&](uint32_t key, uint32_t val) {
       const uint32_t p = atomicAdd(&cur[key >> LB], 1u);
       keys[p] = (uint16_t)key;
       vals[p] = val;
     });
+  }
 }
 
 template <int BINT, int NL>
diff --git a/verifiable-federated-training-with-zero-knowledge-proofs-zk-fl-_amd/csrc/objects.h b/verifiable-federated-training-with-zero-knowledge-proofs-zk-fl-_amd/csrc/objects.h
--- a/verifiable-federated-training-with-zero-knowledge-proofs-zk-fl-_amd/csrc/objects.h
+++ b/verifiable-federated-training-with-zero-knowledge-proofs-zk-fl-_amd/csrc/objects.h
@@ -44,6 +44,7 @@
   int group_min_batch = 8;
   bool group_rows = true;
   int group_rows_cap = 0;
+  bool live_sort = true;
 };
 
 struct zkfl_ctx {
@@ -115,6 +116,8 @@
   uint32_t builds = 0;
   uint32_t last_miss = 0;
   uint32_t* d_rep = nullptr;
+  bool live_on = false;
+  uint32_t live[4] = {0, 0, 0, 0};
   bool rows_on = false;
   uint32_t row_classes = 0;
   uint32_t terms_rep = 0;
diff --git a/verifiable-federated-training-with-zero-knowledge-proofs-zk-fl-_amd/csrc/prove.hip b/verifiable-federated-training-with-zero-knowledge-proofs-zk-fl-_amd/csrc/prove.hip
--- a/verifiable-federated-training-with-zero-knowledge-proofs-zk-fl-_amd/csrc/prove.hip
+++ b/verifiable-federated-training-with-zero-knowledge-proofs-zk-fl-_amd/csrc/prove.hip
@@ -114,11 +114,13 @@
   s->extra = s->h + n;
   ZK_CHECK(hipMalloc(&s->grp_cnt, 2 * sizeof(uint32_t)));
   ZK_CHECK(hipMemsetAsync(s->grp_cnt, 0, 2 * sizeof(uint32_t), st));
-  if (may_group && k->ctx->opts.group_rows && k->K && k->logn > k->ctx->opts.small_logn) {
+  const bool large = may_group && k->logn > k->ctx->opts.small_logn;
+  const bool rows = large && k->ctx->opts.group_rows && k->K;
+  if (rows || (large && k->ctx->opts.live_sort)) {
     ZK_CHECK(hipMalloc(&s->gr_state, group_rows_state_words(n) * sizeof(uint32_t)));
     ZK_CHECK(hipMalloc(&s->gr_missing, (size_t)group_rows_miss_cap((uint32_t)n) * sizeof(uint32_t)));
-    ZK_CHECK(hipMalloc(&s->gr_dirty, (size_t)group_rows_dirty_cap((uint32_t)n) * sizeof(uint32_t)));
-  }
+  }
+  if (rows) ZK_CHECK(hipMalloc(&s->gr_dirty, (size_t)group_rows_dirty_cap((uint32_t)n) * sizeof(uint32_t)));
   s->key = k;
   ZK_CHECK(hipMalloc(&s->abc, n * 3 * 32));
   const size_t abc_chunks = (k->K + ABC_L - 1) / ABC_L + 1;
@@ -279,6 +281,7 @@
   bool graph;
   bool grouped;
   bool group_rows;
+  bool live_sort;
 };
 
 struct PlanBases {
@@ -294,7 +297,7 @@
                      const Profiler* prof) {
   ProofPlan p = {};
   p.mode = mode;
-  p.grouped = mode == ProofMode::Proof && k->grp.on && !ZK_KNOCKOUT;
+  p.grouped = mode == ProofMode::Proof && k->grp.on;
   p.group_rows = p.grouped && k->grp.rows_on && s->gr_state;
   const bool plain = mode == ProofMode::Proof && k->share_b && !prof->serialize && !ZK_KNOCKOUT;
   const bool want_lowlat = batch_of_one && o.lowlat;
@@ -305,6 +308,7 @@
     p.fast_wsum = o.fast_wsum;
     return p;
   }
+  p.live_sort = p.grouped && k->grp.live_on && s->gr_state && s->gr_missing;
   p.joint_tails = p.share_b_sort && k->front;
   const bool front = p.joint_tails && mode != ProofMode::Parts && !(ZK_KNOCKOUT & 2);
   p.schedule = front ? Schedule::Front : Schedule::Chain;
@@ -340,13 +344,19 @@
   if (p.group_rows) {
     ps.gr_state = s->gr_state;
     ps.gr_words = (uint32_t)group_rows_state_words(k->n);
+  } else if (p.live_sort) {
+    ps.gr_state = s->gr_state;
+    ps.gr_words = GROUP_ROWS_STATE_BITS;
   }
   proof_start(s->st_main, reinterpret_cast<const uint32_t*>(s->pinned + 256), reinterpret_cast<uint32_t*>(s->d_rs),
               s->extra, parts, res3, ps);
 }
 
 inline GroupMark group_mark(const zkfl_key* k, const ProofSlot* s, const ProofPlan& p) {
-  if (!p.group_rows) return GroupMark{};
+  if (!p.group_rows) {
+    if (!p.live_sort) return GroupMark{};
+    return {nullptr, nullptr, s->gr_state, s->gr_missing, group_rows_miss_cap(k->n), nullptr, 0};
+  }
   return {k->grp.d_wstart, k->grp.d_wlist, s->gr_state, s->gr_missing, group_rows_miss_cap(k->n), s->gr_dirty,
           group_rows_dirty_cap(k->n)};
 }
@@ -412,23 +422,23 @@
   G2P* o2 = s->resB2;
   HIP_TRY(hipEventRecord(ev, st), "event");
   HIP_TRY(hipStreamWaitEvent(sb, ev, 0), "wait");
-  HIP_TRY(msm_sort(b.B1, s->g1s_b, s->g1t[1].nnz, W, E, sb), "msm B sort");
+  HIP_TRY(msm_sort(b.B1, s->g1s_b, s->g1t[1].nnz, W, E, sb, prof), "msm B sort");
   HIP_TRY(hipEventRecord(ev, sb), "event");
   HIP_TRY(hipStreamWaitEvent(sa, ev, 0), "wait");
   HIP_TRY(b2_from_b1_sort(b.B2, s->g2t, s->g1t[1].nnz, s->nnz_alias, s->g1s_b, sb, prof), "msm B2");
-  HIP_TRY(msm_tails(&t2, &o2, 1, sb, p.fast_wsum), "msm B2 tail");
+  HIP_TRY(msm_tails(&t2, &o2, 1, sb, p.fast_wsum, prof), "msm B2 tail");
   HIP_TRY(hipEventRecord(ev_b2, sb), "event");
   HIP_TRY(msm_accumulate_sorted(b.B1, s->g1s_b.keys_out, s->g1s_b.vals_out, s->g1t[1], sa, prof,
                                    "msm_accumulate_g1"), "msm B1");
   HIP_TRY(msm_accumulate(b.A, s->g1s_a, s->g1t[0], W, E, sa, prof, "msm_accumulate_g1"), "msm A");
-  HIP_TRY(msm_tails(tails, outs, 2, sa, p.fast_wsum), "msm tails A, B1");
+  HIP_TRY(msm_tails(tails, outs, 2, sa, p.fast_wsum, prof), "msm tails A, B1");
   if (k->a_diff) fold_a(sa, s->res);
   assemble_t(sa, s->res, glv_halves(s), proof_out(s));
   HIP_TRY(hipEventRecord(ev_t, sa), "event");
   HIP_TRY(abc_ntt(k, s, d_w, st, p, prof), "ntt");
   HIP_TRY(msm_accumulate(b.CH, s->g1s, s->g1t[2], W, (const uint32_t*)s->h, st, prof, "msm_accumulate_g1"),
           "msm C+H");
-  HIP_TRY(msm_tails(&tails[2], &outs[2], 1, st, p.fast_wsum), "msm tail C+H");
+  HIP_TRY(msm_tails(&tails[2], &outs[2], 1, st, p.fast_wsum, prof), "msm tail C+H");
   HIP_TRY(hipStreamWaitEvent(st, ev_b2, 0), "wait");
   HIP_TRY(hipStreamWaitEvent(st, ev_t, 0), "wait");
   const int pa = prof->begin("assemble", st);
@@ -457,7 +467,7 @@
   const uint16_t* kk[MSM_TAIL_MAX] = {};
   const uint32_t* vv[MSM_TAIL_MAX] = {};
   for (int i = 0; i < n; i++) nn[i] = m.tails[i]->nnz;
-  HIP_TRY(msm_sort_multi(m.bases, m.scratch, nn, m.scalars, m.extra, n, st), "msm A, B1, C+H sorts");
+  HIP_TRY(msm_sort_multi(m.bases, m.scratch, nn, m.scalars, m.extra, n, st, prof), "msm A, B1, C+H sorts");
   for (int i = 0; i < n; i++) {
     kk[i] = m.scratch[i]->keys_out;
     vv[i] = m.scratch[i]->vals_out;
@@ -467,10 +477,10 @@
   MsmTail<Fq2Ops>* t2 = m.t2;
   G2P* o2 = m.out2;
   if (joint) {
-    HIP_TRY(msm_tails_joint(m.tails, m.outs, n, &t2, &o2, 1, st, fast), "msm tails (G1 + G2)");
+    HIP_TRY(msm_tails_joint(m.tails, m.outs, n, &t2, &o2, 1, st, fast, prof), "msm tails (G1 + G2)");
   } else {
-    HIP_TRY(msm_tails(m.tails, m.outs, n, st, fast), "msm tails");
-    HIP_TRY(msm_tails(&t2, &o2, 1, st, fast), "msm B2 tail");
+    HIP_TRY(msm_tails(m.tails, m.outs, n, st, fast, prof), "msm tails");
+    HIP_TRY(msm_tails(&t2, &o2, 1, st, fast, prof), "msm B2 tail");
   }
   return ZKFL_OK;
 }
@@ -524,11 +534,11 @@
   if (p.light_first) HIP_TRY(abc_ntt(k, s, d_w, st, p, prof), "ntt");
   HIP_TRY(msm_accumulate(b.A, sA, s->g1t[0], W, E, st, prof, "msm_accumulate_g1"), "msm A");
   if (p.share_b_sort) {
-    HIP_TRY(msm_sort(b.B1, sB, s->g1t[1].nnz, W, E, st), "msm B1 sort");
+    HIP_TRY(msm_sort(b.B1, sB, s->g1t[1].nnz, W, E, st, prof), "msm B1 sort");
     HIP_TRY(msm_accumulate_sorted(b.B1, sB.keys_out, sB.vals_out, s->g1t[1], st, prof, "msm_accumulate_g1"),
             "msm B1");
     HIP_TRY(b2_from_b1_sort(b.B2, s->g2t, s->g1t[1].nnz, s->nnz_alias, sB, st, prof), "msm B2");
-    if (!p.joint_tails) HIP_TRY(msm_tails(&t2, &o2, 1, st, p.fast_wsum), "msm B2 tail");
+    if (!p.joint_tails) HIP_TRY(msm_tails(&t2, &o2, 1, st, p.fast_wsum, prof), "msm B2 tail");
   } else {
     HIP_TRY(msm_accumulate(b.B1, sB, s->g1t[1], W, E, st, prof, "msm_accumulate_g1"), "msm B1");
   }
@@ -540,9 +550,9 @@
     HIP_TRY(msm_accumulate(b.CH, sCH, s->g1t[2], W, H, st, prof, "msm_accumulate_g1"), "msm C+H");
   const int ntails = parts ? 4 : 3;
   if (p.joint_tails)
-    HIP_TRY(msm_tails_joint(tails, outs, ntails, &t2, &o2, 1, st, p.fast_wsum), "msm tails (G1 + G2)");
+    HIP_TRY(msm_tails_joint(tails, outs, ntails, &t2, &o2, 1, st, p.fast_wsum, prof), "msm tails (G1 + G2)");
   else
-    HIP_TRY(msm_tails(tails, outs, ntails, st, p.fast_wsum), "msm tails");
+    HIP_TRY(msm_tails(tails, outs, ntails, st, p.fast_wsum, prof), "msm tails");
   return finish(k, s, p, prof);
 }
 
@@ -554,6 +564,12 @@
     group_delta(s->st_main, d_w, k->grp.d_rep, k->nVars, s->extra + 4, s->grp_cnt,
                 reinterpret_cast<uint32_t*>(s->pinned + MISS_OFF), group_mark(k, s, p));
   if (p.group_rows) group_mark_rows(s->st_main, group_mark(k, s, p));
+  const MsmSortLive lv = p.live_sort ? MsmSortLive{s->gr_missing, s->gr_state + 2, group_rows_miss_cap(k->n)}
+                                     : MsmSortLive{};
+  s->g1s.lv = s->g2s.lv = lv;
+#if ZK_KNOCKOUT & 2
+  for (MsmScratch<FqOps>& x : s->g1s_ko) x.lv = lv;
+#endif
   const int rc = p.schedule == Schedule::Lowlat  ? run_lowlat(k, s, d_w, p, prof)
                  : p.schedule == Schedule::Front ? run_front(k, s, d_w, p, prof)
                                                  : run_chain(k, s, d_w, p, prof);
@@ -650,7 +666,7 @@
 
 int learn_for_batch(zkfl_ctx* ctx, const Job& J, size_t n) {
   zkfl_key* k = J.key;
-  if (!ctx->opts.groups || ZK_KNOCKOUT || n < (size_t)ctx->opts.group_min_batch || k->nshards != 1 || J.part_out)
+  if (!ctx->opts.groups || n < (size_t)ctx->opts.group_min_batch || k->nshards != 1 || J.part_out)
     return ZKFL_OK;
   const KeyGroups& g = k->grp;
   if (g.on && !(g.learned && 2 * (uint64_t)g.last_miss > g.non_rep)) return ZKFL_OK;
diff --git a/verifiable-federated-training-with-zero-knowledge-proofs-zk-fl-_amd/csrc/zkfl.hip b/verifiable-federated-training-with-zero-knowledge-proofs-zk-fl-_amd/csrc/zkfl.hip
--- a/verifiable-federated-training-with-zero-knowledge-proofs-zk-fl-_amd/csrc/zkfl.hip
+++ b/verifiable-federated-training-with-zero-knowledge-proofs-zk-fl-_amd/csrc/zkfl.hip
@@ -221,6 +221,7 @@
   ctx->opts.group_min_batch = std::max(1, env("ZKFL_GROUP_MIN_BATCH", 8));
   ctx->opts.group_rows = env("ZKFL_GROUP_ROWS", 1) != 0;
   ctx->opts.group_rows_cap = std::max(0, env("ZKFL_GROUP_ROWS_CAP", 0));
+  ctx->opts.live_sort = env("ZKFL_LIVE_SORT", 1) != 0;
   hipError_t e = hipStreamCreateWithFlags(&ctx->st, hipStreamNonBlocking);
   if (e != hipSuccess) {
     delete ctx;
diff --git a/verifiable-federated-training-with-zero-knowledge-proofs-zk-fl-_amd/zkfl/native.py b/verifiable-federated-training-with-zero-knowledge-proofs-zk-fl-_amd/zkfl/native.py
--- a/verifiable-federated-training-with-zero-knowledge-proofs-zk-fl-_amd/zkfl/native.py
+++ b/verifiable-federated-training-with-zero-knowledge-proofs-zk-fl-_amd/zkfl/native.py
@@ -76,7 +76,8 @@
 class GroupsInfo(C.Structure):
     _fields_ = [("grouped", C.c_uint32), ("learned", C.c_uint32), ("groups", C.c_uint32), ("non_rep", C.c_uint32),
                 ("bases", C.c_uint32 * 4), ("bases_rep", C.c_uint32 * 4), ("builds", C.c_uint32),
-                ("last_miss", C.c_uint32), ("build_ms", C.c_double)]
+                ("last_miss", C.c_uint32), ("build_ms", C.c_double), ("live", C.c_uint32 * 4),
+                ("live_lists", C.c_uint32), ("reserved_", C.c_uint32)]
 
 
 class GroupRowsInfo(C.Structure):
@@ -117,6 +118,8 @@
     "zkfl_debug_groups": (C.c_int, [C.c_char_p, C.c_char_p, C.c_size_t, C.POINTER(C.c_uint32), C.POINTER(C.c_uint32),
                                     C.c_size_t, C.c_uint32, C.POINTER(C.c_uint32), C.POINTER(C.c_uint32),
                                     C.POINTER(C.c_uint32)]),
+    "zkfl_debug_live_lists": (C.c_int, [C.POINTER(C.c_uint32), C.c_size_t, C.c_uint32, C.c_uint32,
+                                        C.POINTER(C.c_uint32), C.POINTER(C.c_uint32), C.POINTER(C.c_uint32)]),
     "zkfl_debug_group_rows": (C.c_int, [C.POINTER(C.c_uint32), C.c_uint32, C.POINTER(C.c_uint32), C.c_uint32,
                                         C.POINTER(C.c_uint32), C.POINTER(C.c_uint32), C.c_uint32, C.c_uint32,
                                         C.c_uint32] + [C.POINTER(C.c_uint32)] * 7),
@@ -774,6 +777,7 @@
         return {"grouped": bool(g.grouped), "learned": bool(g.learned), "groups": g.groups, "non_rep": g.non_rep,
                 "bases": dict(zip(GROUP_QUERIES, g.bases)), "bases_rep": dict(zip(GROUP_QUERIES, g.bases_rep)),
                 "builds": g.builds, "last_miss": g.last_miss, "build_ms": g.build_ms,
+                "live_lists": bool(g.live_lists), "live": dict(zip(GROUP_QUERIES, g.live)),
                 "rows_grouped": bool(r.rows_grouped), "row_classes": r.row_classes, "terms": r.terms,
                 "terms_rep": r.terms_rep, "wire_list": r.wire_list, "wires_over_cap": r.wires_over_cap,
                 "last_dirty": r.last_dirty, "last_plain": bool(r.last_plain), "rows_build_ms": r.rows_build_ms}
```
